# vitasoftAI/ImageRetrievalResearch

Measured on AMD Instinct MI355X. Metric: images/sec embed + queries/sec top-k@100k-gallery, EffNet-B3a 224^2, higher is better.
Workload: dtype bf16

## Files before the change

imageretrievalresearch_amd/_lib.py:

```python
from __future__ import annotations

import ctypes as C
import os

_HERE = os.path.dirname(os.path.abspath(__file__))
LIB_PATH = os.environ.get("MI355_LIB_PATH") or os.path.join(_HERE, "libmi355_retrieval.so")

c_f32p = C.POINTER(C.c_float)
c_i64p = C.POINTER(C.c_int64)
vp = C.c_void_p


class GemmExArgs(C.Structure):
    _fields_ = [("A", vp), ("lda", C.c_int), ("W", vp), ("ldw", C.c_int), ("bias", vp),
                ("res", vp), ("ldr", C.c_int), ("res_n", C.c_int),
                ("gate", vp), ("gate_ld", C.c_int), ("rows_per_img", C.c_int), ("a_relu6", C.c_int),
                ("out", vp), ("ldo", C.c_int), ("out_f32", C.c_int),
                ("M", C.c_int), ("N", C.c_int), ("K", C.c_int), ("act", C.c_int),
                ("M_sel", C.c_int64), ("splitk_ws", vp), ("splitk_ws_bytes", C.c_size_t),
                ("ln_stats", vp), ("ln_colsum", vp)]


class DwconvExArgs(C.Structure):
    _fields_ = [("in_", vp), ("w", vp), ("bias", vp), ("out", vp),
                ("B", C.c_int), ("H", C.c_int), ("W", C.c_int), ("C", C.c_int), ("k", C.c_int), ("stride", C.c_int),
                ("act", C.c_int), ("choice", C.c_int),
                ("se_w1", vp), ("se_b1", vp), ("se_w2t", vp), ("se_b2", vp), ("rd", C.c_int), ("act1", C.c_int),
                ("gate", vp), ("squeeze", vp)]


DW_CHOICE_AUTO, DW_CHOICE_DIRECT, DW_CHOICE_TILED, DW_CHOICE_MFMA = 0, 1, 2, 3


class RankFilter(C.Structure):
    _fields_ = [("query_labels", vp), ("gallery_labels", vp), ("label_mode", C.c_int), ("exclude", vp)]


LABEL_ANY, LABEL_SAME, LABEL_DIFFERENT = 0, 1, 2
DTYPE_F32, DTYPE_F16 = 0, 1

PROTOTYPES = {
    "mi355_abi_version": (C.c_int, []),
    "mi355_last_error": (C.c_char_p, []),
    "mi355_device_count": (C.c_int, []),
    "mi355_synth_fill": (C.c_int, [vp, C.c_int64, C.c_uint64, C.c_int64, C.c_int, vp]),
    "mi355_l2_normalize_rows": (C.c_int, [vp, vp, C.c_int64, C.c_int, C.c_float, vp]),
    "mi355_rank_workspace_bytes": (C.c_size_t, [C.c_int64, C.c_int64, C.c_int, C.c_int]),
    "mi355_rank_topk": (C.c_int, [vp, C.c_int64, vp, C.c_int64, C.c_int, C.c_int, C.c_int, C.c_float,
                                  C.c_int64, vp, vp, vp, C.c_size_t, vp]),
    "mi355_gallery_planes_bytes": (C.c_size_t, [C.c_int64, C.c_int]),
    "mi355_gallery_prepare": (C.c_int, [vp, C.c_int64, C.c_int, vp, C.c_size_t, vp]),
    "mi355_rank_topk_prepared": (C.c_int, [vp, C.c_int64, vp, C.c_int64, C.c_int, C.c_int, C.c_float, C.c_int64, vp, vp, vp,
                                           C.c_size_t, vp]),
    "mi355_gallery_f16_bytes": (C.c_size_t, [C.c_int64, C.c_int]),
    "mi355_gallery_to_f16": (C.c_int, [vp, C.c_int64, C.c_int, C.c_int, C.c_float, vp, C.c_size_t, vp]),
    "mi355_rank_f16_workspace_bytes": (C.c_size_t, [C.c_int64, C.c_int64, C.c_int, C.c_int]),
    "mi355_rank_topk_f16": (C.c_int, [vp, C.c_int64, vp, C.c_int64, C.c_int, C.c_int, C.c_float, C.c_int64, vp, vp, vp,
                                      C.c_size_t, vp]),
    "mi355_rank_topk_filtered": (C.c_int, [vp, C.c_int64, vp, C.c_int64, C.c_int, C.c_int, C.c_int, C.c_float, C.c_int64,
                                           C.POINTER(RankFilter), vp, vp, vp, C.c_size_t, vp]),
    "mi355_rank_topk_f16_filtered": (C.c_int, [vp, C.c_int64, vp, C.c_int64, C.c_int, C.c_int, C.c_float, C.c_int64,
                                               C.POINTER(RankFilter), vp, vp, vp, C.c_size_t, vp]),
    "mi355_rank_last_path": (C.c_int, []),
    "mi355_expand_workspace_bytes": (C.c_size_t, [C.c_int64, C.c_int, C.c_int]),
    "mi355_expand_rows": (C.c_int, [vp, C.c_int, C.c_int64, C.c_int, vp, C.c_int, C.c_int64, C.c_int64, C.c_int, vp, vp,
                                    C.c_int64, C.c_int, C.c_int64, C.c_float, C.c_float, vp, C.c_int, C.c_int64, vp,
                                    C.c_size_t, vp]),
    "mi355_kr_sets": (C.c_int, [vp, vp, vp, C.c_int64, C.c_int, vp, C.c_int64, vp, vp, C.c_int64, vp]),
    "mi355_kr_weights": (C.c_int, [vp, C.c_int, C.c_int64, C.c_int64, vp, C.c_int, C.c_int64, C.c_int64, C.c_int, vp, vp,
                                   C.c_int64, vp, vp]),
    "mi355_kr_local_qe": (C.c_int, [vp, C.c_int64, C.c_int, C.c_int, vp, vp, vp, C.c_int64, vp, vp, vp, C.c_int64, C.c_int64,
                                    vp, vp, vp, C.c_int64, vp]),
    "mi355_kr_score": (C.c_int, [vp, vp, vp, C.c_int64, C.c_int64, vp, vp, vp, C.c_int64, C.c_int64, vp, vp, C.c_int,
                                 C.c_float, vp, vp]),
    "mi355_moments_workspace_bytes": (C.c_size_t, [C.c_int64, C.c_int]),
    "mi355_embedding_moments": (C.c_int, [vp, C.c_int, C.c_int64, C.c_int64, C.c_int, C.c_int, C.c_float, C.c_int, vp, vp, vp,
                                          C.c_size_t, vp]),
    "mi355_whiten_workspace_bytes": (C.c_size_t, [C.c_int64, C.c_int, C.c_int, C.c_int]),
    "mi355_whiten_rows": (C.c_int, [vp, C.c_int, C.c_int64, C.c_int64, C.c_int, C.c_int, C.c_float, vp, vp, C.c_int, C.c_int, vp,
                                    C.c_int, C.c_int64, vp, C.c_size_t, vp]),
    "mi355_clear_pads": (C.c_int, [vp, vp, C.c_int64, C.c_int64, C.c_int64, vp]),
    "mi355_range_workspace_bytes": (C.c_size_t, [C.c_int64, C.c_int64, C.c_int]),
    "mi355_cosine_range": (C.c_int, [vp, C.c_int64, vp, C.c_int64, C.c_int, C.c_int, C.c_float, C.c_double, C.c_int64,
                                     C.POINTER(RankFilter), vp, C.c_int64, C.POINTER(C.c_int64), vp, C.c_size_t, vp]),
    "mi355_range_f16_workspace_bytes": (C.c_size_t, [C.c_int64, C.c_int64, C.c_int]),
    "mi355_cosine_range_f16": (C.c_int, [vp, C.c_int64, vp, C.c_int64, C.c_int, C.c_float, C.c_double, C.c_int64,
                                         C.POINTER(RankFilter), vp, C.c_int64, C.POINTER(C.c_int64), vp, C.c_size_t, vp]),
    "mi355_range_compact": (C.c_int, [vp, C.c_int64, C.c_int64, C.c_int64, C.c_int64, vp, C.c_size_t, vp, vp, vp, vp]),
    "mi355_roc_pairs_workspace_bytes": (C.c_size_t, [C.c_int64, C.c_int64, C.c_int]),
    "mi355_roc_pairs_hist": (C.c_int, [vp, C.c_int64, vp, C.c_int64, C.c_int, C.c_int, C.c_float, vp, vp, vp, C.c_int64,
                                       C.POINTER(C.c_double), vp, C.c_int, vp, vp, C.c_size_t, vp]),
    "mi355_roc_pairs_f16_workspace_bytes": (C.c_size_t, [C.c_int64, C.c_int64, C.c_int]),
    "mi355_roc_pairs_hist_f16": (C.c_int, [vp, C.c_int64, vp, C.c_int64, C.c_int, C.c_float, vp, vp, vp, C.c_int64,
                                           C.POINTER(C.c_double), vp, C.c_int, vp, vp, C.c_size_t, vp]),
    "mi355_roc_scores_hist": (C.c_int, [vp, C.c_int, C.c_int64, vp, C.POINTER(C.c_double), vp, C.c_int, vp, vp]),
    "mi355_roc_finalize": (C.c_int, [vp, C.c_int, vp, vp, vp, vp, vp]),
    "mi355_retrieval_metrics": (C.c_int, [vp, C.c_int64, C.c_int, vp, vp, C.c_int64, vp, vp, vp]),
    "mi355_cosine_scores": (C.c_int, [vp, C.c_int64, vp, C.c_int64, C.c_int, C.c_int, C.c_float, vp, vp,
                                      C.c_size_t, vp]),
    "mi355_topk_rows": (C.c_int, [vp, C.c_int64, C.c_int64, C.c_int, C.c_int64, vp, vp, vp, C.c_size_t, vp]),
    "mi355_merge_topk": (C.c_int, [vp, vp, C.c_int64, C.c_int, C.c_int, vp, vp, vp, C.c_size_t, vp]),
    "mi355_pack_candidates": (C.c_int, [vp, vp, C.c_int64, C.c_int, C.c_int, vp, vp]),
    "mi355_merge_packed_workspace_bytes": (C.c_size_t, [C.c_int64, C.c_int, C.c_int]),
    "mi355_merge_packed_topk": (C.c_int, [vp, vp, C.c_int, C.c_int64, C.c_int, vp, vp, vp, C.c_size_t, vp]),
    "mi355_pair_cosine": (C.c_int, [vp, vp, C.c_int64, C.c_int, C.c_float, vp, vp]),
    "mi355_contrastive_loss": (C.c_int, [vp, vp, C.c_int64, C.c_int, C.c_float, C.c_float, C.c_int, vp, vp, vp]),
    "mi355_cosine_embedding_loss": (C.c_int, [vp, vp, C.c_int64, C.c_int, C.c_float, C.c_float, C.c_int, vp, vp]),
    "mi355_hit_counts": (C.c_int, [vp, C.c_int64, C.c_int, vp, vp, C.c_int64, vp, vp]),
    "mi355_distinct_class_topn": (C.c_int, [vp, vp, C.c_int64, C.c_int, vp, C.c_int64, C.c_int, vp, vp, vp, vp]),
    "mi355_model_create": (C.c_int, [C.c_char_p, C.c_int, C.POINTER(vp)]),
    "mi355_model_destroy": (None, [vp]),
    "mi355_model_num_tensors": (C.c_int, [vp]),
    "mi355_model_tensor_info": (C.c_int, [vp, C.c_int, C.POINTER(C.c_char_p), C.POINTER(C.c_int),
                                          C.POINTER(C.c_int64), C.POINTER(C.c_int)]),
    "mi355_model_feature_dim": (C.c_int, [vp]),
    "mi355_model_num_classes": (C.c_int, [vp]),
    "mi355_model_set_tensor": (C.c_int, [vp, C.c_char_p, vp, C.c_int64]),
    "mi355_model_pack": (C.c_int, [vp, vp]),
    "mi355_model_forward_features": (C.c_int, [vp, vp, C.c_int, C.c_int, C.c_int, vp, vp, vp]),
    "mi355_model_forward": (C.c_int, [vp, vp, C.c_int, C.c_int, C.c_int, vp, vp, vp]),
    "mi355_model_forward_u8": (C.c_int, [vp, vp, C.c_int, C.c_int, C.c_int, C.c_int, C.POINTER(C.c_float), C.POINTER(C.c_float),
                                         vp, C.c_int, vp, vp, vp]),
    "mi355_model_enable_taps": (C.c_int, [vp, C.c_int]),
    "mi355_model_read_tap": (C.c_int, [vp, C.c_char_p, vp, C.c_int64, C.POINTER(C.c_int64), vp]),
    "mi355_model_run_between_taps": (C.c_int, [vp, C.c_char_p, C.c_char_p, vp, C.c_int, C.c_int, C.c_int, C.c_int, vp]),
    "mi355_model_traffic": (C.c_int, [vp, C.c_int, C.c_int, C.c_int, C.POINTER(C.c_double),
                                      C.POINTER(C.c_double), C.POINTER(C.c_double)]),
    "mi355_model_traffic_kinds": (C.c_int, [vp, C.c_int, C.c_int, C.c_int, C.POINTER(C.c_double),
                                            C.POINTER(C.c_double), C.c_int]),
    "mi355_model_set_option": (C.c_int, [vp, C.c_char_p, C.c_int64]),
    "mi355_model_profile_read": (C.c_int, [vp, C.POINTER(C.c_double), C.POINTER(C.c_int64), C.c_int]),
    "mi355_model_profile_ops": (C.c_int, [vp, C.c_int, C.c_int, C.c_int, C.c_int, C.POINTER(C.c_double),
                                          C.POINTER(C.c_double), C.POINTER(C.c_int), C.c_char_p, C.c_int]),
    "mi355_model_block_stamps": (C.c_int, [vp, C.POINTER(C.c_double), C.c_int]),
    "mi355_pool_linear": (C.c_int, [vp, C.c_int, C.c_int, C.c_int, vp, vp, C.c_int, vp, vp, vp]),
    "mi355_gemm_bf16": (C.c_int, [vp, vp, vp, vp, C.c_int, C.c_int, C.c_int, C.c_int, C.c_int, vp]),
    "mi355_gemm_bf16_ex": (C.c_int, [vp, C.POINTER(C.c_int), vp]),
    "mi355_dwconv_se_ex": (C.c_int, [vp, C.POINTER(C.c_int), vp]),
    "mi355_window_attention": (C.c_int, [vp, vp, vp, C.c_int, C.c_int, C.c_int, C.c_int, C.c_int, vp]),
    "mi355_window_attention_ws": (C.c_int, [vp, vp, vp, C.c_int, C.c_int, C.c_int, C.c_int, C.c_int, C.c_int, vp]),
    "mi355_swin_layernorm": (C.c_int, [vp, vp, vp, vp, C.c_int64, C.c_int, C.c_int, C.c_int, C.c_int, C.c_int, C.c_float, vp]),
    "mi355_swin_patch_embed": (C.c_int, [vp, vp, vp, C.c_int, C.c_int, C.c_int, C.c_int, C.c_int, C.c_int, C.POINTER(C.c_float),
                                         C.POINTER(C.c_float), vp, vp, vp, vp, C.c_int, C.c_float, vp, vp]),
    "mi355_swin_ln_token_mean": (C.c_int, [vp, vp, vp, vp, vp, C.c_int, C.c_int, C.c_int, C.c_float, vp]),
    "mi355_square_pad_normalize": (C.c_int, [vp, C.c_int, C.c_int, C.c_int, C.POINTER(C.c_float), C.POINTER(C.c_float), vp, vp]),
    "mi355_conv_input_silu": (C.c_int, [vp, vp, C.c_int, C.c_int, C.c_int, vp, vp]),
    "mi355_resize_bilinear_u8": (C.c_int, [vp, C.c_int, C.c_int, vp, C.c_int, C.c_int, vp, vp]),
    "mi355_resize_batch_workspace_bytes": (C.c_size_t, [vp, C.c_int, C.c_int, C.c_int, C.c_int]),
    "mi355_resize_batch_u8": (C.c_int, [vp, C.c_int64, vp, vp, C.c_int, C.c_int, C.c_int, C.c_int, C.c_int, vp, vp, C.c_size_t,
                                        vp]),
    "mi355_model_forward_images_workspace_bytes": (C.c_size_t, [vp, C.c_int, C.c_int, C.c_int]),
    "mi355_model_forward_images": (C.c_int, [vp, vp, C.c_int64, vp, vp, C.c_int, C.c_int, C.c_int, C.c_int, C.POINTER(C.c_float),
                                             C.POINTER(C.c_float), vp, C.c_int, vp, vp, vp, C.c_size_t, vp]),
    "mi355_score_boost": (C.c_int, [vp, C.c_int64, C.c_float, C.c_float, C.c_float, C.c_int, vp, vp]),
}

_lib = None


class MI355Error(RuntimeError):
    """A libmi355_retrieval call returned nonzero; the message is mi355_last_error()."""


def lib() -> C.CDLL:
    global _lib
    if _lib is None:
        if not os.path.exists(LIB_PATH):
            raise ImportError(
                f"{LIB_PATH} is missing: build it with `python -c 'import __graft_entry__ as g; g.build()'` "
                "(or `make -C imageretrievalresearch_amd/csrc`). There is no fallback path.")
        L = C.CDLL(LIB_PATH)
        for name, (res, args) in PROTOTYPES.items():
            fn = getattr(L, name)
            fn.restype = res
            fn.argtypes = args
        if L.mi355_abi_version() != 3:
            raise ImportError(f"ABI version mismatch: library {L.mi355_abi_version()} != binding 3")
        _lib = L
    return _lib


def check(status: int) -> None:
    if status != 0:
        raise MI355Error(lib().mi355_last_error().decode("utf-8", "replace"))


def stream_ptr(device=None) -> int:
    import torch
    return torch.cuda.current_stream(device).cuda_stream


def require_cuda(t, name: str):
    if not t.is_cuda:
        raise MI355Error(f"{name} must live on the GPU (got device {t.device}); "
                         "the MI355X path has no CPU fallback")
```

imageretrievalresearch_amd/csrc/rank.hip:

```cpp
#include "rank_common.h"
#include "../../include/mi355_retrieval.h"

#include <limits.h>
#include <stdlib.h>
#include <math.h>

namespace mi355 {

template <bool WRITE_ROWS>
__global__ __launch_bounds__(256) void k_row_norm(const float* __restrict__ in, float* __restrict__ out,
                                                  float* __restrict__ inv, i64 rows, int dim, float eps,
                                                  int vec) {
    const int lane = threadIdx.x & 63;
    const i64 row = (i64)blockIdx.x * 4 + (threadIdx.x >> 6);
    if (row >= rows) return;
    const float* x = in + row * dim;
    const float r = row_inv_norm(x, dim, eps, vec, lane);
    if (inv != nullptr && lane == 0) inv[row] = r;
    if (WRITE_ROWS) {
        float* y = out + row * dim;
        if (vec) {
            const f32x4* x4 = reinterpret_cast<const f32x4*>(x);
            f32x4* y4 = reinterpret_cast<f32x4*>(y);
            for (int i = lane; i < dim / 4; i += 64) {
                f32x4 v = x4[i];
                v.x *= r; v.y *= r; v.z *= r; v.w *= r;
                y4[i] = v;
            }
        } else {
            for (int i = lane; i < dim; i += 64) y[i] = x[i] * r;
        }
    }
}

__device__ __forceinline__ bool better(float a, i64 ia, float b, i64 ib) {
    const bool an = a != a, bn = b != b;
    if (an || bn) return (an && !bn) || (an && bn && ia < ib);
    return (a > b) || (a == b && ia < ib);
}

typedef __bf16 bf16x8 __attribute__((ext_vector_type(8)));
typedef unsigned u32x4 __attribute__((ext_vector_type(4)));

__device__ __forceinline__ void split3_pair(float x0, float x1, unsigned& h, unsigned& m, unsigned& l) {
    h = pack2bf(x0, x1);
    const float r0 = x0 - __uint_as_float(h << 16), r1 = x1 - __uint_as_float(h & 0xffff0000u);
    m = pack2bf(r0, r1);
    l = pack2bf(r0 - __uint_as_float(m << 16), r1 - __uint_as_float(m & 0xffff0000u));
}
__device__ __forceinline__ void split3(const f32x4 a, const f32x4 b, u32x4& h, u32x4& m, u32x4& l) {
    unsigned hh[4], mm[4], ll[4];
    split3_pair(a.x, a.y, hh[0], mm[0], ll[0]);
    split3_pair(a.z, a.w, hh[1], mm[1], ll[1]);
    split3_pair(b.x, b.y, hh[2], mm[2], ll[2]);
    split3_pair(b.z, b.w, hh[3], mm[3], ll[3]);
    h = (u32x4){hh[0], hh[1], hh[2], hh[3]};
    m = (u32x4){mm[0], mm[1], mm[2], mm[3]};
    l = (u32x4){ll[0], ll[1], ll[2], ll[3]};
}

__global__ __launch_bounds__(256) void k_split_queries(const float* __restrict__ Qn, bf16_t* __restrict__ Qs, int Q, int D,
                                                       int n_steps, int n_frag) {
    const int f = blockIdx.x * 4 + (threadIdx.x >> 6);
    if (blockIdx.x == 0 && threadIdx.x < 64) reinterpret_cast<unsigned*>(Qs + (size_t)n_frag * 3 * 512)[threadIdx.x] = 0u;
    if (f >= n_frag) return;
    const int lane = threadIdx.x & 63;
    const int rb = f / n_steps, s = f % n_steps;
    const int row = rb * 32 + (lane & 31), k0 = s * 16 + (lane >> 5) * 8;
    float x[8];
#pragma unroll
    for (int e = 0; e < 8; ++e) x[e] = (row < Q && k0 + e < D) ? Qn[(i64)row * D + k0 + e] : 0.f;
    u32x4 h, m, l;
    split3((f32x4){x[0], x[1], x[2], x[3]}, (f32x4){x[4], x[5], x[6], x[7]}, h, m, l);
    u32x4* o = reinterpret_cast<u32x4*>(Qs + (size_t)f * 3 * 512) + lane;
    o[0] = h; o[64] = m; o[128] = l;
}




template <int MT, int RK_BK, bool VEC, int FK>
__global__ __launch_bounds__(256) void k_cos_gemm(const float* __restrict__ Qn, const float* __restrict__ Gal,
                                                  const float* __restrict__ ginv, float* __restrict__ S,
                                                  int Q, i64 G, int D, int k, float* __restrict__ cand_val,
                                                  int* __restrict__ cand_idx, int x0, int ntx, int xtiles, int ny) {
    constexpr bool FILT = false;
    const RankFilter flt{};
#include "rank_gemm_f32.inc"
}
template <int MT, int RK_BK, bool VEC, int FK>
__global__ __launch_bounds__(256) void k_cos_gemm_filt(const float* __restrict__ Qn, const float* __restrict__ Gal,
                                                       const float* __restrict__ ginv, int Q, i64 G, int D, int k,
                                                       float* __restrict__ cand_val, int* __restrict__ cand_idx, int x0,
                                                       int ntx, int xtiles, int ny, RankFilter flt) {
    constexpr bool FILT = true;
    float* const S = nullptr;
#include "rank_gemm_f32.inc"
}
template <int MT, int RK_BK, bool VEC>
__global__ __launch_bounds__(256) void k_cos_gemm_roc(const float* __restrict__ Qn, const float* __restrict__ Gal,
                                                      const float* __restrict__ ginv, int Q, i64 G, int D, int x0, int ntx,
                                                      int xtiles, int ny, RocArgs flt) {
    constexpr int FK = FK_ROC;
    constexpr bool FILT = false;
    float* const S = nullptr;
    const int k = 0;
    float* const cand_val = nullptr;
    int* const cand_idx = nullptr;
#include "rank_gemm_f32.inc"
}
template <int MT, int RK_BK, bool VEC>
__global__ __launch_bounds__(256) void k_cos_gemm_range(const float* __restrict__ Qn, const float* __restrict__ Gal,
                                                        const float* __restrict__ ginv, int Q, i64 G, int D, int x0, int ntx,
                                                        int xtiles, int ny, RangeArgs flt) {
    constexpr int FK = FK_RANGE;
    constexpr bool FILT = false;
    float* const S = nullptr;
    const int k = 0;
    float* const cand_val = nullptr;
    int* const cand_idx = nullptr;
#include "rank_gemm_f32.inc"
}

template <int MT, int FK>
__global__ __launch_bounds__(256, 3) void k_cos_gemm_split(const bf16_t* __restrict__ Qs, const float* __restrict__ Gal,
                                                           const float* __restrict__ ginv, float* __restrict__ S, int Q,
                                                           i64 G, int D, int k, float* __restrict__ cand_val,
                                                           int* __restrict__ cand_idx, int x0, int ntx, int n_steps,
                                                           const float* __restrict__ zeros, int xtiles, int ny) {
    constexpr bool FILT = false;
    const RankFilter flt{};
#include "rank_gemm_split.inc"
}
template <int MT, int FK>
__global__ __launch_bounds__(256, 3) void k_cos_gemm_split_filt(const bf16_t* __restrict__ Qs, const float* __restrict__ Gal,
                                                                const float* __restrict__ ginv, int Q, i64 G, int D, int k,
                                                                float* __restrict__ cand_val, int* __restrict__ cand_idx,
                                                                int x0, int ntx, int n_steps, const float* __restrict__ zeros,
                                                                int xtiles, int ny, RankFilter flt) {
    constexpr bool FILT = true;
    float* const S = nullptr;
#include "rank_gemm_split.inc"
}
template <int MT>
__global__ __launch_bounds__(256, 3) void k_cos_gemm_split_roc(const bf16_t* __restrict__ Qs, const float* __restrict__ Gal,
                                                               const float* __restrict__ ginv, int Q, i64 G, int D, int x0,
                                                               int ntx, int n_steps, const float* __restrict__ zeros, int xtiles,
                                                               int ny, RocArgs flt) {
    constexpr int FK = FK_ROC;
    constexpr bool FILT = false;
    float* const S = nullptr;
    const int k = 0;
    float* const cand_val = nullptr;
    int* const cand_idx = nullptr;
#include "rank_gemm_split.inc"
}
template <int MT>
__global__ __launch_bounds__(256, 3) void k_cos_gemm_split_range(const bf16_t* __restrict__ Qs, const float* __restrict__ Gal,
                                                                 const float* __restrict__ ginv, int Q, i64 G, int D, int x0,
                                                                 int ntx, int n_steps, const float* __restrict__ zeros, int xtiles,
                                                                 int ny, RangeArgs flt) {
    constexpr int FK = FK_RANGE;
    constexpr bool FILT = false;
    float* const S = nullptr;
    const int k = 0;
    float* const cand_val = nullptr;
    int* const cand_idx = nullptr;
#include "rank_gemm_split.inc"
}

template <int MT, int FK>
__global__ __launch_bounds__(256, 2) void k_cos_gemm_pre(const bf16_t* __restrict__ Qs, const bf16_t* __restrict__ Gs,
                                                         float* __restrict__ S, int Q, i64 G, int k,
                                                         float* __restrict__ cand_val, int* __restrict__ cand_idx, int x0,
                                                         int ntx, int n_steps, int xtiles, int ny) {
    constexpr int BM = 64 * MT;
    constexpr int A_PIECES = (BM / 32) * 3;
    constexpr int A_STAGE = A_PIECES * 512;
    constexpr int B_PIECES = (RK_BN / 32) * 3;
    constexpr int B_STAGE = B_PIECES * 512;
    constexpr int A_RING = MT == 1 ? 3 : 2;
    extern __shared__ __attribute__((aligned(16))) float smem[];
    bf16_t* As = reinterpret_cast<bf16_t*>(smem);
    bf16_t* Bs = As + A_RING * A_STAGE;

    const int tid = threadIdx.x, lane = tid & 63, wave = tid >> 6;
    const int wm = wave >> 1, wn = wave & 1;
    int bx, by;
    rank_tile_of((int)blockIdx.x, xtiles, ny, bx, by);
    const i64 n0 = (i64)(bx + x0) * RK_BN;
    const int m0 = by * BM;
    const int swave = __builtin_amdgcn_readfirstlane(wave);

    const bf16_t* a_src = Qs + (size_t)(m0 / 32) * n_steps * 3 * 512 + lane * 8;
    const bf16_t* b_src = Gs + (size_t)(n0 / 32) * n_steps * 3 * 512 + lane * 8;
    const bf16_t* a_piece[(A_PIECES + 3) / 4];
    const bf16_t* b_piece[3];
#pragma unroll
    for (int i = 0; i < (A_PIECES + 3) / 4; ++i) {
        const int piece = (swave + 4 * i) % A_PIECES;
        a_piece[i] = a_src + ((size_t)((piece / 3) * n_steps) * 3 + piece % 3) * 512;
    }
#pragma unroll
    for (int i = 0; i < 3; ++i) {
        const int piece = swave + 4 * i;
        b_piece[i] = b_src + ((size_t)((piece / 3) * n_steps) * 3 + piece % 3) * 512;
    }
    auto dma_a = [&](int buf, int t) {
#pragma unroll
        for (int i = 0; i < (A_PIECES + 3) / 4; ++i) {
            const int piece = swave + 4 * i;
            if (A_PIECES % 4 == 0 || i < A_PIECES / 4 || swave < A_PIECES % 4)
                glds16(a_piece[i] + (size_t)t * 3 * 512, As + buf * A_STAGE + piece * 512);
        }
    };
    auto dma_b = [&](int stage, int t) {
        const int tt = t < n_steps ? t : n_steps - 1;
#pragma unroll
        for (int i = 0; i < 3; ++i) glds16(b_piece[i] + (size_t)tt * 3 * 512, Bs + stage * B_STAGE + (swave + 4 * i) * 512);
    };

    f32x16 acc[MT][2];
#pragma unroll
    for (int i = 0; i < MT; ++i)
#pragma unroll
        for (int j = 0; j < 2; ++j)
#pragma unroll
            for (int e = 0; e < 16; ++e) acc[i][j][e] = 0.f;

    auto compute = [&](int abuf, int bstage) {
        const bf16_t* a = As + abuf * A_STAGE + (wm * MT * 3) * 512 + lane * 8;
        const bf16_t* b = Bs + bstage * B_STAGE + (wn * 2 * 3) * 512 + lane * 8;
        bf16x8 af[MT][3], bfr[2][3];
#pragma unroll
        for (int j = 0; j < 2; ++j)
#pragma unroll
            for (int p = 0; p < 3; ++p) bfr[j][p] = *reinterpret_cast<const bf16x8*>(b + (j * 3 + p) * 512);
#pragma unroll
        for (int i = 0; i < MT; ++i)
#pragma unroll
            for (int p = 0; p < 3; ++p) af[i][p] = *reinterpret_cast<const bf16x8*>(a + (i * 3 + p) * 512);
#pragma unroll
        for (int j = 0; j < 2; ++j)
#pragma unroll
            for (int i = 0; i < MT; ++i) {
                acc[i][j] = __builtin_amdgcn_mfma_f32_32x32x16_bf16(af[i][2], bfr[j][0], acc[i][j], 0, 0, 0);
                acc[i][j] = __builtin_amdgcn_mfma_f32_32x32x16_bf16(af[i][0], bfr[j][2], acc[i][j], 0, 0, 0);
                acc[i][j] = __builtin_amdgcn_mfma_f32_32x32x16_bf16(af[i][1], bfr[j][1], acc[i][j], 0, 0, 0);
                acc[i][j] = __builtin_amdgcn_mfma_f32_32x32x16_bf16(af[i][1], bfr[j][0], acc[i][j], 0, 0, 0);
                acc[i][j] = __builtin_amdgcn_mfma_f32_32x32x16_bf16(af[i][0], bfr[j][1], acc[i][j], 0, 0, 0);
                acc[i][j] = __builtin_amdgcn_mfma_f32_32x32x16_bf16(af[i][0], bfr[j][0], acc[i][j], 0, 0, 0);
            }
    };

    dma_a(0, 0);
    if (A_RING == 3 && n_steps > 1) dma_a(1, 1);
    dma_b(0, 0);
    dma_b(1, 1);
    __syncthreads();

    int bs_cur = 0, bs_far = 2;
    for (int t = 0; t < n_steps; ++t) {
        if constexpr (A_RING == 2) {
            if (t + 1 < n_steps) dma_a((t & 1) ^ 1, t + 1);
        } else {
            if (t + 2 < n_steps) dma_a(bs_far, t + 2);
        }
        __builtin_amdgcn_sched_barrier(0);
        dma_b(bs_far, t + 2);
        __builtin_amdgcn_sched_barrier(0);
        compute(A_RING == 2 ? (t & 1) : bs_cur, bs_cur);
        if constexpr (A_RING == 2) {
            asm volatile("s_waitcnt vmcnt(3)" ::: "memory");
        } else {
            if (t + 2 >= n_steps) asm volatile("s_waitcnt vmcnt(3)" ::: "memory");
            else if (swave < A_PIECES % 4) asm volatile("s_waitcnt vmcnt(5)" ::: "memory");
            else asm volatile("s_waitcnt vmcnt(4)" ::: "memory");
        }
        asm volatile("s_waitcnt lgkmcnt(0)" ::: "memory");
        __builtin_amdgcn_s_barrier();
        asm volatile("" ::: "memory");
        bs_cur = bs_cur == 2 ? 0 : bs_cur + 1;
        bs_far = bs_far == 2 ? 0 : bs_far + 1;
    }
    __syncthreads();
    cos_gemm_epilogue<MT, FK>(acc, smem, nullptr, S, Q, G, k, cand_val, cand_idx, x0, ntx, n0, m0);
}

template <int NQ>
__global__ __launch_bounds__(256) void k_cos_gemv(const float* __restrict__ Qn, const float* __restrict__ Gal,
                                                  const float* __restrict__ ginv, float* __restrict__ S, i64 G, int D,
                                                  int vec) {
    extern __shared__ __attribute__((aligned(16))) float qs[];
    for (int i = threadIdx.x; i < NQ * D; i += 256) qs[i] = Qn[i];
    __syncthreads();
    const int lane = threadIdx.x & 63;
    const i64 wave_id = (i64)blockIdx.x * 4 + (threadIdx.x >> 6);
    const i64 nwaves = (i64)gridDim.x * 4;
    for (i64 g = wave_id; g < G; g += nwaves) {
        const float* row = Gal + g * D;
        float acc[NQ];
#pragma unroll
        for (int q = 0; q < NQ; ++q) acc[q] = 0.f;
        if (vec) {
            const f32x4* r4 = reinterpret_cast<const f32x4*>(row);
#pragma unroll 2
            for (int i = lane; i < D / 4; i += 64) {
                const f32x4 v = r4[i];
#pragma unroll
                for (int q = 0; q < NQ; ++q) {
                    const f32x4 u = *reinterpret_cast<const f32x4*>(&qs[q * D + i * 4]);
                    acc[q] += v.x * u.x + v.y * u.y + v.z * u.z + v.w * u.w;
                }
            }
        } else {
            for (int i = lane; i < D; i += 64) {
                const float v = row[i];
#pragma unroll
                for (int q = 0; q < NQ; ++q) acc[q] += v * qs[q * D + i];
            }
        }
        const float gs = ginv ? ginv[g] : 1.0f;
#pragma unroll
        for (int q = 0; q < NQ; ++q) {
            const float t = wave_sum(acc[q]);
            if (lane == 0) S[(i64)q * G + g] = t * gs;
        }
    }
}

template <int K>
__global__ __launch_bounds__(256) void k_topk_small(const float* __restrict__ vals, const i64* __restrict__ idxs,
                                                    const int* __restrict__ idxs32,
                                                    i64 rowlen, i64 in_stride, i64 chunk_len, int k,
                                                    i64 idx_offset, float* __restrict__ ov, i64* __restrict__ oi) {
    constexpr bool FILT = false;
    const RankFilter flt{};
#include "rank_topk_small.inc"
}
template <int K>
__global__ __launch_bounds__(256) void k_topk_small_filt(const float* __restrict__ vals, i64 rowlen, i64 in_stride,
                                                         i64 chunk_len, int k, i64 idx_offset, float* __restrict__ ov,
                                                         i64* __restrict__ oi, RankFilter flt) {
    constexpr bool FILT = true;
    const i64* const idxs = nullptr;
    const int* const idxs32 = nullptr;
#include "rank_topk_small.inc"
}

constexpr int BT_N = 2048;
__global__ __launch_bounds__(256) void k_topk_bitonic(const float* __restrict__ vals, const i64* __restrict__ idxs,
                                                      i64 rowlen, i64 in_stride, int k, i64 idx_offset,
                                                      float* __restrict__ ov, i64* __restrict__ oi) {
    constexpr bool FILT = false;
    const RankFilter flt{};
#include "rank_topk_bitonic.inc"
}
__global__ __launch_bounds__(256) void k_topk_bitonic_filt(const float* __restrict__ vals, i64 rowlen, i64 in_stride, int k,
                                                           i64 idx_offset, float* __restrict__ ov, i64* __restrict__ oi,
                                                           RankFilter flt) {
    constexpr bool FILT = true;
    const i64* const idxs = nullptr;
#include "rank_topk_bitonic.inc"
}

__global__ __launch_bounds__(256) void k_clear_pads(float* __restrict__ v, i64* __restrict__ ix, i64 n, i64 lo, i64 hi) {
    const i64 t = (i64)blockIdx.x * 256 + threadIdx.x;
    if (t < n && (ix[t] < lo || ix[t] >= hi)) { v[t] = NEG_INF; ix[t] = -1; }
}

__global__ __launch_bounds__(256) void k_pair_cosine(const float* __restrict__ a, const float* __restrict__ b,
                                                     i64 rows, int dim, float eps, float* __restrict__ out) {
    const int lane = threadIdx.x & 63;
    const i64 row = (i64)blockIdx.x * 4 + (threadIdx.x >> 6);
    if (row >= rows) return;
    const float* x = a + row * dim;
    const float* y = b + row * dim;
    float xx = 0.f, yy = 0.f, xy = 0.f;
    for (int i = lane; i < dim; i += 64) {
        const float u = x[i], w = y[i];
        xx += u * u; yy += w * w; xy += u * w;
    }
    xx = wave_sum(xx); yy = wave_sum(yy); xy = wave_sum(xy);
    if (lane == 0) out[row] = xy / (fmaxf(sqrtf(xx), eps) * fmaxf(sqrtf(yy), eps));
}

__global__ __launch_bounds__(1024) void k_contrastive(const float* __restrict__ f1, const float* __restrict__ f2,
                                                      i64 rows, int dim, float label, float margin, int mean,
                                                      float* __restrict__ out, float* __restrict__ per_row) {
    __shared__ float part[16];
    const int lane = threadIdx.x & 63, wave = threadIdx.x >> 6;
    float acc = 0.f;
    for (i64 r = wave; r < rows; r += 16) {
        const float* x = f1 + r * dim;
        const float* y = f2 + r * dim;
        float d = 0.f;
        for (int i = lane; i < dim; i += 64) {
            const float t = y[i] - x[i];
            d += t * t;
        }
        d = wave_sum(d);
        const float h = fmaxf(margin - sqrtf(d + 1e-9f), 0.f);
        const float l = 0.5f * (label * d + (1.0f - label) * h * h);
        if (per_row && lane == 0) per_row[r] = l;
        acc += l;
    }
    if (lane == 0) part[wave] = acc;
    __syncthreads();
    if (threadIdx.x == 0) {
        float s = 0.f;
        for (int w = 0; w < 16; ++w) s += part[w];
        out[0] = mean ? s / (float)rows : s;
    }
}

__global__ __launch_bounds__(1024) void k_cos_embedding_loss(const float* __restrict__ f1, const float* __restrict__ f2,
                                                             i64 rows, int dim, float target, float margin, int mean,
                                                             float* __restrict__ out) {
    __shared__ float part[16];
    const int lane = threadIdx.x & 63, wave = threadIdx.x >> 6;
    float acc = 0.f;
    for (i64 r = wave; r < rows; r += 16) {
        const float* x = f1 + r * dim;
        const float* y = f2 + r * dim;
        float xx = 0.f, yy = 0.f, xy = 0.f;
        for (int i = lane; i < dim; i += 64) {
            const float u = x[i], v = y[i];
            xx += u * u; yy += v * v; xy += u * v;
        }
        xx = wave_sum(xx); yy = wave_sum(yy); xy = wave_sum(xy);
        const float c = xy / sqrtf((xx + 1e-12f) * (yy + 1e-12f));
        acc += target > 0.f ? 1.0f - c : fmaxf(c - margin, 0.f);
    }
    if (lane == 0) part[wave] = acc;
    __syncthreads();
    if (threadIdx.x == 0) {
        float t = 0.f;
        for (int w = 0; w < 16; ++w) t += part[w];
        out[0] = mean ? t / (float)rows : t;
    }
}

__global__ __launch_bounds__(256) void k_pack_candidates(const float* __restrict__ val, const i64* __restrict__ idx, i64 Q,
                                                         int kk, int k, int* __restrict__ packed) {
    const i64 t = (i64)blockIdx.x * 256 + threadIdx.x;
    if (t >= Q * k) return;
    const i64 q = t / k;
    const int j = (int)(t - q * k);
    int2 o;
    if (j < kk) { o.x = __float_as_int(val[q * kk + j]); o.y = (int)idx[q * kk + j]; }
    else { o.x = __float_as_int(NEG_INF); o.y = -1; }
    reinterpret_cast<int2*>(packed)[t] = o;
}

constexpr i64 PACKED_PAD_IDX = NO_CAND_IDX;
__global__ __launch_bounds__(256) void k_unpack_candidates(const int* __restrict__ packed, const i64* __restrict__ offsets,
                                                           int world, i64 Q, int k, float* __restrict__ cv, i64* __restrict__ ci) {
    const i64 t = (i64)blockIdx.x * 256 + threadIdx.x;
    const i64 per = (i64)world * k;
    if (t >= Q * per) return;
    const i64 q = t / per;
    const int c = (int)(t - q * per), r = c / k, j = c - r * k;
    const int2 p = reinterpret_cast<const int2*>(packed)[((i64)r * Q + q) * k + j];
    cv[t] = __int_as_float(p.x);
    ci[t] = p.y >= 0 ? (i64)p.y + offsets[r] : PACKED_PAD_IDX;
}

__global__ void k_hit_counts(const i64* __restrict__ idx, i64 Q, int k, const i64* __restrict__ qcls,
                             const i64* __restrict__ gcls, i64 G, i64* __restrict__ counts) {
    const i64 q = (i64)blockIdx.x * blockDim.x + threadIdx.x;
    int h1 = 0, h3 = 0;
    if (q < Q) {
        const i64 c = qcls[q];
        for (int j = 0; j < min(k, 3); ++j) {
            const i64 g = idx[q * k + j];
            const int hit = (g >= 0 && g < G) ? (gcls[g] == c) : 0;
            if (j == 0) h1 = hit;
            h3 |= hit;
        }
    }
    const unsigned long long m1 = __ballot(h1), m3 = __ballot(h3);
    if ((threadIdx.x & 63) == 0) {
        if (m1) atomicAdd((unsigned long long*)&counts[0], (unsigned long long)__popcll(m1));
        if (m3) atomicAdd((unsigned long long*)&counts[1], (unsigned long long)__popcll(m3));
    }
}

__global__ void k_distinct_topn(const i64* __restrict__ idx, const float* __restrict__ val, i64 Q, int k,
                                const i64* __restrict__ gcls, i64 G, int n, i64* __restrict__ ocls,
                                i64* __restrict__ oidx, float* __restrict__ oval) {
    const i64 q = (i64)blockIdx.x * blockDim.x + threadIdx.x;
    if (q >= Q) return;
    i64 seen[8];
    int ns = 0;
    for (int j = 0; j < n; ++j) { ocls[q * n + j] = -1; oidx[q * n + j] = -1; oval[q * n + j] = NAN; }
    for (int j = 0; j < k && ns < n; ++j) {
        const i64 g = idx[q * k + j];
        if (g < 0 || g >= G) continue;
        const i64 c = gcls[g];
        bool dup = false;
#pragma unroll
        for (int s = 0; s < 8; ++s) dup |= (s < ns && seen[s] == c);
        if (!dup) {
#pragma unroll
            for (int s = 0; s < 8; ++s)
                if (s == ns) seen[s] = c;
            ocls[q * n + ns] = c; oidx[q * n + ns] = g; oval[q * n + ns] = val[q * k + j];
            ++ns;
        }
    }
}

__global__ __launch_bounds__(256) void k_retrieval_metrics(const i64* __restrict__ idx, i64 Q, int k, const i64* __restrict__ qcls,
                                                           const i64* __restrict__ gcls, i64 G, const i64* __restrict__ R,
                                                           double* __restrict__ out) {
    const int lane = threadIdx.x & 63;
    const i64 q = (i64)blockIdx.x * 4 + (threadIdx.x >> 6);
    if (q >= Q) return;
    const i64 c = qcls[q], Rq = R[q];
    int first = k, run = 0, hits = 0;
    double ap = 0.0;
    for (int i0 = 0; i0 < k; i0 += 64) {
        const int i = i0 + lane;
        bool rel = false;
        if (i < k) {
            const i64 g = idx[q * k + i];
            rel = g >= 0 && g < G && gcls[g] == c;
        }
        const unsigned long long m = __ballot(rel);
        if (first == k && m) first = i0 + __ffsll((long long)m) - 1;
        const int cum = run + __popcll(m & ((1ull << lane) - 1)) + (rel ? 1 : 0);
        if (rel && i < Rq) ap += (double)cum / (double)(i + 1);
        hits += __popcll(__ballot(rel && i < Rq));
        run += __popcll(m);
    }
#pragma unroll
    for (int o = 32; o > 0; o >>= 1) ap += __shfl_xor(ap, o, 64);
    if (lane == 0) {
        double* o = out + q * 3;
        o[0] = first;
        o[1] = Rq > 0 ? (double)hits / (double)Rq : 0.0;
        o[2] = Rq > 0 ? ap / (double)Rq : 0.0;
    }
}

constexpr i64 SMALL_CHUNK = 8192;

struct TopkPlan {
    bool small;
    i64 nchunk1;
    size_t cand_elems;
};

static i64 level1_chunks(i64 G, int k) { return k <= SMALL_K ? cdiv(G, SMALL_CHUNK) : cdiv(G, BT_N); }

size_t topk_ws_bytes(i64 Q, i64 G, int k) {
    const i64 per_row = level1_chunks(G, k) * k;
    return 2 * align_up((size_t)Q * per_row * (sizeof(float) + sizeof(i64)), 256) + 256;
}

template <int K>
static void launch_small(const float* v, const i64* ix, const int* ix32, i64 rowlen, i64 in_stride, i64 chunk_len, int k,
                         i64 off, float* ov, i64* oi, i64 nchunk, i64 Q, hipStream_t st, const RankFilter* filt) {
    if (filt)
        hipLaunchKernelGGL((k_topk_small_filt<K>), dim3((unsigned)nchunk, (unsigned)Q), dim3(256), 0, st, v, rowlen, in_stride,
                           chunk_len, k, off, ov, oi, *filt);
    else
        hipLaunchKernelGGL((k_topk_small<K>), dim3((unsigned)nchunk, (unsigned)Q), dim3(256), 0, st, v, ix, ix32, rowlen,
                           in_stride, chunk_len, k, off, ov, oi);
}
static void dispatch_small(const float* v, const i64* ix, const int* ix32, i64 rowlen, i64 in_stride, i64 chunk_len, int k,
                           i64 off, float* ov, i64* oi, i64 nchunk, i64 Q, hipStream_t st, const RankFilter* filt) {
    if (k <= 1) launch_small<1>(v, ix, ix32, rowlen, in_stride, chunk_len, k, off, ov, oi, nchunk, Q, st, filt);
    else if (k <= 2) launch_small<2>(v, ix, ix32, rowlen, in_stride, chunk_len, k, off, ov, oi, nchunk, Q, st, filt);
    else if (k <= 4) launch_small<4>(v, ix, ix32, rowlen, in_stride, chunk_len, k, off, ov, oi, nchunk, Q, st, filt);
    else launch_small<8>(v, ix, ix32, rowlen, in_stride, chunk_len, k, off, ov, oi, nchunk, Q, st, filt);
}

static thread_local int g_rank_path = 0;
void set_rank_path(int path) { g_rank_path = path; }

RankFilter filter_from(const RankFilter& f, i64 q0) {
    RankFilter r = f;
    if (r.qlab) r.qlab += q0;
    if (r.excl) r.excl += q0;
    return r;
}

int make_filter(const mi355_rank_filter* f, i64 idx_offset, const char* who, RankFilter* out) {
    MI355_REQUIRE(f, "%s: null filter (use the unfiltered entry)", who);
    MI355_REQUIRE(f->label_mode == MI355_LABEL_ANY || f->label_mode == MI355_LABEL_SAME || f->label_mode == MI355_LABEL_DIFFERENT,
                  "%s: unknown label_mode %d", who, f->label_mode);
    MI355_REQUIRE(f->label_mode == MI355_LABEL_ANY || (f->query_labels && f->gallery_labels),
                  "%s: label_mode %d needs query_labels and gallery_labels (null pointer)", who, f->label_mode);
    out->qlab = f->label_mode != MI355_LABEL_ANY ? (const i64*)f->query_labels : nullptr;
    out->glab = f->label_mode != MI355_LABEL_ANY ? (const i64*)f->gallery_labels : nullptr;
    out->excl = (const i64*)f->exclude;
    out->idx_offset = idx_offset;
    out->mode = f->label_mode;
    return OK;
}

int topk_select(const float* vals, const i64* idxs, i64 Q, i64 rowlen, i64 in_stride, int k, i64 idx_offset,
                float* out_val, i64* out_idx, void* ws, size_t ws_bytes, hipStream_t st, const int* idxs32,
                const RankFilter* filt) {
    MI355_REQUIRE(k >= 1 && k <= LARGE_K, "top-k: k=%d outside [1,%d]", k, LARGE_K);
    MI355_REQUIRE(k <= rowlen, "top-k: k=%d exceeds row length %lld", k, (long long)rowlen);
    MI355_REQUIRE(!idxs32 || k <= SMALL_K, "top-k: int32 candidate lists need k <= %d", SMALL_K);
    MI355_REQUIRE(Q >= 1 && Q <= 65535 * 16, "top-k: Q=%lld out of range", (long long)Q);
    MI355_REQUIRE(ws_bytes >= topk_ws_bytes(Q, rowlen, k), "top-k: workspace %zu < %zu bytes", ws_bytes,
                  topk_ws_bytes(Q, rowlen, k));
    const i64 per_row_max = level1_chunks(rowlen, k) * k;
    const size_t half = align_up((size_t)Q * per_row_max * (sizeof(float) + sizeof(i64)), 256);
    char* base = (char*)(((uintptr_t)ws + 255) & ~(uintptr_t)255);
    float* cv[2];
    i64* ci[2];
    for (int b = 0; b < 2; ++b) {
        ci[b] = (i64*)(base + b * half);
        cv[b] = (float*)(base + b * half + (size_t)Q * per_row_max * sizeof(i64));
    }
    for (i64 qs = 0; qs < Q; qs += 65535) {
        const i64 qn = (Q - qs < 65535) ? Q - qs : 65535;
        const float* v = vals + qs * in_stride;
        const i64* ix = idxs ? idxs + qs * in_stride : nullptr;
        const int* ix32 = idxs32 ? idxs32 + qs * in_stride : nullptr;
        i64 len = rowlen, stride = in_stride;
        i64 off = idx_offset;
        int cur = 0;
        RankFilter fs{};
        if (filt) fs = filter_from(*filt, qs);
        const RankFilter* f1 = (filt && !ix && !ix32) ? &fs : nullptr;
        while (true) {
            const bool small = (k <= SMALL_K);
            const i64 chunk = small ? SMALL_CHUNK : BT_N;
            const i64 nchunk = cdiv(len, chunk);
            const bool last = (nchunk == 1);
            float* ovp = last ? out_val + qs * k : cv[cur];
            i64* oip = last ? out_idx + qs * k : ci[cur];
            if (small) dispatch_small(v, ix, ix32, len, stride, chunk, k, off, ovp, oip, nchunk, qn, st, f1);
            else if (f1) hipLaunchKernelGGL(k_topk_bitonic_filt, dim3((unsigned)nchunk, (unsigned)qn), dim3(256), 0, st, v, len,
                                            stride, k, off, ovp, oip, *f1);
            else hipLaunchKernelGGL(k_topk_bitonic, dim3((unsigned)nchunk, (unsigned)qn), dim3(256), 0, st, v, ix,
                                    len, stride, k, off, ovp, oip);
            MI355_LAUNCH_CHECK();
            if (last) break;
            v = cv[cur]; ix = ci[cur]; ix32 = nullptr; f1 = nullptr;
            len = nchunk * k; stride = len; off = 0;
            cur ^= 1;
        }
    }
    if (filt) {
        hipLaunchKernelGGL(k_clear_pads, dim3((unsigned)cdiv(Q * k, 256)), dim3(256), 0, st, out_val, out_idx, Q * k, (i64)LLONG_MIN,
                           IDX_PAD);
        MI355_LAUNCH_CHECK();
    }
    return OK;
}

bool fused_select(i64 Q, i64 G, int k) { return k >= 1 && k <= SMALL_K && Q > 4 && G < ((i64)1 << 31) - RK_BN; }

i64 query_block(i64 Q, i64 G, int k) {
    if (fused_select(Q, G, k)) {
        i64 qb = ((i64)1 << 25) / (cdiv(G, RK_BN) * (i64)k * 8);
        qb = qb / 128 * 128;
        if (qb < 128) qb = 128;
        return qb < Q ? qb : Q;
    }
    i64 qb = ((i64)1 << 28) / (G > 0 ? G : 1);
    qb = qb / 256 * 256;
    if (qb < 256) qb = 256;
    return qb < Q ? qb : Q;
}

static size_t split_queries_bytes(i64 Q, int D) { return (size_t)cdiv(Q, 128) * 4 * cdiv(D, 16) * 3 * 1024 + 256; }
static int split_rows(const float* x, i64 n, int D, bf16_t* planes, hipStream_t st) {
    const int n_steps = cdiv(D, 16);
    const i64 n_frag = (i64)cdiv(n, 128) * 4 * n_steps;
    hipLaunchKernelGGL(k_split_queries, dim3((unsigned)cdiv(n_frag, 4)), dim3(256), 0, st, x, planes, (int)n, D, n_steps, (int)n_frag);
    MI355_LAUNCH_CHECK();
    return OK;
}

RankWs carve(void* ws, i64 Q, i64 G, int D, int k, size_t (*planes_bytes)(i64, int), bool need_ginv, bool need_S) {
    RankWs r{};
    const bool fused = need_S && fused_select(Q, G, k);
    const i64 qb = query_block(Q, G, need_S ? k : 0);
    size_t off = 0;
    char* base = ws ? (char*)(((uintptr_t)ws + 255) & ~(uintptr_t)255) : nullptr;
    auto take = [&](size_t bytes) { char* p = base ? base + off : nullptr; off += align_up(bytes, 256); return p; };
    r.qn = (float*)take((size_t)Q * D * sizeof(float));
    const i64 q_split = need_S ? qb : (Q < 256 * 64 ? Q : 256 * 64);
    r.qs = take(planes_bytes ? planes_bytes(q_split, D) : 0);
    r.ginv = (float*)take(need_ginv ? (size_t)G * sizeof(float) : 0);
    if (fused) {
        const size_t ncand = (size_t)qb * cdiv(G, RK_BN) * k;
        r.cand_val = (float*)take(ncand * sizeof(float));
        r.cand_idx = (int*)take(ncand * sizeof(int));
        r.topk_bytes = topk_ws_bytes(qb, cdiv(G, RK_BN) * (i64)k, k);
    } else {
        r.S = (float*)take(need_S ? (size_t)qb * G * sizeof(float) : 0);
        r.topk_bytes = k > 0 ? topk_ws_bytes(qb, G, k) : 0;
    }
    r.topk = take(r.topk_bytes);
    r.total = off + 256;
    return r;
}

int kernel_slots(const void* fn, size_t lds, int* cache, int* slots_out) {
    int dev = 0;
    MI355_CHECK_HIP(hipGetDevice(&dev));
    MI355_REQUIRE(dev >= 0 && dev < MI355_MAX_DEVICES, "rank: device ordinal %d out of range", dev);
    if (!cache[dev]) {
        MI355_CHECK_HIP(hipFuncSetAttribute(fn, hipFuncAttributeMaxDynamicSharedMemorySize, (int)lds));
        int per_cu = 0, cus = 0;
        MI355_CHECK_HIP(hipOccupancyMaxActiveBlocksPerMultiprocessor(&per_cu, fn, 256, lds));
        MI355_CHECK_HIP(hipDeviceGetAttribute(&cus, hipDeviceAttributeMultiprocessorCount, dev));
        cache[dev] = (per_cu > 0 ? per_cu : 1) * (cus > 0 ? cus : 1);
    }
    *slots_out = cache[dev];
    return OK;
}

int whole_round_tiles(int ntx, int ny, int slots) {
    if ((long)ntx * ny > slots && ((long)ntx * ny) % slots != 0) return (int)(((long)ntx * ny / slots) * slots / ny);
    return ntx;
}

template <bool VEC>
struct F32Gemm {
    static constexpr bool SLAB = true, FILTERED = true, ROC = true, RANGE = true;
    template <int MT> static constexpr int BK = MT == 2 ? 16 : 32;
    template <int MT> static constexpr size_t stage_bytes() { return (size_t)2 * (64 * MT + RK_BN) * (BK<MT> + 4) * sizeof(float); }
    template <int MT, int FK, bool FILT> static const void* kernel() {
        if constexpr (FK == FK_ROC) return (const void*)k_cos_gemm_roc<MT, BK<MT>, VEC>;
        else if constexpr (FK == FK_RANGE) return (const void*)k_cos_gemm_range<MT, BK<MT>, VEC>;
        else if constexpr (FILT) return (const void*)k_cos_gemm_filt<MT, BK<MT>, VEC, FK>;
        else return (const void*)k_cos_gemm<MT, BK<MT>, VEC, FK>;
    }
    template <int MT, int FK, bool FILT>
    static void launch(dim3 grid, size_t lds, hipStream_t st, const TileArgs& a, int x0, int ntx, int xtiles, int ny) {
        const float* qn = (const float*)a.qry;
        const float* gal = (const float*)a.gal;
        if constexpr (FK == FK_ROC)
            hipLaunchKernelGGL((k_cos_gemm_roc<MT, BK<MT>, VEC>), grid, dim3(256), lds, st, qn, gal, a.ginv, a.Q, a.G, a.D, x0, ntx,
                               xtiles, ny, *a.roc);
        else if constexpr (FK == FK_RANGE)
            hipLaunchKernelGGL((k_cos_gemm_range<MT, BK<MT>, VEC>), grid, dim3(256), lds, st, qn, gal, a.ginv, a.Q, a.G, a.D, x0, ntx,
                               xtiles, ny, *a.rng);
        else if constexpr (FILT)
            hipLaunchKernelGGL((k_cos_gemm_filt<MT, BK<MT>, VEC, FK>), grid, dim3(256), lds, st, qn, gal, a.ginv, a.Q, a.G, a.D, a.k,
                               a.cand_val, a.cand_idx, x0, ntx, xtiles, ny, *a.filt);
        else
            hipLaunchKernelGGL((k_cos_gemm<MT, BK<MT>, VEC, FK>), grid, dim3(256), lds, st, qn, gal, a.ginv, a.S, a.Q, a.G, a.D, a.k,
                               a.cand_val, a.cand_idx, x0, ntx, xtiles, ny);
    }
};

struct SplitGemm {
    static constexpr bool SLAB = true, FILTERED = true, ROC = true, RANGE = true;
    template <int MT> static constexpr size_t stage_bytes() {
        return (size_t)(MT == 1 ? 3 : 2) * (64 * MT / 32) * 3 * 1024 + (size_t)3 * RK_BN * 16 * sizeof(float);
    }
    template <int MT, int FK, bool FILT> static const void* kernel() {
        if constexpr (FK == FK_ROC) return (const void*)k_cos_gemm_split_roc<MT>;
        else if constexpr (FK == FK_RANGE) return (const void*)k_cos_gemm_split_range<MT>;
        else if constexpr (FILT) return (const void*)k_cos_gemm_split_filt<MT, FK>;
        else return (const void*)k_cos_gemm_split<MT, FK>;
    }
    template <int MT, int FK, bool FILT>
    static void launch(dim3 grid, size_t lds, hipStream_t st, const TileArgs& a, int x0, int ntx, int xtiles, int ny) {
        const bf16_t* qs = (const bf16_t*)a.qry;
        const float* gal = (const float*)a.gal;
        const int n_steps = cdiv(a.D, 16);
        const float* zeros = reinterpret_cast<const float*>(qs + (size_t)cdiv(a.Q, 128) * 4 * n_steps * 3 * 512);
        if constexpr (FK == FK_ROC)
            hipLaunchKernelGGL((k_cos_gemm_split_roc<MT>), grid, dim3(256), lds, st, qs, gal, a.ginv, a.Q, a.G, a.D, x0, ntx, n_steps,
                               zeros, xtiles, ny, *a.roc);
        else if constexpr (FK == FK_RANGE)
            hipLaunchKernelGGL((k_cos_gemm_split_range<MT>), grid, dim3(256), lds, st, qs, gal, a.ginv, a.Q, a.G, a.D, x0, ntx, n_steps,
                               zeros, xtiles, ny, *a.rng);
        else if constexpr (FILT)
            hipLaunchKernelGGL((k_cos_gemm_split_filt<MT, FK>), grid, dim3(256), lds, st, qs, gal, a.ginv, a.Q, a.G, a.D, a.k,
                               a.cand_val, a.cand_idx, x0, ntx, n_steps, zeros, xtiles, ny, *a.filt);
        else
            hipLaunchKernelGGL((k_cos_gemm_split<MT, FK>), grid, dim3(256), lds, st, qs, gal, a.ginv, a.S, a.Q, a.G, a.D, a.k,
                               a.cand_val, a.cand_idx, x0, ntx, n_steps, zeros, xtiles, ny);
    }
};

struct PreparedGemm {
    static constexpr bool SLAB = false, FILTERED = false, ROC = false, RANGE = false;
    template <int MT> static constexpr size_t stage_bytes() {
        return (size_t)(MT == 1 ? 3 : 2) * (64 * MT / 32) * 3 * 1024 + (size_t)3 * (RK_BN / 32) * 3 * 1024;
    }
    template <int MT, int FK, bool FILT> static const void* kernel() {
        static_assert(!FILT && FK > 0, "the prepared gallery has fused unfiltered kernels only");
        return (const void*)k_cos_gemm_pre<MT, FK>;
    }
    template <int MT, int FK, bool FILT>
    static void launch(dim3 grid, size_t lds, hipStream_t st, const TileArgs& a, int x0, int ntx, int xtiles, int ny) {
        hipLaunchKernelGGL((k_cos_gemm_pre<MT, FK>), grid, dim3(256), lds, st, (const bf16_t*)a.qry, (const bf16_t*)a.gal, a.S, a.Q,
                           a.G, a.k, a.cand_val, a.cand_idx, x0, ntx, cdiv(a.D, 16), xtiles, ny);
    }
};

static bool rank_exact_f32() {
    const char* e = getenv("MI355_RANK_EXACT_F32");
    return e && e[0] && e[0] != '0';
}

static int cos_gemm(const float* qn, bf16_t* qs, const float* gal, const float* ginv, float* S, i64 Q, i64 G, int D,
                    hipStream_t st, int k = 0, float* cand_val = nullptr, int* cand_idx = nullptr,
                    const RankFilter* filt = nullptr, const RocArgs* roc = nullptr, const RangeArgs* rng = nullptr) {
    const bool vec = vec_ok(qn, D) && vec_ok(gal, D);
    const int fused_bit = cand_val ? MI355_RANK_PATH_FUSED : 0;
    if (!cand_val && !roc && !rng && Q <= 4 && (size_t)Q * D * sizeof(float) <= 60 * 1024) {
        set_rank_path(MI355_RANK_PATH_GEMV);
        const size_t lds = (size_t)Q * D * sizeof(float);
        const unsigned blocks = (unsigned)(cdiv(G, 4) < 4096 ? cdiv(G, 4) : 4096);
#define GEMV_LAUNCH(NQ) hipLaunchKernelGGL((k_cos_gemv<NQ>), dim3(blocks), dim3(256), lds, st, qn, gal, ginv, S, G, D, (int)vec)
        if (Q == 1) GEMV_LAUNCH(1); else if (Q == 2) GEMV_LAUNCH(2); else if (Q == 3) GEMV_LAUNCH(3); else GEMV_LAUNCH(4);
#undef GEMV_LAUNCH
        MI355_LAUNCH_CHECK();
        return OK;
    }
    TileArgs a{qn, gal, ginv, S, (int)Q, G, D, k, cand_val, cand_idx, filt, roc, rng};
    if (qs && vec_ok(gal, D) && !rank_exact_f32()) {
        if (int e = split_rows(qn, Q, D, qs, st)) return e;
        set_rank_path(MI355_RANK_PATH_SPLIT | fused_bit);
        a.qry = qs;
        return cos_gemm_tiles<SplitGemm>(a, st);
    }
    set_rank_path(MI355_RANK_PATH_EXACT_F32 | fused_bit);
    return vec ? cos_gemm_tiles<F32Gemm<true>>(a, st) : cos_gemm_tiles<F32Gemm<false>>(a, st);
}

int normalize_search(const float* queries, i64 Q, const float* gallery, i64 G, int dim, float eps, const RankWs& w,
                     hipStream_t st) {
    const int vq = vec_ok(queries, dim) && vec_ok(w.qn, dim);
    RoctxRange range("rank/normalize");
    hipLaunchKernelGGL((k_row_norm<true>), dim3((unsigned)cdiv(Q, 4)), dim3(256), 0, st, queries, w.qn, (float*)nullptr, (i64)Q,
                       dim, eps, vq);
    MI355_LAUNCH_CHECK();
    if (gallery) {
        hipLaunchKernelGGL((k_row_norm<false>), dim3((unsigned)cdiv(G, 4)), dim3(256), 0, st, gallery, (float*)nullptr, w.ginv,
                           (i64)G, dim, eps, vec_ok(gallery, dim));
        MI355_LAUNCH_CHECK();
    }
    return OK;
}

static int check_rank_args(const float* queries, i64 Q, const float* gallery, i64 G, int dim) {
    MI355_REQUIRE(queries && gallery, "rank: null queries/gallery pointer");
    MI355_REQUIRE(Q >= 1, "rank: Q=%lld must be >= 1", (long long)Q);
    MI355_REQUIRE(G >= 1, "rank: G=%lld must be >= 1", (long long)G);
    MI355_REQUIRE(dim >= 1, "rank: dim=%d must be >= 1", dim);
    return OK;
}
static int check_topk_args(const float* queries, i64 Q, const float* gallery, i64 G, int dim, int k, const float* out_val,
                           const int64_t* out_idx, const char* who) {
    if (int e = check_rank_args(queries, Q, gallery, G, dim)) return e;
    MI355_REQUIRE(out_val && out_idx, "%s: null output", who);
    MI355_REQUIRE(k >= 1 && k <= LARGE_K, "%s: k=%d outside [1,%d]", who, k, LARGE_K);
    MI355_REQUIRE(k <= G, "%s: k=%d exceeds gallery rows %lld", who, k, (long long)G);
    return OK;
}

static int rank_topk(const float* queries, i64 Q, const float* gallery, i64 G, int dim, int gallery_is_normalized, int k, float eps,
                     i64 idx_offset, float* out_val, i64* out_idx, void* workspace, size_t workspace_bytes, hipStream_t st,
                     const RankFilter* filt) {
    const RankWs w = carve(workspace, Q, G, dim, k, split_queries_bytes, !gallery_is_normalized);
    MI355_REQUIRE(workspace && workspace_bytes >= w.total, "rank_topk: workspace %zu < %zu bytes", workspace_bytes,
                  w.total);
    const float* ginv = gallery_is_normalized ? nullptr : w.ginv;
    return search_blocks(queries, ginv ? gallery : nullptr, Q, G, dim, k, eps, idx_offset, filt, out_val, out_idx, w, st, nullptr,
                         [&](i64 q0, i64 qn, const RankFilter* f) -> int {
                             RoctxRange range(w.cand_val ? "rank/cosine gemm + per-tile top-k" : nullptr);
                             return cos_gemm(w.qn + q0 * dim, (bf16_t*)w.qs, gallery, ginv, w.S, qn, G, dim, st, k, w.cand_val,
                                             w.cand_idx, f);
                         });
}

}

using namespace mi355;

extern "C" {

int mi355_l2_normalize_rows(const float* in, float* out, int64_t rows, int dim, float eps, void* stream) {
    MI355_REQUIRE(in && out, "l2_normalize_rows: null pointer");
    MI355_REQUIRE(rows >= 0 && dim >= 1, "l2_normalize_rows: bad shape rows=%lld dim=%d", (long long)rows, dim);
    if (rows == 0) return OK;
    const int vec = vec_ok(in, dim) && vec_ok(out, dim);
    hipLaunchKernelGGL((k_row_norm<true>), dim3((unsigned)cdiv(rows, 4)), dim3(256), 0, (hipStream_t)stream, in, out,
                       (float*)nullptr, (i64)rows, dim, eps, vec);
    MI355_LAUNCH_CHECK();
    return OK;
}

size_t mi355_rank_workspace_bytes(int64_t Q, int64_t G, int dim, int k) {
    if (Q < 1 || G < 1) return 0;
    if (dim <= 0) return topk_ws_bytes(Q, G, k < 1 ? 1 : k) + 256;
    return carve(nullptr, Q, G, dim, k, split_queries_bytes, true).total;
}

int mi355_cosine_scores(const float* queries, int64_t Q, const float* gallery, int64_t G, int dim,
                        int gallery_is_normalized, float eps, float* out, void* workspace, size_t workspace_bytes,
                        void* stream) {
    if (int e = check_rank_args(queries, Q, gallery, G, dim)) return e;
    MI355_REQUIRE(out, "cosine_scores: null output");
    hipStream_t st = (hipStream_t)stream;
    RankWs w = carve(workspace, Q, G, dim, 0, split_queries_bytes, !gallery_is_normalized, false);
    MI355_REQUIRE(workspace && workspace_bytes >= w.total, "cosine_scores: workspace %zu < %zu bytes",
                  workspace_bytes, w.total);
    const int vq = vec_ok(queries, dim) && vec_ok(w.qn, dim);
    hipLaunchKernelGGL((k_row_norm<true>), dim3((unsigned)cdiv(Q, 4)), dim3(256), 0, st, queries, w.qn,
                       (float*)nullptr, (i64)Q, dim, eps, vq);
    MI355_LAUNCH_CHECK();
    if (!gallery_is_normalized) {
        hipLaunchKernelGGL((k_row_norm<false>), dim3((unsigned)cdiv(G, 4)), dim3(256), 0, st, gallery,
                           (float*)nullptr, w.ginv, (i64)G, dim, eps, vec_ok(gallery, dim));
        MI355_LAUNCH_CHECK();
    }
    const float* ginv = gallery_is_normalized ? nullptr : w.ginv;
    for (i64 qs = 0; qs < Q; qs += 256 * 64) {
        const i64 qn = (Q - qs < 256 * 64) ? Q - qs : 256 * 64;
        if (int e = cos_gemm(w.qn + qs * dim, (bf16_t*)w.qs, gallery, ginv, out + qs * G, qn, G, dim, st)) return e;
    }
    return OK;
}

int mi355_rank_topk(const float* queries, int64_t Q, const float* gallery, int64_t G, int dim,
                    int gallery_is_normalized, int k, float eps, int64_t idx_offset, float* out_val,
                    int64_t* out_idx, void* workspace, size_t workspace_bytes, void* stream) {
    if (int e = check_topk_args(queries, Q, gallery, G, dim, k, out_val, out_idx, "rank_topk")) return e;
    return rank_topk(queries, Q, gallery, G, dim, gallery_is_normalized, k, eps, idx_offset, out_val, (i64*)out_idx, workspace,
                     workspace_bytes, (hipStream_t)stream, nullptr);
}

int mi355_rank_topk_filtered(const float* queries, int64_t Q, const float* gallery, int64_t G, int dim,
                             int gallery_is_normalized, int k, float eps, int64_t idx_offset, const mi355_rank_filter* filter,
                             float* out_val, int64_t* out_idx, void* workspace, size_t workspace_bytes, void* stream) {
    if (int e = check_topk_args(queries, Q, gallery, G, dim, k, out_val, out_idx, "rank_topk_filtered")) return e;
    RankFilter f{};
    if (int e = make_filter(filter, idx_offset, "rank_topk_filtered", &f)) return e;
    return rank_topk(queries, Q, gallery, G, dim, gallery_is_normalized, k, eps, idx_offset, out_val, (i64*)out_idx, workspace,
                     workspace_bytes, (hipStream_t)stream, &f);
}

int mi355_rank_last_path(void) { return g_rank_path; }

size_t mi355_roc_pairs_workspace_bytes(int64_t Q, int64_t G, int dim) {
    if (Q < 1 || G < 1 || dim < 1) return 0;
    return carve(nullptr, Q, G, dim, 0, split_queries_bytes, true, false).total;
}

int mi355_roc_pairs_hist(const float* queries, int64_t Q, const float* gallery, int64_t G, int dim, int gallery_is_normalized,
                         float eps, const int64_t* query_labels, const int64_t* gallery_labels, const int64_t* exclude,
                         int64_t idx_offset, const double* thresholds, const double* thresholds_dev, int T, int64_t* hist,
                         void* workspace, size_t workspace_bytes, void* stream) {
    const char* who = "roc_pairs_hist";
    RocArgs roc{};
    if (int e = roc_check_thresholds(thresholds, T, who, &roc)) return e;
    if (int e = roc_check_pairs(query_labels, gallery_labels, exclude, idx_offset, thresholds_dev, hist, who, &roc)) return e;
    MI355_REQUIRE(queries && gallery, "%s: null queries/gallery pointer", who);
    MI355_REQUIRE(Q >= 1 && G >= 1 && dim >= 1, "%s: bad shape Q=%lld G=%lld dim=%d", who, (long long)Q, (long long)G, dim);
    MI355_REQUIRE(Q <= INT_MAX && G < ((int64_t)1 << 31) - RK_BN, "%s: shape too large Q=%lld G=%lld", who, (long long)Q,
                  (long long)G);
    const i64 qb = roc_query_block(Q, G);
    const RankWs w = carve(workspace, Q, G, dim, 0, split_queries_bytes, !gallery_is_normalized, false);
    const size_t need = mi355_roc_pairs_workspace_bytes(Q, G, dim);
    MI355_REQUIRE(workspace && workspace_bytes >= need, "%s: workspace %zu < %zu bytes", who, workspace_bytes, need);
    hipStream_t st = (hipStream_t)stream;
    MI355_CHECK_HIP(hipMemsetAsync(hist, 0, (size_t)2 * (T + 1) * sizeof(int64_t), st));
    const float* ginv = gallery_is_normalized ? nullptr : w.ginv;
    if (int e = normalize_search(queries, Q, ginv ? gallery : nullptr, G, dim, eps, w, st)) return e;
    for (i64 q0 = 0; q0 < Q; q0 += qb) {
        const i64 qn = (Q - q0 < qb) ? Q - q0 : qb;
        const RocArgs rb = roc_from(roc, q0);
        RoctxRange range("roc/cosine gemm + histogram");
        if (int e = cos_gemm(w.qn + q0 * dim, (bf16_t*)w.qs, gallery, ginv, nullptr, qn, G, dim, st, 0, nullptr, nullptr, nullptr, &rb))
            return e;
    }
    return OK;
}

size_t mi355_range_workspace_bytes(int64_t Q, int64_t G, int dim) {
    if (Q < 0 || G < 0 || dim < 1) return 0;
    return range_carve(nullptr, Q, G, dim, split_queries_bytes, true).total;
}

int mi355_cosine_range(const float* queries, int64_t Q, const float* gallery, int64_t G, int dim, int gallery_is_normalized,
                       float eps, double threshold, int64_t idx_offset, const mi355_rank_filter* filter, void* candidates,
                       int64_t capacity, int64_t* nnz, void* workspace, size_t workspace_bytes, void* stream) {
    const char* who = "cosine_range";
    RankFilter f{};
    if (int e = range_check(queries, Q, gallery, G, dim, threshold, filter, idx_offset, candidates, capacity, nnz, who, &f)) return e;
    const RangeWs w = range_carve(workspace, Q, G, dim, split_queries_bytes, !gallery_is_normalized);
    MI355_REQUIRE(workspace && workspace_bytes >= w.total, "%s: workspace %zu < %zu bytes", who, workspace_bytes, w.total);
    hipStream_t st = (hipStream_t)stream;
    if (Q == 0 || G == 0) return range_empty(w, Q, nnz, st);
    const float* ginv = gallery_is_normalized ? nullptr : w.w.ginv;
    if (int e = normalize_search(queries, Q, ginv ? gallery : nullptr, G, dim, eps, w.w, st)) return e;
    return range_blocks(Q, G, f, threshold, candidates, capacity, nnz, w, st, [&](i64 q0, i64 qn, const RangeArgs& a) -> int {
        RoctxRange range("range/cosine gemm + hits");
        return cos_gemm(w.w.qn + q0 * dim, (bf16_t*)w.w.qs, gallery, ginv, nullptr, qn, G, dim, st, 0, nullptr, nullptr, nullptr,
                        nullptr, &a);
    });
}

int mi355_clear_pads(float* val, int64_t* idx, int64_t n, int64_t lo, int64_t hi, void* stream) {
    MI355_REQUIRE(val && idx, "clear_pads: null pointer");
    MI355_REQUIRE(n >= 0, "clear_pads: n=%lld < 0", (long long)n);
    if (n == 0) return OK;
    hipLaunchKernelGGL(k_clear_pads, dim3((unsigned)cdiv(n, 256)), dim3(256), 0, (hipStream_t)stream, val, (i64*)idx, (i64)n,
                       (i64)lo, (i64)hi);
    MI355_LAUNCH_CHECK();
    return OK;
}

int mi355_retrieval_metrics(const int64_t* idx, int64_t Q, int k, const int64_t* query_cls, const int64_t* gallery_cls,
                            int64_t G, const int64_t* R, double* per_query, void* stream) {
    MI355_REQUIRE(idx && query_cls && gallery_cls && R && per_query, "retrieval_metrics: null pointer");
    MI355_REQUIRE(Q >= 1 && G >= 1, "retrieval_metrics: bad shape Q=%lld G=%lld", (long long)Q, (long long)G);
    MI355_REQUIRE(k >= 1 && k <= LARGE_K, "retrieval_metrics: k=%d outside [1,%d]", k, LARGE_K);
    hipLaunchKernelGGL(k_retrieval_metrics, dim3((unsigned)cdiv(Q, 4)), dim3(256), 0, (hipStream_t)stream, (const i64*)idx, (i64)Q,
                       k, (const i64*)query_cls, (const i64*)gallery_cls, (i64)G, (const i64*)R, per_query);
    MI355_LAUNCH_CHECK();
    return OK;
}

size_t mi355_gallery_planes_bytes(int64_t G, int dim) {
    if (G < 1 || dim < 1) return 0;
    return split_queries_bytes(G, dim);
}

int mi355_gallery_prepare(const float* gallery_normalized, int64_t G, int dim, void* planes, size_t planes_bytes, void* stream) {
    MI355_REQUIRE(gallery_normalized && planes, "gallery_prepare: null pointer");
    MI355_REQUIRE(G >= 1 && dim >= 1 && G < ((int64_t)1 << 31) - RK_BN, "gallery_prepare: bad shape G=%lld dim=%d", (long long)G, dim);
    MI355_REQUIRE(planes_bytes >= mi355_gallery_planes_bytes(G, dim), "gallery_prepare: planes buffer %zu < %zu bytes", planes_bytes,
                  mi355_gallery_planes_bytes(G, dim));
    MI355_REQUIRE((i64)cdiv(G, 128) * 4 * cdiv(dim, 16) < ((i64)1 << 31), "gallery_prepare: gallery too large for one call");
    return split_rows(gallery_normalized, G, dim, (bf16_t*)planes, (hipStream_t)stream);
}

int mi355_rank_topk_prepared(const float* queries, int64_t Q, const void* gallery_planes, int64_t G, int dim, int k, float eps,
                             int64_t idx_offset, float* out_val, int64_t* out_idx, void* workspace, size_t workspace_bytes,
                             void* stream) {
    MI355_REQUIRE(queries && gallery_planes && out_val && out_idx, "rank_topk_prepared: null pointer");
    MI355_REQUIRE(Q >= 1 && G >= 1 && dim >= 1, "rank_topk_prepared: bad shape Q=%lld G=%lld dim=%d", (long long)Q, (long long)G, dim);
    MI355_REQUIRE(k >= 1 && k <= G, "rank_topk_prepared: k=%d outside [1, %lld]", k, (long long)G);
    MI355_REQUIRE(fused_select(Q, G, k), "rank_topk_prepared: needs k <= %d and more than 4 queries (got k=%d, Q=%lld)", SMALL_K, k, (long long)Q);
    hipStream_t st = (hipStream_t)stream;
    const RankWs w = carve(workspace, Q, G, dim, k, split_queries_bytes, false);
    MI355_REQUIRE(workspace && workspace_bytes >= w.total, "rank_topk_prepared: workspace %zu < %zu bytes", workspace_bytes, w.total);
    return search_blocks(queries, nullptr, Q, G, dim, k, eps, idx_offset, nullptr, out_val, (i64*)out_idx, w, st, nullptr,
                         [&](i64 q0, i64 qn, const RankFilter*) -> int {
                             RoctxRange range("rank/cosine gemm (prepared gallery) + per-tile top-k");
                             if (int e = split_rows(w.qn + q0 * dim, qn, dim, (bf16_t*)w.qs, st)) return e;
                             set_rank_path(MI355_RANK_PATH_PREPARED | MI355_RANK_PATH_FUSED);
                             return cos_gemm_tiles<PreparedGemm>({w.qs, gallery_planes, nullptr, nullptr, (int)qn, G, dim, k, w.cand_val,
                                                                  w.cand_idx, nullptr}, st);
                         });
}

int mi355_topk_rows(const float* scores, int64_t Q, int64_t G, int k, int64_t idx_offset, float* out_val,
                    int64_t* out_idx, void* workspace, size_t workspace_bytes, void* stream) {
    MI355_REQUIRE(scores && out_val && out_idx, "topk_rows: null pointer");
    MI355_REQUIRE(Q >= 1 && G >= 1, "topk_rows: bad shape Q=%lld G=%lld", (long long)Q, (long long)G);
    MI355_REQUIRE(workspace, "topk_rows: null workspace");
    return topk_select(scores, nullptr, Q, G, G, k, idx_offset, out_val, (i64*)out_idx, workspace, workspace_bytes,
                       (hipStream_t)stream);
}

int mi355_merge_topk(const float* cand_val, const int64_t* cand_idx, int64_t Q, int ncand, int k, float* out_val,
                     int64_t* out_idx, void* workspace, size_t workspace_bytes, void* stream) {
    MI355_REQUIRE(cand_val && cand_idx && out_val && out_idx, "merge_topk: null pointer");
    MI355_REQUIRE(Q >= 1 && ncand >= 1, "merge_topk: bad shape Q=%lld ncand=%d", (long long)Q, ncand);
    MI355_REQUIRE(workspace, "merge_topk: null workspace");
    return topk_select(cand_val, (const i64*)cand_idx, Q, ncand, ncand, k, 0, out_val, (i64*)out_idx, workspace,
                       workspace_bytes, (hipStream_t)stream);
}

int mi355_pack_candidates(const float* val, const int64_t* idx, int64_t Q, int kk, int k, int32_t* packed, void* stream) {
    MI355_REQUIRE(packed && Q >= 1 && k >= 1 && kk >= 0 && kk <= k, "pack_candidates: bad arguments Q=%lld kk=%d k=%d",
                  (long long)Q, kk, k);
    MI355_REQUIRE(kk == 0 || (val && idx), "pack_candidates: null candidates");
    const i64 n = (i64)Q * k;
    hipLaunchKernelGGL(k_pack_candidates, dim3((unsigned)cdiv(n, 256)), dim3(256), 0, (hipStream_t)stream, val,
                       (const i64*)idx, (i64)Q, kk, k, packed);
    MI355_LAUNCH_CHECK();
    return OK;
}

size_t mi355_merge_packed_workspace_bytes(int64_t Q, int world, int k) {
    if (Q < 1 || world < 1 || k < 1) return 0;
    const size_t n = (size_t)Q * world * k;
    return align_up(n * sizeof(i64), 256) + align_up(n * sizeof(float), 256) + topk_ws_bytes(Q, (i64)world * k, k) + 512;
}

int mi355_merge_packed_topk(const int32_t* packed, const int64_t* shard_offsets, int world, int64_t Q, int k,
                            float* out_val, int64_t* out_idx, void* workspace, size_t workspace_bytes, void* stream) {
    MI355_REQUIRE(packed && shard_offsets && out_val && out_idx, "merge_packed_topk: null pointer");
    MI355_REQUIRE(Q >= 1 && world >= 1 && k >= 1, "merge_packed_topk: bad shape Q=%lld world=%d k=%d", (long long)Q, world, k);
    MI355_REQUIRE(workspace && workspace_bytes >= mi355_merge_packed_workspace_bytes(Q, world, k),
                  "merge_packed_topk: workspace %zu < %zu bytes", workspace_bytes, mi355_merge_packed_workspace_bytes(Q, world, k));
    const size_t n = (size_t)Q * world * k;
    char* base = (char*)(((uintptr_t)workspace + 255) & ~(uintptr_t)255);
    i64* ci = (i64*)base;
    float* cv = (float*)(base + align_up(n * sizeof(i64), 256));
    char* rest = base + align_up(n * sizeof(i64), 256) + align_up(n * sizeof(float), 256);
    hipLaunchKernelGGL(k_unpack_candidates, dim3((unsigned)cdiv((i64)n, 256)), dim3(256), 0, (hipStream_t)stream, packed,
                       (const i64*)shard_offsets, world, (i64)Q, k, cv, ci);
    MI355_LAUNCH_CHECK();
    return topk_select(cv, ci, Q, (i64)world * k, (i64)world * k, k, 0, out_val, (i64*)out_idx, rest,
                       workspace_bytes - (size_t)(rest - (char*)workspace), (hipStream_t)stream);
}

int mi355_pair_cosine(const float* a, const float* b, int64_t rows, int dim, float eps, float* out, void* stream) {
    MI355_REQUIRE(a && b && out, "pair_cosine: null pointer");
    MI355_REQUIRE(rows >= 0 && dim >= 1, "pair_cosine: bad shape");
    if (rows == 0) return OK;
    hipLaunchKernelGGL(k_pair_cosine, dim3((unsigned)cdiv(rows, 4)), dim3(256), 0, (hipStream_t)stream, a, b,
                       (i64)rows, dim, eps, out);
    MI355_LAUNCH_CHECK();
    return OK;
}

int mi355_contrastive_loss(const float* fm1, const float* fm2, int64_t rows, int dim, float label, float margin,
                           int mean, float* out, float* per_row, void* stream) {
    MI355_REQUIRE(fm1 && fm2 && out, "contrastive_loss: null pointer");
    MI355_REQUIRE(rows >= 1 && dim >= 1, "contrastive_loss: bad shape rows=%lld dim=%d", (long long)rows, dim);
    hipLaunchKernelGGL(k_contrastive, dim3(1), dim3(1024), 0, (hipStream_t)stream, fm1, fm2, (i64)rows, dim, label,
                       margin, mean, out, per_row);
    MI355_LAUNCH_CHECK();
    return OK;
}

int mi355_cosine_embedding_loss(const float* x1, const float* x2, int64_t rows, int dim, float target, float margin,
                                int mean, float* out, void* stream) {
    MI355_REQUIRE(x1 && x2 && out, "cosine_embedding_loss: null pointer");
    MI355_REQUIRE(rows >= 1 && dim >= 1, "cosine_embedding_loss: bad shape rows=%lld dim=%d", (long long)rows, dim);
    MI355_REQUIRE(target == 1.0f || target == -1.0f, "cosine_embedding_loss: target must be +1 or -1");
    hipLaunchKernelGGL(k_cos_embedding_loss, dim3(1), dim3(1024), 0, (hipStream_t)stream, x1, x2, (i64)rows, dim, target,
                       margin, mean, out);
    MI355_LAUNCH_CHECK();
    return OK;
}

int mi355_hit_counts(const int64_t* idx, int64_t Q, int k, const int64_t* query_cls, const int64_t* gallery_cls,
                     int64_t G, int64_t* counts, void* stream) {
    MI355_REQUIRE(idx && query_cls && gallery_cls && counts, "hit_counts: null pointer");
    MI355_REQUIRE(Q >= 1 && k >= 1 && G >= 1, "hit_counts: bad shape");
    hipLaunchKernelGGL(k_hit_counts, dim3((unsigned)cdiv(Q, 256)), dim3(256), 0, (hipStream_t)stream, (const i64*)idx,
                       (i64)Q, k, (const i64*)query_cls, (const i64*)gallery_cls, (i64)G, (i64*)counts);
    MI355_LAUNCH_CHECK();
    return OK;
}

int mi355_distinct_class_topn(const int64_t* idx, const float* val, int64_t Q, int k, const int64_t* gallery_cls,
                              int64_t G, int n, int64_t* out_cls, int64_t* out_idx, float* out_val, void* stream) {
    MI355_REQUIRE(idx && val && gallery_cls && out_cls && out_idx && out_val, "distinct_class_topn: null pointer");
    MI355_REQUIRE(Q >= 1 && k >= 1 && G >= 1 && n >= 1 && n <= 8, "distinct_class_topn: bad shape (n must be 1..8)");
    hipLaunchKernelGGL(k_distinct_topn, dim3((unsigned)cdiv(Q, 128)), dim3(128), 0, (hipStream_t)stream,
                       (const i64*)idx, val, (i64)Q, k, (const i64*)gallery_cls, (i64)G, n, (i64*)out_cls, (i64*)out_idx,
                       out_val);
    MI355_LAUNCH_CHECK();
    return OK;
}

}
```

imageretrievalresearch_amd/csrc/rank_common.h:

```cpp
#pragma once
#include "common.h"
#include "../../include/mi355_retrieval.h"

#include <limits.h>
#include <math.h>

namespace mi355 {

typedef float f32x4 __attribute__((ext_vector_type(4)));
typedef float f32x16 __attribute__((ext_vector_type(16)));
typedef long long i64;

constexpr float NEG_INF = -INFINITY;
constexpr i64 IDX_PAD = LLONG_MAX;
constexpr i64 NO_CAND_IDX = (i64)1 << 62;

constexpr int IDX32_PAD = INT_MAX;

__device__ __forceinline__ unsigned score_key(float x) {
    const unsigned u = __float_as_uint(x + 0.0f);
    if ((u & 0x7fffffffu) > 0x7f800000u) return 0xffffffffu;
    return (u & 0x80000000u) ? ~u : (u | 0x80000000u);
}
__device__ __forceinline__ float key_score(unsigned key) {
// ... 115 lines not shown
#pragma unroll
                for (int src = 1; src < 4; ++src) {
#pragma unroll
                    for (int i = 0; i < FK; ++i) {
                        const unsigned ok = (unsigned)__shfl(kv[i], (lane & ~3) + src, 64);
                        const int oi = __shfl(ki[i], (lane & ~3) + src, 64);
                        if (part == 0) insert(ok, oi);
                    }
                }
                const int qrow = m0 + h * 64 + lrow;
                if (part == 0 && qrow < Q) {
                    const size_t o = ((size_t)qrow * ntx + (size_t)(n0 / RK_BN)) * k;
#pragma unroll
                    for (int i = 0; i < FK; ++i)
                        if (i < k) { cand_val[o + i] = ki[i] == IDX32_PAD ? NEG_INF : key_score(kv[i]); cand_idx[o + i] = ki[i]; }
                }
            }
            __syncthreads();
        }
        return;
    }
#pragma unroll
    for (int j = 0; j < 2; ++j) {
        const i64 col = n0 + wn * 64 + j * 32 + lr;
        if (col >= G) continue;
        const float gs = ginv ? ginv[col] : 1.0f;
#pragma unroll
        for (int i = 0; i < MT; ++i) {
#pragma unroll
            for (int r = 0; r < 16; ++r) {
                const int row = m0 + wm * MT * 32 + i * 32 + (r & 3) + 8 * (r >> 2) + 4 * (lane >> 5);
                if (row < Q) S[(i64)row * G + col] = acc[i][j][r] * gs;
            }
        }
    }
}

constexpr int ROC_MAX_T = MI355_ROC_MAX_THRESHOLDS;
constexpr int ROC_SUB_T = 1024;
constexpr int ROC_BIN_WORDS = ROC_MAX_T + 4;
constexpr int FK_ROC = -1;

__host__ __device__ __forceinline__ float roc_ceil_f32(double t) {
    float f = (float)t;
    if ((double)f < t) f = nextafterf(f, INFINITY);
    return f;
}

struct RocArgs {
    const i64* qlab;
    const i64* glab;
    const i64* excl;
    i64 idx_offset;
    const double* thr;
    unsigned long long* hist;
    int T;
    int top;
    int uniform;
    float scale;
};

template <class V>
__device__ __forceinline__ int roc_bin(V s, const V* tab, const RocArgs& a) {
    if (a.uniform) {
        if (!(s >= tab[0])) return 0;
        const V x = (s - tab[0]) * (V)a.scale;
        int g = x < (V)(a.T - 1) ? (int)x + 1 : a.T;
        while (g < a.T && s >= tab[g]) ++g;
        while (s < tab[g - 1]) --g;
        return g;
    }
    int b = 0;
    for (int step = a.top; step > 0; step >>= 1)
        if (b + step <= a.T && tab[b + step - 1] <= s) b += step;
    return b;
}

constexpr size_t ROC_EPI_BYTES = (size_t)ROC_MAX_T * sizeof(float) + (size_t)ROC_BIN_WORDS * sizeof(unsigned) +
                                 (size_t)3 * RK_BN * sizeof(i64);

template <int MT, int FK, bool FILT>
__device__ __forceinline__ void cos_gemm_epilogue(f32x16 (&acc)[MT][2], float* smem, const float* __restrict__ ginv, float*, int Q,
                                                  i64 G, int, float*, int*, int, int, i64 n0, int m0, const RocArgs& roc) {
    static_assert(FK == FK_ROC && !FILT, "the histogram twins pass FK = FK_ROC, FILT = false");
    constexpr int BM = 64 * MT;
    const int tid = threadIdx.x, lane = tid & 63, wave = tid >> 6;
    const int wm = wave >> 1, wn = wave & 1, lr = lane & 31;
    const int T = roc.T, nb = T + 1;
    const bool sub = T <= ROC_SUB_T;
    float* tab = smem;
    unsigned* bins = reinterpret_cast<unsigned*>(smem + ROC_MAX_T);
    i64* glab = reinterpret_cast<i64*>(bins + ROC_BIN_WORDS);
    i64* qlab = glab + RK_BN;
    i64* qex = qlab + RK_BN;
    for (int i = tid; i < T; i += 256) tab[i] = roc_ceil_f32(roc.thr[i]);
    for (int i = tid; i < (sub ? 4 * nb : nb); i += 256) bins[i] = 0u;
    if (tid < RK_BN) glab[tid] = n0 + tid < G ? roc.glab[n0 + tid] : 0;
    if (tid < BM) {
        const bool ok = m0 + tid < Q;
        const i64 e = ok && roc.excl ? roc.excl[m0 + tid] : -1;
        qlab[tid] = ok ? roc.qlab[m0 + tid] : 0;
        qex[tid] = e >= 0 ? e - roc.idx_offset : -1;
    }
    __syncthreads();
    unsigned* mine = bins + (sub ? wave * nb : 0);
#pragma unroll
    for (int j = 0; j < 2; ++j) {
        const int c = wn * 64 + j * 32 + lr;
        const i64 col = n0 + c;
        if (col < G) {
            const float gs = ginv ? ginv[col] : 1.0f;
            const i64 gl = glab[c];
#pragma unroll
            for (int i = 0; i < MT; ++i)
#pragma unroll
                for (int r = 0; r < 16; ++r) {
                    const int row = wm * MT * 32 + i * 32 + (r & 3) + 8 * (r >> 2) + 4 * (lane >> 5);
                    if (m0 + row < Q && col != qex[row])
                        atomicAdd(&mine[roc_bin(acc[i][j][r] * gs, tab, roc)], qlab[row] == gl ? 0x10000u : 1u);
                }
        }
    }
    __syncthreads();
    for (int b = tid; b < nb; b += 256) {
        unsigned u = bins[b];
        if (sub) u += bins[nb + b] + bins[2 * nb + b] + bins[3 * nb + b];
        if (u >> 16) atomicAdd(&roc.hist[b], (unsigned long long)(u >> 16));
        if (u & 0xffffu) atomicAdd(&roc.hist[nb + b], (unsigned long long)(u & 0xffffu));
    }
}

constexpr int FK_RANGE = -2;

struct RangeArgs {
    RankFilter f;
    float thr;
    unsigned long long* cursor;
    unsigned long long* raw;
    i64 cap;
    i64* tstart;
    int* tcount;
};

constexpr size_t RANGE_EPI_BYTES = (size_t)128 * 4 * sizeof(unsigned) + (size_t)128 * sizeof(int) + 2 * sizeof(i64) +
                                   (size_t)(RK_BN + 2 * 128) * sizeof(i64);

template <int MT, int FK, bool FILT>
__device__ __forceinline__ void cos_gemm_epilogue(f32x16 (&acc)[MT][2], float* smem, const float* __restrict__ ginv, float*, int Q,
                                                  i64 G, int, float*, int*, int, int ntx, i64 n0, int m0, const RangeArgs& rg) {
    static_assert(FK == FK_RANGE && !FILT, "the range twins pass FK = FK_RANGE, FILT = false");
    constexpr int BM = 64 * MT;
    const int tid = threadIdx.x, lane = tid & 63, wave = tid >> 6;
    const int wm = wave >> 1, wn = wave & 1, lr = lane & 31;
    unsigned* mask = reinterpret_cast<unsigned*>(smem);
    int* rpre = reinterpret_cast<int*>(mask + 128 * 4);
    unsigned long long* sbase = reinterpret_cast<unsigned long long*>(rpre + 128);
    i64* glab = reinterpret_cast<i64*>(sbase + 2);
    i64* qlab = glab + RK_BN;
    i64* qex = qlab + 128;
    const bool filt = rg.f.mode != MI355_LABEL_ANY || rg.f.excl;
    if (filt) {
        if (tid < RK_BN) glab[tid] = rg.f.mode != MI355_LABEL_ANY && n0 + tid < G ? rg.f.glab[n0 + tid] : 0;
        if (tid < BM) {
            i64 l = 0, e = -1;
            if (m0 + tid < Q) query_filter(rg.f, m0 + tid, l, e);
            qlab[tid] = l;
            qex[tid] = e;
        }
        __syncthreads();
    }
#pragma unroll
    for (int j = 0; j < 2; ++j) {
        const int c = wn * 64 + j * 32 + lr;
        const i64 col = n0 + c;
        const float gs = (ginv && col < G) ? ginv[col] : 1.0f;
        const i64 gl = filt ? glab[c] : 0;
#pragma unroll
        for (int i = 0; i < MT; ++i)
#pragma unroll
            for (int r = 0; r < 16; ++r) {
                const int row = wm * MT * 32 + i * 32 + (r & 3) + 8 * (r >> 2) + 4 * (lane >> 5);
                bool hit = col < G && m0 + row < Q && acc[i][j][r] * gs >= rg.thr;
                if (filt) hit = hit && eligible(rg.f.mode, qlab[row], gl, qex[row], col);
                const unsigned long long b = __ballot(hit);
                if (lane == 0) {
                    mask[row * 4 + wn * 2 + j] = (unsigned)b;
                    mask[(row + 4) * 4 + wn * 2 + j] = (unsigned)(b >> 32);
                }
            }
    }
    __syncthreads();
    int cnt = 0, incl = 0;
    if (tid < BM) {
        cnt = __popc(mask[tid * 4]) + __popc(mask[tid * 4 + 1]) + __popc(mask[tid * 4 + 2]) + __popc(mask[tid * 4 + 3]);
        incl = cnt;
#pragma unroll
        for (int d = 1; d < 64; d <<= 1) {
            const int v = __shfl_up(incl, d, 64);
            if (lane >= d) incl += v;
        }
        if (tid == 63) sbase[1] = (unsigned long long)incl;
    }
    __syncthreads();
    if (tid < BM) {
        if (tid >= 64) incl += (int)sbase[1];
        rpre[tid] = incl - cnt;
        if (tid == BM - 1) sbase[0] = incl > 0 ? atomicAdd(rg.cursor, (unsigned long long)incl) : 0ull;
    }
    __syncthreads();
    const unsigned long long base = sbase[0];
    const int tile = (int)(n0 / RK_BN);
    if (tid < BM && m0 + tid < Q) {
        const size_t t = (size_t)(m0 + tid) * ntx + tile;
        rg.tstart[t] = (i64)base + rpre[tid];
        rg.tcount[t] = cnt;
    }
    const int total = rpre[BM - 1] + __popc(mask[(BM - 1) * 4]) + __popc(mask[(BM - 1) * 4 + 1]) + __popc(mask[(BM - 1) * 4 + 2]) +
                      __popc(mask[(BM - 1) * 4 + 3]);
    if (total == 0 || (i64)base + total > rg.cap) return;
#pragma unroll
    for (int j = 0; j < 2; ++j) {
        const int c = wn * 64 + j * 32 + lr, w = wn * 2 + j;
        const i64 col = n0 + c;
        const float gs = (ginv && col < G) ? ginv[col] : 1.0f;
#pragma unroll
        for (int i = 0; i < MT; ++i)
#pragma unroll
            for (int r = 0; r < 16; ++r) {
                const int row = wm * MT * 32 + i * 32 + (r & 3) + 8 * (r >> 2) + 4 * (lane >> 5);
                const unsigned* m = mask + row * 4;
                if ((m[w] >> lr) & 1u) {
                    int before = __popc(m[w] & ((1u << lr) - 1u));
                    for (int u = 0; u < w; ++u) before += __popc(m[u]);
                    const float s = acc[i][j][r] * gs;
                    rg.raw[base + rpre[row] + before] = (unsigned long long)(unsigned)col |
                                                        ((unsigned long long)__float_as_uint(s) << 32);
                }
            }
    }
}

__device__ __forceinline__ float row_inv_norm(const float* __restrict__ x, int dim, float eps, int vec, int lane) {
    float ss = 0.f;
    if (vec) {
        const f32x4* x4 = reinterpret_cast<const f32x4*>(x);
        for (int i = lane; i < dim / 4; i += 64) {
            f32x4 v = x4[i];
            ss += v.x * v.x + v.y * v.y + v.z * v.z + v.w * v.w;
        }
    } else {
        for (int i = lane; i < dim; i += 64) ss += x[i] * x[i];
    }
    ss = wave_sum(ss);
    return 1.0f / fmaxf(sqrtf(ss), eps);
}

__device__ __forceinline__ _Float16 scaled_f16(float x, float r) {
    float p = x * r;
    asm volatile("" : "+v"(p));
    return (_Float16)p;
}

typedef _Float16 f16x4_t __attribute__((ext_vector_type(4)));
template <bool VEC, bool OF16>
__device__ __forceinline__ void normalize_row_store(float* x, _Float16* y, int dim, int ld, float eps, int lane) {
    const int nu = VEC ? dim / 4 : dim;
    const float r = row_inv_norm(x, dim, eps, VEC ? 1 : 0, lane);
    if constexpr (!OF16) {
        if constexpr (VEC) {
            f32x4* x4 = reinterpret_cast<f32x4*>(x);
            for (int i = lane; i < nu; i += 64) {
                f32x4 v = x4[i];
                v.x *= r; v.y *= r; v.z *= r; v.w *= r;
                x4[i] = v;
            }
        } else {
            for (int i = lane; i < dim; i += 64) x[i] = x[i] * r;
        }
    } else {
        if constexpr (VEC) {
            const f32x4* x4 = reinterpret_cast<const f32x4*>(x);
            for (int i = lane; i < ld / 4; i += 64) {
                f16x4_t h = {(_Float16)0.f, (_Float16)0.f, (_Float16)0.f, (_Float16)0.f};
                if (i < nu) {
                    const f32x4 v = x4[i];
                    h = (f16x4_t){scaled_f16(v.x, r), scaled_f16(v.y, r), scaled_f16(v.z, r), scaled_f16(v.w, r)};
                }
                reinterpret_cast<f16x4_t*>(y)[i] = h;
            }
        } else {
            for (int i = lane; i < ld; i += 64) y[i] = i < dim ? scaled_f16(x[i], r) : (_Float16)0.f;
        }
    }
}

static inline int vec_ok(const void* p, int dim) { return (dim % 4 == 0) && (((uintptr_t)p & 15) == 0); }

constexpr int SMALL_K = 8;
constexpr int LARGE_K = 1024;

size_t topk_ws_bytes(i64 Q, i64 G, int k);
int topk_select(const float* vals, const i64* idxs, i64 Q, i64 rowlen, i64 in_stride, int k, i64 idx_offset, float* out_val,
                i64* out_idx, void* ws, size_t ws_bytes, hipStream_t st, const int* idxs32 = nullptr,
                const RankFilter* filt = nullptr);
RankFilter filter_from(const RankFilter& f, i64 q0);
int make_filter(const mi355_rank_filter* f, i64 idx_offset, const char* who, RankFilter* out);
void set_rank_path(int path);
bool fused_select(i64 Q, i64 G, int k);
i64 query_block(i64 Q, i64 G, int k);
int kernel_slots(const void* fn, size_t lds, int* cache, int* slots_out);
int whole_round_tiles(int ntx, int ny, int slots);


struct TileArgs {
    const void* qry;
    const void* gal;
    const float* ginv;
    float* S;
    int Q;
    i64 G;
    int D;
    int k;
    float* cand_val;
    int* cand_idx;
    const RankFilter* filt;
    const RocArgs* roc;
    const RangeArgs* rng;
};

constexpr size_t EPI_TILE_BYTES = (size_t)64 * (RK_BN + 4) * sizeof(float);

template <class F, int MT, int FK, bool FILT>
int tile_slots(size_t lds, int* slots_out) {
    static int slots[MI355_MAX_DEVICES] = {0};
    return kernel_slots((const void*)F::template kernel<MT, FK, FILT>(), lds, slots, slots_out);
}

template <class F, int MT, int FK, bool FILT>
int launch_tiles(const TileArgs& a, hipStream_t st, int x0 = 0) {
    constexpr size_t stage = F::template stage_bytes<MT>();
    static_assert(!FILT || stage >= EPI_TILE_BYTES + FILT_LABELS_BYTES, "the filtered epilogue would grow the GEMM's LDS");
    static_assert(FK != FK_RANGE || stage >= RANGE_EPI_BYTES, "the range epilogue would grow the GEMM's LDS");
    constexpr size_t lds = FK == FK_ROC ? (ROC_EPI_BYTES > stage ? ROC_EPI_BYTES : stage)
                                        : FK > 0 && EPI_TILE_BYTES > stage ? EPI_TILE_BYTES : stage;
    int slots = 0;
    if (int e = tile_slots<F, MT, FK, FILT>(lds, &slots)) return e;
    const int ntx = cdiv(a.G, RK_BN), ny = cdiv(a.Q, 64 * MT);
    const int x1 = MT == 2 ? whole_round_tiles(ntx, ny, slots) : ntx;
    if (x1 > x0) {
        F::template launch<MT, FK, FILT>(dim3((unsigned)(x1 - x0) * (unsigned)ny), lds, st, a, x0, ntx, x1 - x0, ny);
        MI355_LAUNCH_CHECK();
    }
    if constexpr (MT == 2) {
        if (x1 < ntx) return launch_tiles<F, 1, FK, FILT>(a, st, x1);
    }
    return OK;
}

template <class F, int MT, bool FILT>
int launch_fk(const TileArgs& a, hipStream_t st) {
    if (a.k <= 1) return launch_tiles<F, MT, 1, FILT>(a, st);
    if (a.k <= 2) return launch_tiles<F, MT, 2, FILT>(a, st);
    if (a.k <= 4) return launch_tiles<F, MT, 4, FILT>(a, st);
    return launch_tiles<F, MT, 8, FILT>(a, st);
}
template <class F, int MT>
int launch_mt(const TileArgs& a, hipStream_t st) {
    if constexpr (F::ROC) {
        if (a.roc) return launch_tiles<F, MT, FK_ROC, false>(a, st);
    }
    if constexpr (F::RANGE) {
        if (a.rng) return launch_tiles<F, MT, FK_RANGE, false>(a, st);
    }
    if constexpr (F::SLAB) {
        if (!a.cand_val) {
            TileArgs s = a;
            s.k = 0;
            return launch_tiles<F, MT, 0, false>(s, st);
        }
    }
    if constexpr (F::FILTERED) {
        if (a.filt) return launch_fk<F, MT, true>(a, st);
    }
    return launch_fk<F, MT, false>(a, st);
}
template <class F>
int cos_gemm_tiles(const TileArgs& a, hipStream_t st) {
    return a.Q > 64 ? launch_mt<F, 2>(a, st) : launch_mt<F, 1>(a, st);
}

int roc_check_thresholds(const double* thr, int T, const char* who, RocArgs* a);
int roc_check_pairs(const int64_t* query_labels, const int64_t* gallery_labels, const int64_t* exclude, int64_t idx_offset,
                    const double* thresholds_dev, int64_t* hist, const char* who, RocArgs* a);
RocArgs roc_from(const RocArgs& a, i64 q0);
i64 roc_query_block(i64 Q, i64 G);

struct RankWs {
    float* qn; void* qs; float* ginv; float* S; float* cand_val; int* cand_idx; void* topk; size_t topk_bytes; size_t total;
};
RankWs carve(void* ws, i64 Q, i64 G, int D, int k, size_t (*planes_bytes)(i64, int), bool need_ginv, bool need_S = true);
int normalize_search(const float* queries, i64 Q, const float* gallery, i64 G, int dim, float eps, const RankWs& w,
                     hipStream_t st);

template <class Score>
int search_blocks(const float* queries, const float* gallery_to_norm, i64 Q, i64 G, int dim, int k, float eps, i64 idx_offset,
                  const RankFilter* filt, float* out_val, i64* out_idx, const RankWs& w, hipStream_t st, const char* slab_range,
                  Score&& score) {
    if (int e = normalize_search(queries, Q, gallery_to_norm, G, dim, eps, w, st)) return e;
    const bool fused = fused_select(Q, G, k);
    const i64 qb = query_block(Q, G, k), rowlen = fused ? cdiv(G, RK_BN) * (i64)k : G;
    for (i64 q0 = 0; q0 < Q; q0 += qb) {
        const i64 qn = (Q - q0 < qb) ? Q - q0 : qb;
        const RankFilter fb = filt ? filter_from(*filt, q0) : RankFilter{};
        const RankFilter* f = filt ? &fb : nullptr;
        if (int e = score(q0, qn, f)) return e;
        if (!fused && k > SMALL_K) set_rank_path(mi355_rank_last_path() | MI355_RANK_PATH_BITONIC);
        RoctxRange range(fused ? "rank/merge candidates" : slab_range);
        if (int e = topk_select(fused ? w.cand_val : w.S, nullptr, qn, rowlen, rowlen, k, idx_offset, out_val + q0 * k,
                                out_idx + q0 * k, w.topk, w.topk_bytes, st, w.cand_idx, f))
            return e;
    }
    return OK;
}

struct RangeWs {
    i64* offsets; unsigned long long* cursor; RankWs w; i64* tstart; int* tcount; i64* rowcnt; size_t total;
};
RangeWs range_carve(void* ws, i64 Q, i64 G, int D, size_t (*planes_bytes)(i64, int), bool need_ginv);
i64 range_query_block(i64 Q, i64 G);
int range_check(const void* queries, i64 Q, const void* gallery, i64 G, int dim, double threshold,
                const mi355_rank_filter* filter, i64 idx_offset, void* candidates, i64 capacity, const int64_t* nnz,
                const char* who, RankFilter* f);
int range_empty(const RangeWs& w, i64 Q, int64_t* nnz, hipStream_t st);
int range_compact_block(const RangeWs& w, i64 q0, i64 qn, i64 G, i64 off, const unsigned long long* raw,
                        unsigned long long* canon, hipStream_t st);

template <class Score>
int range_blocks(i64 Q, i64 G, const RankFilter& filt, double threshold, void* candidates, i64 capacity, int64_t* nnz,
                 const RangeWs& w, hipStream_t st, Score&& score) {
    unsigned long long* raw = (unsigned long long*)candidates;
    unsigned long long* canon = raw ? raw + capacity : nullptr;
    MI355_CHECK_HIP(hipMemsetAsync(w.offsets, 0, sizeof(i64), st));
    const i64 qb = range_query_block(Q, G);
    i64 off = 0;
    bool fits = true;
    for (i64 q0 = 0; q0 < Q; q0 += qb) {
        const i64 qn = (Q - q0 < qb) ? Q - q0 : qb;
        MI355_CHECK_HIP(hipMemsetAsync(w.cursor, 0, sizeof(unsigned long long), st));
        const RangeArgs a{filter_from(filt, q0), roc_ceil_f32(threshold), w.cursor, raw, fits ? capacity : 0, w.tstart, w.tcount};
        if (int e = score(q0, qn, a)) return e;
        unsigned long long n = 0;
        MI355_CHECK_HIP(hipMemcpyAsync(&n, w.cursor, sizeof(n), hipMemcpyDeviceToHost, st));
        MI355_CHECK_HIP(hipStreamSynchronize(st));
        fits = fits && off + (i64)n <= capacity;
        if (fits) {
            RoctxRange range("range/compact");
            if (int e = range_compact_block(w, q0, qn, G, off, raw, canon, st)) return e;
        }
        off += (i64)n;
    }
    *nnz = off;
    return OK;
}

}
```

imageretrievalresearch_amd/csrc/rank_gemm_split.inc:

```
    constexpr int BM = 64 * MT;
    constexpr int BK = 16;
    constexpr int A_STAGE = (BM / 32) * 3 * 512;
    constexpr int A_PIECES = (BM / 32) * 3;
    constexpr int B_STAGE = RK_BN * BK;
    extern __shared__ __attribute__((aligned(16))) float smem[];
    bf16_t* As = reinterpret_cast<bf16_t*>(smem);
    constexpr int A_RING = MT == 1 ? 3 : 2;
    float* Bs = smem + (A_RING * A_STAGE * 2) / 4;

    const int tid = threadIdx.x, lane = tid & 63, wave = tid >> 6;
    const int wm = wave >> 1, wn = wave & 1;
    int bx, by;
    rank_tile_of((int)blockIdx.x, xtiles, ny, bx, by);
    const i64 n0 = (i64)(bx + x0) * RK_BN;
    const int m0 = by * BM;
    const int swave = __builtin_amdgcn_readfirstlane(wave);

    const float* b_row[2];
    int b_k[2];
    bool b_ok[2];
#pragma unroll
    for (int i = 0; i < 2; ++i) {
        const int r = (swave * 2 + i) * 16 + (lane >> 2);
        const int c = (lane & 3) ^ ((r >> 2) & 3);
        b_ok[i] = n0 + r < G;
        b_row[i] = Gal + (b_ok[i] ? (n0 + r) * D : 0);
        b_k[i] = c * 4;
    }
    auto dma_b = [&](int stage, int k0) {
#pragma unroll
        for (int i = 0; i < 2; ++i) {
            const bool ok = b_ok[i] && k0 + b_k[i] < D;
            glds16(reinterpret_cast<const bf16_t*>(ok ? b_row[i] + k0 + b_k[i] : zeros),
                   reinterpret_cast<bf16_t*>(Bs + stage * B_STAGE + (swave * 2 + i) * 256));
        }
    };
    const bf16_t* a_src = Qs + (size_t)(m0 / 32) * n_steps * 3 * 512 + lane * 8;
    const bf16_t* a_piece[(A_PIECES + 3) / 4];
#pragma unroll
    for (int i = 0; i < (A_PIECES + 3) / 4; ++i) {
        const int piece = (swave + 4 * i) % A_PIECES;
        a_piece[i] = a_src + ((size_t)((piece / 3) * n_steps) * 3 + piece % 3) * 512;
    }
    auto dma_a = [&](int buf, int t) {
#pragma unroll
        for (int i = 0; i < (A_PIECES + 3) / 4; ++i) {
            const int piece = swave + 4 * i;
            if (A_PIECES % 4 == 0 || i < A_PIECES / 4 || swave < A_PIECES % 4)
                glds16(a_piece[i] + (size_t)t * 3 * 512, As + buf * A_STAGE + piece * 512);
        }
    };

    f32x16 acc[MT][2];
#pragma unroll
    for (int i = 0; i < MT; ++i)
#pragma unroll
        for (int j = 0; j < 2; ++j)
#pragma unroll
            for (int e = 0; e < 16; ++e) acc[i][j][e] = 0.f;

    const int lr = lane & 31;
    int b_off[2][2];
#pragma unroll
    for (int j = 0; j < 2; ++j) {
        const int r = wn * 64 + j * 32 + lr, sw = (r >> 2) & 3, c0 = (lane >> 5) * 2;
        b_off[j][0] = r * BK + ((c0 ^ sw) << 2);
        b_off[j][1] = r * BK + (((c0 + 1) ^ sw) << 2);
    }
    auto compute = [&](int abuf, int bstage) {
        const bf16_t* a = As + abuf * A_STAGE + (wm * MT * 3) * 512 + lane * 8;
        const float* b = Bs + bstage * B_STAGE;
        bf16x8 af[MT][3];
        u32x4 bh[2], bm[2], bl[2];
        f32x4 v0[2], v1[2];
#pragma unroll
        for (int j = 0; j < 2; ++j) {
            v0[j] = *reinterpret_cast<const f32x4*>(b + b_off[j][0]);
            v1[j] = *reinterpret_cast<const f32x4*>(b + b_off[j][1]);
        }
#pragma unroll
        for (int i = 0; i < MT; ++i)
#pragma unroll
            for (int p = 0; p < 3; ++p) af[i][p] = *reinterpret_cast<const bf16x8*>(a + (i * 3 + p) * 512);
        split3(v0[0], v1[0], bh[0], bm[0], bl[0]);
        auto products = [&](int j) {
            const bf16x8 gh = *reinterpret_cast<const bf16x8*>(&bh[j]);
            const bf16x8 gm = *reinterpret_cast<const bf16x8*>(&bm[j]);
            const bf16x8 gl = *reinterpret_cast<const bf16x8*>(&bl[j]);
#pragma unroll
            for (int i = 0; i < MT; ++i) {
                acc[i][j] = __builtin_amdgcn_mfma_f32_32x32x16_bf16(af[i][2], gh, acc[i][j], 0, 0, 0);
                acc[i][j] = __builtin_amdgcn_mfma_f32_32x32x16_bf16(af[i][0], gl, acc[i][j], 0, 0, 0);
                acc[i][j] = __builtin_amdgcn_mfma_f32_32x32x16_bf16(af[i][1], gm, acc[i][j], 0, 0, 0);
                acc[i][j] = __builtin_amdgcn_mfma_f32_32x32x16_bf16(af[i][1], gh, acc[i][j], 0, 0, 0);
                acc[i][j] = __builtin_amdgcn_mfma_f32_32x32x16_bf16(af[i][0], gm, acc[i][j], 0, 0, 0);
                acc[i][j] = __builtin_amdgcn_mfma_f32_32x32x16_bf16(af[i][0], gh, acc[i][j], 0, 0, 0);
            }
        };
        split3(v0[1], v1[1], bh[1], bm[1], bl[1]);
        products(0);
#pragma unroll
        for (int g = 0; g < 6 * MT; ++g) {
            __builtin_amdgcn_sched_group_barrier(0x008, 1, 0);
            __builtin_amdgcn_sched_group_barrier(0x002, 4, 0);
        }
        products(1);
    };

    dma_a(0, 0);
    if (A_RING == 3 && n_steps > 1) dma_a(1, 1);
    dma_b(0, 0);
    dma_b(1, BK);
    __syncthreads();

    int bs_cur = 0, bs_far = 2;
    for (int t = 0; t < n_steps; ++t) {
        if constexpr (A_RING == 2) {
            if (t + 1 < n_steps) dma_a((t & 1) ^ 1, t + 1);
        } else {
            if (t + 2 < n_steps) dma_a(bs_far, t + 2);
        }
        __builtin_amdgcn_sched_barrier(0);
        dma_b(bs_far, (t + 2) * BK);
        __builtin_amdgcn_sched_barrier(0);
        compute(A_RING == 2 ? (t & 1) : bs_cur, bs_cur);
        if constexpr (A_RING == 2) {
            asm volatile("s_waitcnt vmcnt(2)" ::: "memory");
        } else {
            if (t + 2 >= n_steps) asm volatile("s_waitcnt vmcnt(2)" ::: "memory");
            else if (swave < A_PIECES % 4) asm volatile("s_waitcnt vmcnt(4)" ::: "memory");
            else asm volatile("s_waitcnt vmcnt(3)" ::: "memory");
        }
        asm volatile("s_waitcnt lgkmcnt(0)" ::: "memory");
        __builtin_amdgcn_s_barrier();
        asm volatile("" ::: "memory");
        bs_cur = bs_cur == 2 ? 0 : bs_cur + 1;
        bs_far = bs_far == 2 ? 0 : bs_far + 1;
    }
    __syncthreads();
    cos_gemm_epilogue<MT, FK, FILT>(acc, smem, ginv, S, Q, G, k, cand_val, cand_idx, x0, ntx, n0, m0, flt);
```

imageretrievalresearch_amd/rank.py:

```python
from __future__ import annotations

import ctypes
from typing import NamedTuple

import numpy as np
import torch

from ._lib import (DTYPE_F16, DTYPE_F32, LABEL_ANY, LABEL_DIFFERENT, LABEL_SAME, MI355Error, RankFilter, check, lib,
                   require_cuda, stream_ptr)

_EPS = 1e-6


def _f32c(t: torch.Tensor, name: str) -> torch.Tensor:
    require_cuda(t, name)
    if t.dtype != torch.float32:
        t = t.float()
    return t.contiguous()


class _Workspace:

    def __init__(self):
        self.buf = {}

    def get(self, device, nbytes: int) -> torch.Tensor:
        device = torch.device(device)
        stream = torch.cuda.current_stream(device)
        key = (device, stream.cuda_stream)
        b = self.buf.get(key)
        if b is None or b.numel() < nbytes:
            if b is not None:
                b.record_stream(stream)
            with torch.cuda.stream(stream):
                b = torch.empty(int(nbytes), dtype=torch.uint8, device=device)
            self.buf[key] = b
        return b


_ws = _Workspace()


def synth_fill(n: int, seed: int, kind: int, device, offset: int = 0) -> torch.Tensor:
    out = torch.empty(int(n), dtype=torch.float32, device=device)
    require_cuda(out, "synth_fill output")
    with torch.cuda.device(out.device):
        check(lib().mi355_synth_fill(out.data_ptr(), int(n), int(seed), int(offset), int(kind),
                                     stream_ptr(out.device)))
    return out


def l2_normalize_rows(x: torch.Tensor, eps: float = _EPS, out: torch.Tensor | None = None) -> torch.Tensor:
    x = _f32c(x, "x")
    if x.dim() != 2:
        raise MI355Error(f"l2_normalize_rows expects (rows, dim), got {tuple(x.shape)}")
    if out is None:
        out = torch.empty_like(x)
    with torch.cuda.device(x.device):
        check(lib().mi355_l2_normalize_rows(x.data_ptr(), out.data_ptr(), x.shape[0], x.shape[1], eps,
                                            stream_ptr(x.device)))
    return out


def _check_qg(q, g):
    if len(q.shape) != 2 or len(g.shape) != 2:
        raise MI355Error(f"expected (Q,D) queries and (G,D) gallery, got {tuple(q.shape)} and {tuple(g.shape)}")
    if q.shape[1] != g.shape[1]:
        raise MI355Error(f"embedding dims differ: {q.shape[1]} vs {g.shape[1]}")
    if q.device != g.device:
        raise MI355Error(f"queries on {q.device} but gallery on {g.device}")


def _row_stride(t: torch.Tensor) -> int:
    return int(t.stride(0)) if t.shape[0] > 1 else int(t.shape[1])


class _Rows:

    def __init__(self, buf, rows: int, dim: int, normalized: bool, planes: torch.Tensor | None = None):
        self.buf, self.rows, self.dim, self.normalized, self.planes = buf, int(rows), int(dim), bool(normalized), planes
        self.shape = (self.rows, self.dim)
        self.dtype = torch.float32 if buf is None else buf.dtype
        self.device = planes.device if buf is None else buf.device
        self.ld = self.dim if buf is None else _row_stride(buf)

    @classmethod
    def of(cls, gallery, normalized: bool = False) -> "_Rows":
        if isinstance(gallery, cls):
            return gallery
        g = _f32c(gallery, "gallery")
        if g.dim() != 2:
            raise MI355Error(f"expected a (G,D) gallery, got {tuple(g.shape)}")
        return cls(g, g.shape[0], g.shape[1], normalized)

    @property
    def data(self) -> torch.Tensor:
        return self.buf[: self.rows, : self.dim]

    def c_args(self):
        norm = () if self.dtype == torch.float16 else (int(self.normalized),)
        return (self.buf.data_ptr(), self.rows, self.dim) + norm


_ENTRIES = {
    torch.float32: {"topk": ("mi355_rank_topk", "mi355_rank_topk_filtered", "mi355_rank_workspace_bytes"),
                    "range": ("mi355_cosine_range", "mi355_range_workspace_bytes"),
                    "roc": ("mi355_roc_pairs_hist", "mi355_roc_pairs_workspace_bytes")},
    torch.float16: {"topk": ("mi355_rank_topk_f16", "mi355_rank_topk_f16_filtered", "mi355_rank_f16_workspace_bytes"),
                    "range": ("mi355_cosine_range_f16", "mi355_range_f16_workspace_bytes"),
                    "roc": ("mi355_roc_pairs_hist_f16", "mi355_roc_pairs_f16_workspace_bytes")},
}


def cosine_scores(queries: torch.Tensor, gallery: torch.Tensor, eps: float = _EPS,
                  gallery_is_normalized: bool = False) -> torch.Tensor:
    q, g = _f32c(queries, "queries"), _f32c(gallery, "gallery")
    _check_qg(q, g)
    Q, D = q.shape
    G = g.shape[0]
    out = torch.empty((Q, G), dtype=torch.float32, device=q.device)
    if Q == 0 or G == 0:
        return out
    nbytes = lib().mi355_rank_workspace_bytes(Q, G, D, 0)
    ws = _ws.get(q.device, nbytes)
    with torch.cuda.device(q.device):
        check(lib().mi355_cosine_scores(q.data_ptr(), Q, g.data_ptr(), G, D, int(gallery_is_normalized), eps,
                                        out.data_ptr(), ws.data_ptr(), ws.numel(), stream_ptr(q.device)))
    return out


_LABEL_MODES = {None: LABEL_ANY, "same": LABEL_SAME, "different": LABEL_DIFFERENT}


def _int64_on(t, name: str, n: int, device) -> torch.Tensor:
    if not torch.is_tensor(t):
        raise MI355Error(f"{name} must be a tensor")
    require_cuda(t, name)
    if t.device != torch.device(device):
        raise MI355Error(f"{name} is on {t.device} but the search runs on {device}")
    if t.dtype.is_floating_point or t.dtype.is_complex or t.dtype == torch.bool:
        raise MI355Error(f"{name} must hold integers, got {t.dtype}")
    if t.dim() != 1 or t.shape[0] != n:
        raise MI355Error(f"{name} must have shape ({n},), got {tuple(t.shape)}")
    return t.to(torch.int64).contiguous()


def _need_labels(labels, rows: int, what: str, source: str) -> torch.Tensor:
    if labels is None:
        raise MI355Error(f"{what} needs {source}")
    if labels.shape[0] != rows:
        raise MI355Error(f"{what}: {labels.shape[0]} labels for {rows} rows ({source})")
    return labels


def _rank_filter(Q: int, G: int, device, query_labels, gallery_labels, label_filter, exclude):
    if label_filter not in _LABEL_MODES:
        raise MI355Error(f'label_filter must be None, "same" or "different", got {label_filter!r}')
    if label_filter is None and exclude is None:
        return None
    keep = []
    f = RankFilter()
    f.label_mode = _LABEL_MODES[label_filter]
    if label_filter is not None:
        if query_labels is None or gallery_labels is None:
            raise MI355Error(f'label_filter="{label_filter}" needs query_labels and gallery labels')
        ql = _int64_on(query_labels, "query_labels", Q, device)
        gl = _int64_on(gallery_labels, "gallery_labels", G, device)
        keep += [ql, gl]
        f.query_labels, f.gallery_labels = ql.data_ptr(), gl.data_ptr()
    if exclude is not None:
        ex = _int64_on(exclude, "exclude", Q, device)
        keep.append(ex)
        f.exclude = ex.data_ptr()
    return f, keep


def cosine_topk(queries: torch.Tensor, gallery: torch.Tensor, k: int, eps: float = _EPS,
                gallery_is_normalized: bool = False, idx_offset: int = 0, query_labels: torch.Tensor | None = None,
                gallery_labels: torch.Tensor | None = None, label_filter: str | None = None,
                exclude: torch.Tensor | None = None):
    return _topk(queries, _Rows.of(gallery, gallery_is_normalized), k, eps, idx_offset, query_labels, gallery_labels,
                 label_filter, exclude)


def _topk(queries: torch.Tensor, rows: _Rows, k: int, eps: float = _EPS, idx_offset: int = 0, query_labels=None,
          gallery_labels=None, label_filter=None, exclude=None):
    q = _f32c(queries, "queries")
    _check_qg(q, rows)
    Q, G = q.shape[0], rows.rows
    if k > G or k < 1:
        raise MI355Error(f"selected index k out of range: k={k}, gallery rows={G}")
    filt = _rank_filter(Q, G, q.device, query_labels, gallery_labels, label_filter, exclude)
    vals = torch.empty((Q, k), dtype=torch.float32, device=q.device)
    idx = torch.empty((Q, k), dtype=torch.int64, device=q.device)
    if Q == 0:
        return vals, idx
    on_planes = filt is None and rows.planes is not None and PreparedGallery.supports(Q, k)
    if not on_planes and rows.buf is None:
        raise MI355Error(f"prepared search needs k <= 8 and more than 4 queries (got k={k}, Q={Q}): use cosine_topk on the rows")
    L = lib()
    plain, filtered, ws_bytes = _ENTRIES[torch.float32 if on_planes else rows.dtype]["topk"]
    ws = _ws.get(q.device, getattr(L, ws_bytes)(Q, G, rows.dim, k))
    out = (vals.data_ptr(), idx.data_ptr(), ws.data_ptr(), ws.numel(), stream_ptr(q.device))
    with torch.cuda.device(q.device):
        if on_planes:
            check(L.mi355_rank_topk_prepared(q.data_ptr(), Q, rows.planes.data_ptr(), G, rows.dim, k, eps, int(idx_offset), *out))
        elif filt is None:
            check(getattr(L, plain)(q.data_ptr(), Q, *rows.c_args(), k, eps, int(idx_offset), *out))
        else:
            check(getattr(L, filtered)(q.data_ptr(), Q, *rows.c_args(), k, eps, int(idx_offset), filt[0], *out))
    return vals, idx


class PreparedGallery:

    def __init__(self, gallery_normalized: torch.Tensor):
        g = _f32c(gallery_normalized, "gallery")
        if g.dim() != 2 or g.shape[0] < 1:
            raise MI355Error(f"a prepared gallery needs (G, D) rows with G >= 1, got {tuple(g.shape)}")
        self.rows, self.dim, self.device = int(g.shape[0]), int(g.shape[1]), g.device
        nbytes = lib().mi355_gallery_planes_bytes(self.rows, self.dim)
        self.planes = torch.empty((nbytes,), dtype=torch.uint8, device=g.device)
        with torch.cuda.device(g.device):
            check(lib().mi355_gallery_prepare(g.data_ptr(), self.rows, self.dim, self.planes.data_ptr(), nbytes,
                                              stream_ptr(g.device)))

    @staticmethod
    def supports(Q: int, k: int) -> bool:
        return Q > 4 and 1 <= k <= 8

    def search(self, queries: torch.Tensor, k: int, eps: float = _EPS, idx_offset: int = 0):
        return _topk(queries, _Rows(None, self.rows, self.dim, True, self.planes), k, eps, idx_offset)


def topk(scores: torch.Tensor, k: int, idx_offset: int = 0):
    squeeze = scores.dim() == 1
    s = _f32c(scores.unsqueeze(0) if squeeze else scores, "scores")
    if s.dim() != 2:
        raise MI355Error(f"topk expects a 1-D or 2-D tensor, got {tuple(scores.shape)}")
    Q, G = s.shape
    if k > G or k < 1:
        raise MI355Error(f"selected index k out of range: k={k}, row length={G}")
    vals = torch.empty((Q, k), dtype=torch.float32, device=s.device)
    idx = torch.empty((Q, k), dtype=torch.int64, device=s.device)
    if Q:
        nbytes = lib().mi355_rank_workspace_bytes(Q, G, 0, k)
        ws = _ws.get(s.device, nbytes)
        with torch.cuda.device(s.device):
            check(lib().mi355_topk_rows(s.data_ptr(), Q, G, k, int(idx_offset), vals.data_ptr(), idx.data_ptr(),
                                        ws.data_ptr(), ws.numel(), stream_ptr(s.device)))
    return (vals[0], idx[0]) if squeeze else (vals, idx)


def merge_topk(cand_val: torch.Tensor, cand_idx: torch.Tensor, k: int):
    v = _f32c(cand_val, "cand_val")
    require_cuda(cand_idx, "cand_idx")
    i = cand_idx.to(torch.int64).contiguous()
    if v.shape != i.shape or v.dim() != 2:
        raise MI355Error(f"merge_topk expects matching (Q, ncand) tensors, got {tuple(v.shape)} / {tuple(i.shape)}")
    Q, n = v.shape
    if k > n or k < 1:
        raise MI355Error(f"selected index k out of range: k={k}, candidates={n}")
    vals = torch.empty((Q, k), dtype=torch.float32, device=v.device)
    idx = torch.empty((Q, k), dtype=torch.int64, device=v.device)
    if Q:
        nbytes = lib().mi355_rank_workspace_bytes(Q, n, 0, k)
        ws = _ws.get(v.device, nbytes)
        with torch.cuda.device(v.device):
            check(lib().mi355_merge_topk(v.data_ptr(), i.data_ptr(), Q, n, k, vals.data_ptr(), idx.data_ptr(),
                                         ws.data_ptr(), ws.numel(), stream_ptr(v.device)))
    return vals, idx


def pack_candidates(vals: "torch.Tensor | None", idx: "torch.Tensor | None", Q: int, k: int, device) -> torch.Tensor:
    packed = torch.empty((Q, k, 2), dtype=torch.int32, device=device)
    kk = 0 if vals is None else vals.shape[1]
    if Q:
        v = _f32c(vals, "vals") if kk else None
        i = idx.to(torch.int64).contiguous() if kk else None
        with torch.cuda.device(packed.device):
            check(lib().mi355_pack_candidates(v.data_ptr() if kk else None, i.data_ptr() if kk else None, Q, kk, k,
                                              packed.data_ptr(), stream_ptr(packed.device)))
    return packed


def merge_packed_topk(packed: torch.Tensor, shard_offsets: torch.Tensor, k: int):
    require_cuda(packed, "packed candidates")
    if packed.dtype != torch.int32 or packed.dim() != 4 or packed.shape[3] != 2 or packed.shape[2] != k:
        raise MI355Error(f"merge_packed_topk expects (world, Q, {k}, 2) int32, got {packed.dtype} {tuple(packed.shape)}")
    packed = packed.contiguous()
    world, Q = packed.shape[0], packed.shape[1]
    off = shard_offsets.to(packed.device, torch.int64).contiguous().view(-1)
    if off.numel() != world:
        raise MI355Error(f"merge_packed_topk: {off.numel()} shard offsets for {world} shards")
    vals = torch.empty((Q, k), dtype=torch.float32, device=packed.device)
    idx = torch.empty((Q, k), dtype=torch.int64, device=packed.device)
    if Q:
        ws = _ws.get(packed.device, lib().mi355_merge_packed_workspace_bytes(Q, world, k))
        with torch.cuda.device(packed.device):
            check(lib().mi355_merge_packed_topk(packed.data_ptr(), off.data_ptr(), world, Q, k, vals.data_ptr(),
                                                idx.data_ptr(), ws.data_ptr(), ws.numel(), stream_ptr(packed.device)))
    return vals, idx


def pair_cosine(a: torch.Tensor, b: torch.Tensor, eps: float = _EPS) -> torch.Tensor:
    a, b = _f32c(a, "a"), _f32c(b, "b")
    if a.shape != b.shape or a.dim() != 2:
        raise MI355Error(f"pair_cosine expects two (B,D) tensors, got {tuple(a.shape)} / {tuple(b.shape)}")
    out = torch.empty((a.shape[0],), dtype=torch.float32, device=a.device)
    if a.shape[0]:
        with torch.cuda.device(a.device):
            check(lib().mi355_pair_cosine(a.data_ptr(), b.data_ptr(), a.shape[0], a.shape[1], eps, out.data_ptr(),
                                          stream_ptr(a.device)))
    return out


class CosineSimilarity(torch.nn.Module):

    def __init__(self, dim: int = 1, eps: float = _EPS):
        super().__init__()
        if dim != 1:
            raise MI355Error("only dim=1 (the reference's setting) is implemented")
        self.dim, self.eps = dim, eps

    def forward(self, x1: torch.Tensor, x2: torch.Tensor) -> torch.Tensor:
        if x1.dim() != 2 or x2.dim() != 2:
            raise MI355Error(f"CosineSimilarity expects 2-D inputs, got {tuple(x1.shape)} / {tuple(x2.shape)}")
        if x1.shape == x2.shape and x1.shape[0] != 1:
            return pair_cosine(x1, x2, self.eps)
        if x1.shape[0] == 1:
            return cosine_scores(x1, x2, self.eps)[0]
        if x2.shape[0] == 1:
            return cosine_scores(x2, x1, self.eps)[0]
        raise MI355Error(f"unsupported broadcast {tuple(x1.shape)} vs {tuple(x2.shape)}")


class ContrastiveLoss(torch.nn.Module):

    def __init__(self, margin):
        super().__init__()
        self.margin, self.eps = margin, 1e-9

    def forward(self, fm1, fm2, label, mean=True):
        a, b = _f32c(fm1, "fm1"), _f32c(fm2, "fm2")
        if a.shape != b.shape or a.dim() != 2:
            raise MI355Error(f"ContrastiveLoss expects two (B,D) tensors, got {tuple(a.shape)} / {tuple(b.shape)}")
        out = torch.empty((), dtype=torch.float32, device=a.device)
        with torch.cuda.device(a.device):
            check(lib().mi355_contrastive_loss(a.data_ptr(), b.data_ptr(), a.shape[0], a.shape[1], float(label),
                                               float(self.margin), int(bool(mean)), out.data_ptr(), None,
                                               stream_ptr(a.device)))
        return out


class CosineEmbeddingLoss(torch.nn.Module):

    def __init__(self, margin: float = 0.0, reduction: str = "mean"):
        super().__init__()
        if reduction not in ("mean", "sum"):
            raise MI355Error("reduction must be 'mean' or 'sum'")
        self.margin, self.reduction = margin, reduction

    def forward(self, input1, input2, target):
        a, b = _f32c(input1, "input1"), _f32c(input2, "input2")
        if a.shape != b.shape or a.dim() != 2:
            raise MI355Error(f"CosineEmbeddingLoss expects two (B,D) tensors, got {tuple(a.shape)} / {tuple(b.shape)}")
        t = float(target.reshape(-1)[0].item()) if torch.is_tensor(target) else float(target)
        if torch.is_tensor(target) and target.numel() != 1:
            raise MI355Error("only a scalar (broadcast) target is supported, as in the reference")
        out = torch.empty((), dtype=torch.float32, device=a.device)
        with torch.cuda.device(a.device):
            check(lib().mi355_cosine_embedding_loss(a.data_ptr(), b.data_ptr(), a.shape[0], a.shape[1], t,
                                                    float(self.margin), int(self.reduction == "mean"), out.data_ptr(),
                                                    stream_ptr(a.device)))
        return out


def validation_metrics(fm_ims, fm_poss, fm_negs, clss, margin: float = 0.5, k: int = 3):
    cel = CosineEmbeddingLoss(margin)
    loss_pos = cel(fm_ims, fm_poss, 1.0)
    loss_neg = cel(fm_ims, fm_negs, -1.0)
    vals, inds = cosine_topk(fm_ims, fm_poss, min(k, fm_poss.shape[0]))
    counts = hit_counts(inds, clss, clss)
    n = fm_ims.shape[0]
    return {"loss_cos_poss": loss_pos, "loss_cos_negs": loss_neg, "loss_cos": loss_pos + loss_neg,
            "cos_sims": pair_cosine(fm_ims, fm_poss).mean(), "cos_unsims": pair_cosine(fm_ims, fm_negs).mean(),
            "top1": counts[0].float() / n, "top3": counts[1].float() / n, "topk_vals": vals, "topk_inds": inds}


def hit_counts(idx: torch.Tensor, query_cls: torch.Tensor, gallery_cls: torch.Tensor):
    require_cuda(idx, "idx")
    idx = idx.to(torch.int64).contiguous()
    qc = query_cls.to(idx.device, torch.int64).contiguous()
    gc = gallery_cls.to(idx.device, torch.int64).contiguous()
    if idx.dim() != 2 or qc.shape[0] != idx.shape[0]:
        raise MI355Error("hit_counts expects idx (Q,k) and query_cls (Q,)")
    counts = torch.zeros(2, dtype=torch.int64, device=idx.device)
    if idx.shape[0]:
        with torch.cuda.device(idx.device):
            check(lib().mi355_hit_counts(idx.data_ptr(), idx.shape[0], idx.shape[1], qc.data_ptr(), gc.data_ptr(),
                                         gc.numel(), counts.data_ptr(), stream_ptr(idx.device)))
    return counts


def distinct_class_topn(idx: torch.Tensor, val: torch.Tensor, gallery_cls: torch.Tensor, n: int = 3):
    require_cuda(idx, "idx")
    idx = idx.to(torch.int64).contiguous()
    val = _f32c(val, "val")
    gc = gallery_cls.to(idx.device, torch.int64).contiguous()
    Q, k = idx.shape
    oc = torch.empty((Q, n), dtype=torch.int64, device=idx.device)
    oi = torch.empty((Q, n), dtype=torch.int64, device=idx.device)
    ov = torch.empty((Q, n), dtype=torch.float32, device=idx.device)
    if Q:
        with torch.cuda.device(idx.device):
            check(lib().mi355_distinct_class_topn(idx.data_ptr(), val.data_ptr(), Q, k, gc.data_ptr(), gc.numel(), n,
                                                  oc.data_ptr(), oi.data_ptr(), ov.data_ptr(),
                                                  stream_ptr(idx.device)))
    return oc, oi, ov


def _score_boost(score, eps, alpha, threshold, mode):
    s = _f32c(score, "score")
    out = torch.empty_like(s)
    if s.numel():
        with torch.cuda.device(s.device):
            check(lib().mi355_score_boost(s.data_ptr(), s.numel(), float(eps), float(alpha), float(threshold), mode,
                                          out.data_ptr(), stream_ptr(s.device)))
    return out


# ... 491 lines not shown
```

include/mi355_retrieval.h:

```cpp
#ifndef MI355_RETRIEVAL_H
#define MI355_RETRIEVAL_H

#include <stddef.h>
#include <stdint.h>

#ifdef __cplusplus
extern "C" {
#endif

#define MI355_ABI_VERSION 3

int mi355_abi_version(void);
const char* mi355_last_error(void);
int mi355_device_count(void);

int mi355_synth_fill(float* out, int64_t n, uint64_t seed, int64_t offset, int kind, void* stream);


int mi355_l2_normalize_rows(const float* in, float* out, int64_t rows, int dim, float eps, void* stream);

size_t mi355_rank_workspace_bytes(int64_t Q, int64_t G, int dim, int k);

int mi355_rank_topk(const float* queries, int64_t Q, const float* gallery, int64_t G, int dim,
                    int gallery_is_normalized, int k, float eps, int64_t idx_offset,
                    float* out_val, int64_t* out_idx, void* workspace, size_t workspace_bytes,
                    void* stream);

int mi355_cosine_scores(const float* queries, int64_t Q, const float* gallery, int64_t G, int dim,
                        int gallery_is_normalized, float eps, float* out, void* workspace,
                        size_t workspace_bytes, void* stream);

size_t mi355_gallery_planes_bytes(int64_t G, int dim);
int mi355_gallery_prepare(const float* gallery_normalized, int64_t G, int dim, void* planes, size_t planes_bytes, void* stream);
int mi355_rank_topk_prepared(const float* queries, int64_t Q, const void* gallery_planes, int64_t G, int dim, int k, float eps,
                             int64_t idx_offset, float* out_val, int64_t* out_idx, void* workspace, size_t workspace_bytes,
                             void* stream);

size_t mi355_gallery_f16_bytes(int64_t G, int dim);
int mi355_gallery_to_f16(const float* rows, int64_t G, int dim, int rows_are_normalized, float eps, void* out, size_t out_bytes,
                         void* stream);
size_t mi355_rank_f16_workspace_bytes(int64_t Q, int64_t G, int dim, int k);
int mi355_rank_topk_f16(const float* queries, int64_t Q, const void* gallery_f16, int64_t G, int dim, int k, float eps,
                        int64_t idx_offset, float* out_val, int64_t* out_idx, void* workspace, size_t workspace_bytes,
                        void* stream);

enum { MI355_LABEL_ANY = 0, MI355_LABEL_SAME = 1, MI355_LABEL_DIFFERENT = 2 };
typedef struct mi355_rank_filter {
    const int64_t* query_labels;
    const int64_t* gallery_labels;
    int label_mode;
    const int64_t* exclude;
} mi355_rank_filter;
int mi355_rank_topk_filtered(const float* queries, int64_t Q, const float* gallery, int64_t G, int dim,
                             int gallery_is_normalized, int k, float eps, int64_t idx_offset, const mi355_rank_filter* filter,
                             float* out_val, int64_t* out_idx, void* workspace, size_t workspace_bytes, void* stream);
int mi355_rank_topk_f16_filtered(const float* queries, int64_t Q, const void* gallery_f16, int64_t G, int dim, int k, float eps,
                                 int64_t idx_offset, const mi355_rank_filter* filter, float* out_val, int64_t* out_idx,
                                 void* workspace, size_t workspace_bytes, void* stream);
enum {
    MI355_RANK_PATH_GEMV = 1,
    MI355_RANK_PATH_SPLIT = 2,
    MI355_RANK_PATH_EXACT_F32 = 3,
    MI355_RANK_PATH_PREPARED = 4,
    MI355_RANK_PATH_F16_GEMM = 5,
    MI355_RANK_PATH_F16_GEMV = 6,
    MI355_RANK_PATH_FUSED = 0x100,
    MI355_RANK_PATH_BITONIC = 0x200
};
int mi355_rank_last_path(void);

#define MI355_ROC_MAX_THRESHOLDS 4096
size_t mi355_roc_pairs_workspace_bytes(int64_t Q, int64_t G, int dim);
int mi355_roc_pairs_hist(const float* queries, int64_t Q, const float* gallery, int64_t G, int dim, int gallery_is_normalized,
                         float eps, const int64_t* query_labels, const int64_t* gallery_labels, const int64_t* exclude,
                         int64_t idx_offset, const double* thresholds, const double* thresholds_dev, int T, int64_t* hist,
                         void* workspace, size_t workspace_bytes, void* stream);
size_t mi355_roc_pairs_f16_workspace_bytes(int64_t Q, int64_t G, int dim);
int mi355_roc_pairs_hist_f16(const float* queries, int64_t Q, const void* gallery_f16, int64_t G, int dim, float eps,
                             const int64_t* query_labels, const int64_t* gallery_labels, const int64_t* exclude, int64_t idx_offset,
                             const double* thresholds, const double* thresholds_dev, int T, int64_t* hist, void* workspace,
                             size_t workspace_bytes, void* stream);
int mi355_roc_scores_hist(const void* scores, int scores_f64, int64_t n, const int8_t* actual, const double* thresholds,
                          const double* thresholds_dev, int T, int64_t* hist, void* stream);
int mi355_roc_finalize(const int64_t* hist, int T, int64_t* counts, int64_t* totals, double* rates, double* auc, void* stream);

size_t mi355_range_workspace_bytes(int64_t Q, int64_t G, int dim);
int mi355_cosine_range(const float* queries, int64_t Q, const float* gallery, int64_t G, int dim, int gallery_is_normalized,
                       float eps, double threshold, int64_t idx_offset, const mi355_rank_filter* filter, void* candidates,
                       int64_t capacity, int64_t* nnz, void* workspace, size_t workspace_bytes, void* stream);
size_t mi355_range_f16_workspace_bytes(int64_t Q, int64_t G, int dim);
int mi355_cosine_range_f16(const float* queries, int64_t Q, const void* gallery_f16, int64_t G, int dim, float eps, double threshold,
                           int64_t idx_offset, const mi355_rank_filter* filter, void* candidates, int64_t capacity, int64_t* nnz,
                           void* workspace, size_t workspace_bytes, void* stream);
int mi355_range_compact(const void* candidates, int64_t capacity, int64_t Q, int64_t nnz, int64_t idx_offset, const void* workspace,
                        size_t workspace_bytes, int64_t* offsets, int64_t* indices, float* scores, void* stream);

enum { MI355_DTYPE_F32 = 0, MI355_DTYPE_F16 = 1 };
size_t mi355_expand_workspace_bytes(int64_t R, int dim, int out_dtype);
int mi355_expand_rows(const void* base, int base_dtype, int64_t base_ld, int normalize_base, const void* gallery,
                      int gallery_dtype, int64_t gallery_rows, int64_t gallery_ld, int dim, const float* vals,
                      const int64_t* idx, int64_t R, int n, int64_t idx_offset, float alpha, float eps, void* out,
                      int out_dtype, int64_t out_ld, void* workspace, size_t workspace_bytes, void* stream);

#define MI355_KR_MAX_K1 32
int mi355_kr_sets(const int64_t* lists, const float* list_vals, const float* tau, int64_t R, int k1, const int64_t* graph,
                  int64_t G, int64_t* offsets, int32_t* cols, int64_t cols_capacity, void* stream);
int mi355_kr_weights(const void* rows, int rows_dtype, int64_t rows_ld, int64_t R, const void* gallery, int gallery_dtype,
                     int64_t G, int64_t gallery_ld, int dim, const int64_t* offsets, const int32_t* cols, int64_t nnz,
                     float* vals, void* stream);
int mi355_kr_local_qe(const int64_t* lists, int64_t R, int k1, int k2, const int64_t* own_offsets, const int32_t* own_cols,
                      const float* own_vals, int64_t own_nnz, const int64_t* gallery_offsets, const int32_t* gallery_cols,
                      const float* gallery_vals, int64_t gallery_nnz, int64_t G, int64_t* out_offsets, int32_t* out_cols,
                      float* out_vals, int64_t out_capacity, void* stream);
int mi355_kr_score(const int64_t* query_offsets, const int32_t* query_cols, const float* query_vals, int64_t query_nnz, int64_t Q,
                   const int64_t* gallery_offsets, const int32_t* gallery_cols, const float* gallery_vals, int64_t gallery_nnz,
                   int64_t G, const float* shortlist_vals, const int64_t* shortlist_idx, int K, float lam, float* out,
                   void* stream);

size_t mi355_moments_workspace_bytes(int64_t R, int dim);
int mi355_embedding_moments(const void* rows, int rows_dtype, int64_t R, int64_t ld, int dim, int normalize_rows, float eps,
                            int accumulate, double* sum, double* outer, void* workspace, size_t workspace_bytes, void* stream);

size_t mi355_whiten_workspace_bytes(int64_t R, int dim_in, int dim_out, int out_dtype);
int mi355_whiten_rows(const void* x, int x_dtype, int64_t R, int64_t x_ld, int dim_in, int normalize_input, float eps,
                      const float* matrix, const float* bias, int dim_out, int normalize_output, void* out, int out_dtype,
                      int64_t out_ld, void* workspace, size_t workspace_bytes, void* stream);

int mi355_clear_pads(float* val, int64_t* idx, int64_t n, int64_t lo, int64_t hi, void* stream);

int mi355_retrieval_metrics(const int64_t* idx, int64_t Q, int k, const int64_t* query_cls, const int64_t* gallery_cls,
                            int64_t G, const int64_t* R, double* per_query, void* stream);

int mi355_topk_rows(const float* scores, int64_t Q, int64_t G, int k, int64_t idx_offset,
                    float* out_val, int64_t* out_idx, void* workspace, size_t workspace_bytes,
                    void* stream);

int mi355_merge_topk(const float* cand_val, const int64_t* cand_idx, int64_t Q, int ncand, int k,
                     float* out_val, int64_t* out_idx, void* workspace, size_t workspace_bytes,
                     void* stream);

int mi355_pack_candidates(const float* val, const int64_t* idx, int64_t Q, int kk, int k, int32_t* packed, void* stream);
size_t mi355_merge_packed_workspace_bytes(int64_t Q, int world, int k);
int mi355_merge_packed_topk(const int32_t* packed, const int64_t* shard_offsets, int world, int64_t Q, int k,
                            float* out_val, int64_t* out_idx, void* workspace, size_t workspace_bytes, void* stream);

int mi355_pair_cosine(const float* a, const float* b, int64_t rows, int dim, float eps, float* out,
                      void* stream);

int mi355_contrastive_loss(const float* fm1, const float* fm2, int64_t rows, int dim, float label,
                           float margin, int mean, float* out, float* per_row, void* stream);

int mi355_cosine_embedding_loss(const float* x1, const float* x2, int64_t rows, int dim, float target, float margin,
                                int mean, float* out, void* stream);

int mi355_hit_counts(const int64_t* idx, int64_t Q, int k, const int64_t* query_cls,
                     const int64_t* gallery_cls, int64_t G, int64_t* counts, void* stream);

int mi355_distinct_class_topn(const int64_t* idx, const float* val, int64_t Q, int k,
                              const int64_t* gallery_cls, int64_t G, int n, int64_t* out_cls, int64_t* out_idx,
                              float* out_val, void* stream);

typedef struct mi355_model* mi355_model_t;

int mi355_model_create(const char* name, int num_classes, mi355_model_t* out);
void mi355_model_destroy(mi355_model_t m);

int mi355_model_num_tensors(mi355_model_t m);
int mi355_model_tensor_info(mi355_model_t m, int i, const char** name, int* ndim, int64_t shape[4],
                            int* kind);
int mi355_model_feature_dim(mi355_model_t m);
int mi355_model_num_classes(mi355_model_t m);

int mi355_model_set_tensor(mi355_model_t m, const char* name, const float* host_data, int64_t numel);

int mi355_model_pack(mi355_model_t m, void* stream);

int mi355_model_forward_features(mi355_model_t m, const float* x, int B, int H, int W, float* out,
                                 float* pooled_out, void* stream);
int mi355_model_forward(mi355_model_t m, const float* x, int B, int H, int W, float* out,
                        float* pooled_out, void* stream);

int mi355_model_forward_u8(mi355_model_t m, const unsigned char* images, int B, int h, int w, int fill,
                           const float* mean, const float* stdv, const float* conv_input_w, int features_only,
                           float* out, float* pooled_out, void* stream);

size_t mi355_resize_batch_workspace_bytes(const int64_t* desc_host, int B, int out_h, int out_w, int pad);
int mi355_resize_batch_u8(const unsigned char* pixels, int64_t pixels_bytes, const int64_t* desc_host, const int64_t* desc_dev,
                          int B, int out_h, int out_w, int pad, int fill, unsigned char* out, void* workspace,
                          size_t workspace_bytes, void* stream);

size_t mi355_model_forward_images_workspace_bytes(const int64_t* desc_host, int B, int transform, int out_size);
int mi355_model_forward_images(mi355_model_t m, const unsigned char* pixels, int64_t pixels_bytes, const int64_t* desc_host,
                               const int64_t* desc_dev, int B, int transform, int out_size, int fill, const float* mean,
                               const float* stdv, const float* conv_input_w, int features_only, float* out, float* pooled_out,
                               void* workspace, size_t workspace_bytes, void* stream);

int mi355_model_enable_taps(mi355_model_t m, int enable);
int mi355_model_read_tap(mi355_model_t m, const char* tap_name, float* out, int64_t out_numel,
                         int64_t shape[4], void* stream);

int mi355_model_run_between_taps(mi355_model_t m, const char* from_tap, const char* to_tap, const float* x, int B,
                                 int C, int h, int w, void* stream);

int mi355_model_traffic(mi355_model_t m, int B, int H, int W, double* act_bytes, double* weight_bytes,
                        double* macs);

int mi355_model_traffic_kinds(mi355_model_t m, int B, int H, int W, double* bytes_by_kind, double* macs_by_kind, int n);

int mi355_model_set_option(mi355_model_t m, const char* key, int64_t value);
int mi355_model_profile_read(mi355_model_t m, double* ms_by_kind, int64_t* launches_by_kind, int n);

int mi355_model_profile_ops(mi355_model_t m, int B, int H, int W, int max_ops, double* avg_ms, double* bytes,
                            int* kinds, char* labels, int label_stride);

int mi355_model_block_stamps(mi355_model_t m, double* out, int max_ops);

int mi355_pool_linear(const float* fm, int B, int C, int HW, const float* weight, const float* bias, int N, float* out,
                      float* pooled_out, void* stream);

int mi355_gemm_bf16(const void* A, const void* W, const float* bias, void* out, int M, int N, int K, int ldw, int act,
                    void* stream);

typedef struct mi355_gemm_ex_args {
    const void* A; int lda;
    const void* W; int ldw;
    const float* bias;
    const void* res; int ldr; int res_n;
    const float* gate; int gate_ld; int rows_per_img; int a_relu6;
    void* out; int ldo; int out_f32;
    int M, N, K, act;
    int64_t M_sel;
    void* splitk_ws; size_t splitk_ws_bytes;
    const float* ln_stats; const float* ln_colsum;
} mi355_gemm_ex_args;

enum {
    MI355_GEMM_PATH_TILE_M64_BK32 = 1,
    MI355_GEMM_PATH_TILE_M64_BK64 = 2,
    MI355_GEMM_PATH_TILE = 3,
    MI355_GEMM_PATH_BIG = 4,
    MI355_GEMM_PATH_BIG_KTAIL = 5,
    MI355_GEMM_PATH_BIG32 = 6,
    MI355_GEMM_PATH_BIG32_KTAIL = 7,
    MI355_GEMM_PATH_BIG_GATED = 8,
    MI355_GEMM_PATH_BIG_GATED_KTAIL = 9,
    MI355_GEMM_PATH_STREAM = 10,
    MI355_GEMM_PATH_PROJ = 11,
    MI355_GEMM_PATH_SPLITK = 12,
    MI355_GEMM_PATH_WIDE = 13
};
#define MI355_GEMM_PATH_KIND(p) ((p) & 0xff)
#define MI355_GEMM_PATH_NT(p) (((p) >> 8) & 0xff)

int mi355_gemm_bf16_ex(const mi355_gemm_ex_args* args, int* path, void* stream);

typedef struct mi355_dwconv_ex_args {
    const void* in; const void* w; const float* bias; void* out;
    int B, H, W, C, k, stride, act, choice;
    const float* se_w1; const float* se_b1; const float* se_w2t; const float* se_b2;
    int rd, act1;
    float* gate;
    float* squeeze;
} mi355_dwconv_ex_args;

enum { MI355_DW_CHOICE_AUTO = 0, MI355_DW_CHOICE_DIRECT = 1, MI355_DW_CHOICE_TILED = 2, MI355_DW_CHOICE_MFMA = 3 };

enum {
    MI355_DW_PATH_DIRECT = 1,
    MI355_DW_PATH_LDS3 = 2,
    MI355_DW_PATH_TILED = 3,
    MI355_DW_PATH_SE_SMALL = 1,
    MI355_DW_PATH_SE_FULL = 2
};
#define MI355_DW_PATH(kind, ks, s, arg, se) ((kind) | (ks) << 8 | (s) << 12 | (arg) << 16 | (se) << 24)
#define MI355_DW_PATH_KIND(p) ((p) & 0xff)
#define MI355_DW_PATH_KS(p) (((p) >> 8) & 0xf)
#define MI355_DW_PATH_S(p) (((p) >> 12) & 0xf)
#define MI355_DW_PATH_ARG(p) (((p) >> 16) & 0xff)
#define MI355_DW_PATH_SE(p) (((p) >> 24) & 0xff)

int mi355_dwconv_se_ex(const mi355_dwconv_ex_args* args, int* path, void* stream);

int mi355_window_attention(const void* qkv, const float* bias_table, void* out, int B, int res, int C, int heads, int shift,
                           void* stream);

int mi355_window_attention_ws(const void* qkv, const float* bias_table, void* out, int B, int res, int C, int heads, int window,
                              int shift, void* stream);

int mi355_swin_layernorm(const void* in, const float* gamma, const float* beta, void* out, int64_t rows, int C, int merge, int gh, int gw,
                         int stats, float eps, void* stream);

int mi355_swin_patch_embed(const float* x, const unsigned char* images, const int64_t* desc_dev, int b0, int B, int H, int h, int w,
                           int fill, const float* mean, const float* stdv, const float* weight, const float* bias, const float* gamma,
                           const float* beta, int embed, float eps, void* out, void* stream);

int mi355_swin_ln_token_mean(const void* in, const float* gamma, const float* beta, float* pooled, void* pooled_bf16, int B, int L, int C,
                             float eps, void* stream);

int mi355_square_pad_normalize(const unsigned char* img, int h, int w, int fill, const float* mean, const float* stdv,
                               float* out, void* stream);

int mi355_resize_bilinear_u8(const unsigned char* img, int h, int w, unsigned char* out, int out_h, int out_w,
                             unsigned char* tmp, void* stream);

int mi355_score_boost(const float* scores, int64_t n, float eps, float alpha, float threshold, int mode, float* out,
                      void* stream);

int mi355_conv_input_silu(const float* x, const float* w, int B, int H, int W, float* out, void* stream);

#ifdef __cplusplus
}
#endif
#endif
```

Baseline: 60650.

## Add screened top-k: bf16 screen pass then exact rescoring of candidate rows

Adds a screened ranking path. A bf16 MFMA screen GEMM computes approximate scores and gallery norms, per-row error bounds mark every gallery row that could still enter the top-k, and an exact split GEMM then rescoring runs only over the compacted row list, with a gated full fallback when the list overflows. The aim is to skip most exact fp32-gallery GEMM work over the 100k gallery. In exchange it adds several extra kernels, atomics on a bitmap and more workspace, and the path only pays off when the screen prunes well.

```diff
diff --git a/imageretrievalresearch_amd/_lib.py b/imageretrievalresearch_amd/_lib.py
--- a/imageretrievalresearch_amd/_lib.py
+++ b/imageretrievalresearch_amd/_lib.py
@@ -62,6 +62,8 @@
     "mi355_rank_topk_f16_filtered": (C.c_int, [vp, C.c_int64, vp, C.c_int64, C.c_int, C.c_int, C.c_float, C.c_int64,
                                                C.POINTER(RankFilter), vp, vp, vp, C.c_size_t, vp]),
     "mi355_rank_last_path": (C.c_int, []),
+    "mi355_rank_screen_stats": (C.c_int, [vp, vp, vp]),
+    "mi355_rank_screen_scores": (C.c_int, [vp, C.c_int64, vp, C.c_int64, C.c_int, C.c_int, C.c_float, vp, vp, vp, C.c_size_t, vp]),
     "mi355_expand_workspace_bytes": (C.c_size_t, [C.c_int64, C.c_int, C.c_int]),
     "mi355_expand_rows": (C.c_int, [vp, C.c_int, C.c_int64, C.c_int, vp, C.c_int, C.c_int64, C.c_int64, C.c_int, vp, vp,
                                     C.c_int64, C.c_int, C.c_int64, C.c_float, C.c_float, vp, C.c_int, C.c_int64, vp,
diff --git a/imageretrievalresearch_amd/csrc/rank.hip b/imageretrievalresearch_amd/csrc/rank.hip
--- a/imageretrievalresearch_amd/csrc/rank.hip
+++ b/imageretrievalresearch_amd/csrc/rank.hip
@@ -130,6 +130,7 @@
                                                            const float* __restrict__ zeros, int xtiles, int ny) {
     constexpr bool FILT = false;
     const RankFilter flt{};
+    const auto split_row = [](i64 i) { return i; };
 #include "rank_gemm_split.inc"
 }
 template <int MT, int FK>
@@ -140,6 +141,7 @@
                                                                 int xtiles, int ny, RankFilter flt) {
     constexpr bool FILT = true;
     float* const S = nullptr;
+    const auto split_row = [](i64 i) { return i; };
 #include "rank_gemm_split.inc"
 }
 template <int MT>
@@ -153,6 +155,7 @@
     const int k = 0;
     float* const cand_val = nullptr;
     int* const cand_idx = nullptr;
+    const auto split_row = [](i64 i) { return i; };
 #include "rank_gemm_split.inc"
 }
 template <int MT>
@@ -166,7 +169,60 @@
     const int k = 0;
     float* const cand_val = nullptr;
     int* const cand_idx = nullptr;
+    const auto split_row = [](i64 i) { return i; };
 #include "rank_gemm_split.inc"
+}
+
+template <int MT, int FK>
+__global__ __launch_bounds__(256, 3) void k_cos_gemm_split_list(const bf16_t* __restrict__ Qs, const float* __restrict__ Gal,
+                                                                const float* __restrict__ ginv, int Q, int D, int k,
+                                                                float* __restrict__ cand_val, int* __restrict__ cand_idx, int x0,
+                                                                int ntx, int n_steps, const float* __restrict__ zeros, int xtiles,
+                                                                int ny, const unsigned* __restrict__ cur,
+                                                                const int* __restrict__ row_list) {
+    constexpr bool FILT = false;
+    const RankFilter flt{};
+    float* const S = nullptr;
+    const i64 G = cur[0];
+    {
+        int tx, ty;
+        rank_tile_of((int)blockIdx.x, xtiles, ny, tx, ty);
+        if ((i64)(tx + x0) * RK_BN >= G) {
+            for (int i = threadIdx.x; i < 64 * MT * k; i += 256) {
+                const int row = ty * 64 * MT + i / k;
+                if (row < Q) {
+                    const size_t o = ((size_t)row * ntx + (size_t)(tx + x0)) * k + i % k;
+                    cand_val[o] = NEG_INF;
+                    cand_idx[o] = IDX32_PAD;
+                }
+            }
+            return;
+        }
+    }
+    const auto split_row = [&](i64 i) { return (i64)row_list[i]; };
+#include "rank_gemm_split.inc"
+}
+template <int MT, int FK>
+__global__ __launch_bounds__(256, 3) void k_cos_gemm_split_gated(const bf16_t* __restrict__ Qs, const float* __restrict__ Gal,
+                                                                 const float* __restrict__ ginv, int Q, i64 G, int D, int k,
+                                                                 float* __restrict__ cand_val, int* __restrict__ cand_idx, int x0,
+                                                                 int ntx, int n_steps, const float* __restrict__ zeros, int xtiles,
+                                                                 int ny, const unsigned* __restrict__ cur) {
+    constexpr bool FILT = false;
+    const RankFilter flt{};
+    float* const S = nullptr;
+    if (cur[1] == 0u) return;
+    const auto split_row = [](i64 i) { return i; };
+#include "rank_gemm_split.inc"
+}
+
+template <int MT, int FK>
+__global__ __launch_bounds__(256, 2) void k_cos_gemm_screen(const bf16_t* __restrict__ Qs, const float* __restrict__ Gal,
+                                                            const float* __restrict__ ginv, float* __restrict__ S, int Q, i64 G,
+                                                            int D, int k, float* __restrict__ cand_val, int* __restrict__ cand_idx,
+                                                            int x0, int ntx, int n_steps, const float* __restrict__ zeros,
+                                                            int xtiles, int ny, float* __restrict__ gn2) {
+#include "rank_gemm_screen.inc"
 }
 
 template <int MT, int FK>
@@ -345,6 +401,17 @@
     constexpr bool FILT = true;
     const i64* const idxs = nullptr;
     const int* const idxs32 = nullptr;
+#include "rank_topk_small.inc"
+}
+
+template <int K>
+__global__ __launch_bounds__(256) void k_topk_small_gated(const float* __restrict__ vals, const i64* __restrict__ idxs,
+                                                          const int* __restrict__ idxs32, i64 rowlen, i64 in_stride,
+                                                          i64 chunk_len, int k, i64 idx_offset, float* __restrict__ ov,
+                                                          i64* __restrict__ oi, const unsigned* __restrict__ gate) {
+    constexpr bool FILT = false;
+    const RankFilter flt{};
+    if (gate[1] == 0u) return;
 #include "rank_topk_small.inc"
 }
 
@@ -561,8 +628,12 @@
 
 template <int K>
 static void launch_small(const float* v, const i64* ix, const int* ix32, i64 rowlen, i64 in_stride, i64 chunk_len, int k,
-                         i64 off, float* ov, i64* oi, i64 nchunk, i64 Q, hipStream_t st, const RankFilter* filt) {
-    if (filt)
+                         i64 off, float* ov, i64* oi, i64 nchunk, i64 Q, hipStream_t st, const RankFilter* filt,
+                         const unsigned* gate) {
+    if (gate)
+        hipLaunchKernelGGL((k_topk_small_gated<K>), dim3((unsigned)nchunk, (unsigned)Q), dim3(256), 0, st, v, ix, ix32, rowlen,
+                           in_stride, chunk_len, k, off, ov, oi, gate);
+    else if (filt)
         hipLaunchKernelGGL((k_topk_small_filt<K>), dim3((unsigned)nchunk, (unsigned)Q), dim3(256), 0, st, v, rowlen, in_stride,
                            chunk_len, k, off, ov, oi, *filt);
     else
@@ -570,11 +641,12 @@
                            in_stride, chunk_len, k, off, ov, oi);
 }
 static void dispatch_small(const float* v, const i64* ix, const int* ix32, i64 rowlen, i64 in_stride, i64 chunk_len, int k,
-                           i64 off, float* ov, i64* oi, i64 nchunk, i64 Q, hipStream_t st, const RankFilter* filt) {
-    if (k <= 1) launch_small<1>(v, ix, ix32, rowlen, in_stride, chunk_len, k, off, ov, oi, nchunk, Q, st, filt);
-    else if (k <= 2) launch_small<2>(v, ix, ix32, rowlen, in_stride, chunk_len, k, off, ov, oi, nchunk, Q, st, filt);
-    else if (k <= 4) launch_small<4>(v, ix, ix32, rowlen, in_stride, chunk_len, k, off, ov, oi, nchunk, Q, st, filt);
-    else launch_small<8>(v, ix, ix32, rowlen, in_stride, chunk_len, k, off, ov, oi, nchunk, Q, st, filt);
+                           i64 off, float* ov, i64* oi, i64 nchunk, i64 Q, hipStream_t st, const RankFilter* filt,
+                           const unsigned* gate) {
+    if (k <= 1) launch_small<1>(v, ix, ix32, rowlen, in_stride, chunk_len, k, off, ov, oi, nchunk, Q, st, filt, gate);
+    else if (k <= 2) launch_small<2>(v, ix, ix32, rowlen, in_stride, chunk_len, k, off, ov, oi, nchunk, Q, st, filt, gate);
+    else if (k <= 4) launch_small<4>(v, ix, ix32, rowlen, in_stride, chunk_len, k, off, ov, oi, nchunk, Q, st, filt, gate);
+    else launch_small<8>(v, ix, ix32, rowlen, in_stride, chunk_len, k, off, ov, oi, nchunk, Q, st, filt, gate);
 }
 
 static thread_local int g_rank_path = 0;
@@ -603,7 +675,8 @@
 
 int topk_select(const float* vals, const i64* idxs, i64 Q, i64 rowlen, i64 in_stride, int k, i64 idx_offset,
                 float* out_val, i64* out_idx, void* ws, size_t ws_bytes, hipStream_t st, const int* idxs32,
-                const RankFilter* filt) {
+                const RankFilter* filt, const unsigned* gate) {
+    MI355_REQUIRE(!gate || (k <= SMALL_K && !filt), "top-k: a gated selection needs k <= %d and no filter", SMALL_K);
     MI355_REQUIRE(k >= 1 && k <= LARGE_K, "top-k: k=%d outside [1,%d]", k, LARGE_K);
     MI355_REQUIRE(k <= rowlen, "top-k: k=%d exceeds row length %lld", k, (long long)rowlen);
     MI355_REQUIRE(!idxs32 || k <= SMALL_K, "top-k: int32 candidate lists need k <= %d", SMALL_K);
@@ -637,7 +710,7 @@
             const bool last = (nchunk == 1);
             float* ovp = last ? out_val + qs * k : cv[cur];
             i64* oip = last ? out_idx + qs * k : ci[cur];
-            if (small) dispatch_small(v, ix, ix32, len, stride, chunk, k, off, ovp, oip, nchunk, qn, st, f1);
+            if (small) dispatch_small(v, ix, ix32, len, stride, chunk, k, off, ovp, oip, nchunk, qn, st, f1, gate);
             else if (f1) hipLaunchKernelGGL(k_topk_bitonic_filt, dim3((unsigned)nchunk, (unsigned)qn), dim3(256), 0, st, v, len,
                                             stride, k, off, ovp, oip, *f1);
             else hipLaunchKernelGGL(k_topk_bitonic, dim3((unsigned)nchunk, (unsigned)qn), dim3(256), 0, st, v, ix,
@@ -681,13 +754,14 @@
     return OK;
 }
 
-RankWs carve(void* ws, i64 Q, i64 G, int D, int k, size_t (*planes_bytes)(i64, int), bool need_ginv, bool need_S) {
+RankWs carve(void* ws, i64 Q, i64 G, int D, int k, size_t (*planes_bytes)(i64, int), bool need_ginv, bool need_S, bool screen) {
     RankWs r{};
     const bool fused = need_S && fused_select(Q, G, k);
     const i64 qb = query_block(Q, G, need_S ? k : 0);
     size_t off = 0;
-    char* base = ws ? (char*)(((uintptr_t)ws + 255) & ~(uintptr_t)255) : nullptr;
+    char* base = ws ? ws_base(ws) : nullptr;
     auto take = [&](size_t bytes) { char* p = base ? base + off : nullptr; off += align_up(bytes, 256); return p; };
+    r.stats = (unsigned*)take(256);
     r.qn = (float*)take((size_t)Q * D * sizeof(float));
     const i64 q_split = need_S ? qb : (Q < 256 * 64 ? Q : 256 * 64);
     r.qs = take(planes_bytes ? planes_bytes(q_split, D) : 0);
@@ -702,6 +776,16 @@
         r.topk_bytes = k > 0 ? topk_ws_bytes(qb, G, k) : 0;
     }
     r.topk = take(r.topk_bytes);
+    if (screen && fused) {
+        const i64 ntx = cdiv(G, RK_BN);
+        r.sc.cap = ntx * RK_BN < SCREEN_CAP ? ntx * RK_BN : SCREEN_CAP;
+        r.sc.blk = (unsigned*)take(256 + (size_t)ntx * 4 * sizeof(unsigned));
+        r.sc.bitmap = r.sc.blk ? r.sc.blk + 64 : nullptr;
+        r.sc.list = (int*)take((size_t)r.sc.cap * sizeof(int));
+        r.sc.ginv_c = (float*)take((size_t)r.sc.cap * sizeof(float));
+        r.sc.erow = (float*)take((size_t)G * sizeof(float));
+        r.sc.etile = (float*)take((size_t)ntx * sizeof(float));
+    }
     r.total = off + 256;
     return r;
 }
@@ -788,6 +872,43 @@
     }
 };
 
+struct ScreenGemm {
+    static constexpr bool SLAB = true, FILTERED = false, ROC = false, RANGE = false;
+    template <int MT> static constexpr size_t stage_bytes() { return (size_t)3 * (64 * MT / 32) * 2 * 1024 + (size_t)3 * RK_BN * 32 * sizeof(float); }
+    template <int MT, int FK, bool FILT> static const void* kernel() { return (const void*)k_cos_gemm_screen<MT, FK>; }
+    template <int MT, int FK, bool FILT>
+    static void launch(dim3 grid, size_t lds, hipStream_t st, const TileArgs& a, int x0, int ntx, int xtiles, int ny) {
+        static_assert(!FILT, "the screen is unfiltered");
+        const bf16_t* qs = (const bf16_t*)a.qry;
+        const int n_steps = cdiv(a.D, 16);
+        const float* zeros = reinterpret_cast<const float*>(qs + (size_t)cdiv(a.Q, 128) * 4 * n_steps * 3 * 512);
+        hipLaunchKernelGGL((k_cos_gemm_screen<MT, FK>), grid, dim3(256), lds, st, qs, (const float*)a.gal, a.ginv, a.S, a.Q, a.G, a.D,
+                           a.k, a.cand_val, a.cand_idx, x0, ntx, n_steps, zeros, xtiles, ny, a.gn2);
+    }
+};
+template <bool LIST>
+struct SplitTwinGemm {
+    static constexpr bool SLAB = false, FILTERED = false, ROC = false, RANGE = false;
+    template <int MT> static constexpr size_t stage_bytes() { return SplitGemm::stage_bytes<MT>(); }
+    template <int MT, int FK, bool FILT> static const void* kernel() {
+        if constexpr (LIST) return (const void*)k_cos_gemm_split_list<MT, FK>;
+        else return (const void*)k_cos_gemm_split_gated<MT, FK>;
+    }
+    template <int MT, int FK, bool FILT>
+    static void launch(dim3 grid, size_t lds, hipStream_t st, const TileArgs& a, int x0, int ntx, int xtiles, int ny) {
+        static_assert(!FILT && FK > 0, "the twins of the screened search are fused and unfiltered");
+        const bf16_t* qs = (const bf16_t*)a.qry;
+        const int n_steps = cdiv(a.D, 16);
+        const float* zeros = reinterpret_cast<const float*>(qs + (size_t)cdiv(a.Q, 128) * 4 * n_steps * 3 * 512);
+        if constexpr (LIST)
+            hipLaunchKernelGGL((k_cos_gemm_split_list<MT, FK>), grid, dim3(256), lds, st, qs, (const float*)a.gal, a.ginv, a.Q, a.D, a.k,
+                               a.cand_val, a.cand_idx, x0, ntx, n_steps, zeros, xtiles, ny, a.cur, a.row_list);
+        else
+            hipLaunchKernelGGL((k_cos_gemm_split_gated<MT, FK>), grid, dim3(256), lds, st, qs, (const float*)a.gal, a.ginv, a.Q, a.G, a.D,
+                               a.k, a.cand_val, a.cand_idx, x0, ntx, n_steps, zeros, xtiles, ny, a.cur);
+    }
+};
+
 struct PreparedGemm {
     static constexpr bool SLAB = false, FILTERED = false, ROC = false, RANGE = false;
     template <int MT> static constexpr size_t stage_bytes() {
@@ -850,6 +971,209 @@
     return OK;
 }
 
+static float screen_c(int D) {
+    const double u = 1.0 / 256, v = 1.0 / 16777216;
+    return (float)((2 * u + u * u + 15.0 * D * v + 8 * v) * (1.0 + 1.0 / 128) * (1.0 + 1e-6));
+}
+static float screen_floor(int D) { return (float)(sqrt((double)D) * ldexp(1.0, -62) * (1.0 + 1e-6)); }
+constexpr int SCREEN_MAX_D = 16384;
+
+__device__ __forceinline__ float nan_max(float a, float b) { return (a > b || a != a) ? a : b; }
+
+__global__ __launch_bounds__(128) void k_screen_eps(float* __restrict__ erow, const float* __restrict__ ginv,
+                                                    float* __restrict__ etile, i64 G, float c, float floor_) {
+    __shared__ float part[2];
+    const i64 g = (i64)blockIdx.x * RK_BN + threadIdx.x;
+    float e = 0.f;
+    if (g < G) {
+        const float n2 = erow[g];
+        if (ginv) e = (n2 < INFINITY && ginv[g] > 0.f) ? c : INFINITY;
+        else e = c * (sqrtf(n2) + floor_);
+        erow[g] = e;
+    }
+    float m = e;
+#pragma unroll
+    for (int o = 32; o > 0; o >>= 1) m = nan_max(m, __shfl_xor(m, o, 64));
+    if ((threadIdx.x & 63) == 0) part[threadIdx.x >> 6] = m;
+    __syncthreads();
+    if (threadIdx.x == 0 && etile) etile[blockIdx.x] = nan_max(part[0], part[1]);
+}
+
+__device__ __forceinline__ bool screen_finite(float x) { return fabsf(x) < INFINITY; }
+
+__global__ __launch_bounds__(256) void k_screen_mark(const float* __restrict__ cand_val, const int* __restrict__ cand_idx, int Q,
+                                                     int ntx, int k, i64 G, const float* __restrict__ tv, const i64* __restrict__ ti,
+                                                     const float* __restrict__ erow, const float* __restrict__ etile,
+                                                     unsigned* __restrict__ bitmap, unsigned* __restrict__ blk) {
+    const i64 t = (i64)blockIdx.x * 256 + threadIdx.x;
+    if (t >= (i64)Q * ntx) return;
+    const int q = (int)(t / ntx), tile = (int)(t - (i64)q * ntx);
+    float ea = 0.f;
+    for (int j = 0; j < k; ++j) {
+        const i64 id = ti[(i64)q * k + j];
+        ea = nan_max(ea, (id >= 0 && id < G) ? erow[id] : NAN);
+    }
+    const float thr = tv[(i64)q * k + k - 1] - ea;
+    const bool thr_ok = screen_finite(thr);
+    const size_t o = (size_t)t * k;
+    bool full = true;
+    float last = 0.f;
+    for (int i = 0; i < k; ++i) {
+        const int id = cand_idx[o + i];
+        if (id == IDX32_PAD) { full = false; break; }
+        last = cand_val[o + i];
+        if (!(thr_ok && screen_finite(last) && last + erow[id] < thr)) atomicOr(&bitmap[id >> 5], 1u << (id & 31));
+    }
+    if (full && !(thr_ok && screen_finite(last) && last + etile[tile] < thr)) {
+        const i64 left = G - (i64)tile * RK_BN;
+        for (int w = 0; w < 4; ++w) {
+            const i64 n = left - w * 32;
+            if (n > 0) atomicOr(&bitmap[tile * 4 + w], n >= 32 ? 0xffffffffu : ((1u << n) - 1u));
+        }
+        atomicAdd(&blk[2], 1u);
+    }
+}
+
+__global__ __launch_bounds__(1024) void k_screen_compact(const unsigned* __restrict__ bitmap, i64 nwords, i64 cap,
+                                                         int* __restrict__ list, const float* __restrict__ ginv,
+                                                         float* __restrict__ ginv_c, unsigned* __restrict__ blk,
+                                                         unsigned* __restrict__ stats, int first) {
+    __shared__ unsigned wtot[16];
+    __shared__ unsigned long long base;
+    const int tid = threadIdx.x, lane = tid & 63, wave = tid >> 6;
+    if (tid == 0) base = 0ull;
+    __syncthreads();
+    for (i64 w0 = 0; w0 < nwords; w0 += 1024) {
+        unsigned w = w0 + tid < nwords ? bitmap[w0 + tid] : 0u;
+        const unsigned c = __popc(w);
+        unsigned incl = c;
+#pragma unroll
+        for (int d = 1; d < 64; d <<= 1) {
+            const unsigned v = __shfl_up(incl, d, 64);
+            if (lane >= d) incl += v;
+        }
+        if (lane == 63) wtot[wave] = incl;
+        __syncthreads();
+        unsigned before = 0, total = 0;
+        for (int i = 0; i < 16; ++i) { before += i < wave ? wtot[i] : 0u; total += wtot[i]; }
+        unsigned long long pos = base + before + incl - c;
+        while (w) {
+            const int b = __ffs(w) - 1;
+            w &= w - 1;
+            if (pos < (unsigned long long)cap) {
+                const i64 row = (w0 + tid) * 32 + b;
+                list[pos] = (int)row;
+                if (ginv) ginv_c[pos] = ginv[row];
+            }
+            ++pos;
+        }
+        __syncthreads();
+        if (tid == 0) base += total;
+        __syncthreads();
+    }
+    if (tid == 0) {
+        const unsigned long long n = base;
+        const unsigned fb = n > (unsigned long long)cap ? 1u : 0u;
+        blk[0] = fb ? 0u : (unsigned)n;
+        blk[1] = fb;
+        const unsigned rows = n > 0xffffffffull ? 0xffffffffu : (unsigned)n;
+        stats[0] = (first ? 0u : stats[0]) + rows;
+        stats[1] = (first ? 0u : stats[1]) + blk[2];
+        stats[2] = (first ? 0u : stats[2]) + fb;
+        stats[3] = (unsigned)cap;
+        stats[4] = (first ? 0u : stats[4]) + 1u;
+    }
+}
+
+__global__ __launch_bounds__(256) void k_screen_remap(i64* __restrict__ idx, i64 n, const int* __restrict__ list,
+                                                      const unsigned* __restrict__ blk, i64 idx_offset) {
+    const i64 t = (i64)blockIdx.x * 256 + threadIdx.x;
+    if (t >= n) return;
+    const i64 v = idx[t];
+    if (v >= 0 && v < (i64)blk[0]) idx[t] = (i64)list[v] + idx_offset;
+}
+
+constexpr i64 SCREEN_MIN_Q = 256, SCREEN_MIN_G = 100000, SCREEN_BLOCK_Q = 256;
+constexpr int SCREEN_MAX_K = 4;
+enum { SCREEN_OFF = 0, SCREEN_FORCED = 1, SCREEN_AUTO = 2 };
+static int screen_mode(i64 Q, i64 G, int k) {
+    const char* e = getenv("MI355_RANK_SCREEN");
+    if (e && e[0] == '0') return SCREEN_OFF;
+    if (e && e[0] == '1') return SCREEN_FORCED;
+    return Q >= SCREEN_MIN_Q && G >= SCREEN_MIN_G && k <= SCREEN_MAX_K ? SCREEN_AUTO : SCREEN_OFF;
+}
+static bool screen_in_scope(const float* gallery, i64 Q, i64 G, int dim, int k, float eps, const RankFilter* filt) {
+    return !filt && fused_select(Q, G, k) && vec_ok(gallery, dim) && !rank_exact_f32() && dim <= SCREEN_MAX_D && eps >= 1e-12f;
+}
+
+static int rank_topk_screened(const float* queries, i64 Q, const float* gallery, const float* ginv, i64 G, int dim, int k, float eps,
+                              i64 idx_offset, float* out_val, i64* out_idx, const RankWs& w, hipStream_t st, bool forced) {
+    if (int e = normalize_search(queries, Q, ginv ? gallery : nullptr, G, dim, eps, w, st)) return e;
+    const ScreenWs& sc = w.sc;
+    const i64 qb0 = query_block(Q, G, k), qb = qb0 < SCREEN_BLOCK_Q ? qb0 : SCREEN_BLOCK_Q;
+    bool first = true;
+    const int ntx = cdiv(G, RK_BN), ltx = (int)(sc.cap / RK_BN);
+    const i64 rowlen = (i64)ntx * k;
+    const float c = screen_c(dim), fl = screen_floor(dim);
+    bf16_t* qs = (bf16_t*)w.qs;
+    for (i64 q0 = 0; q0 < Q; q0 += qb) {
+        const i64 qn = (Q - q0 < qb) ? Q - q0 : qb;
+        float* ov = out_val + q0 * k;
+        i64* oi = out_idx + q0 * k;
+        if (!forced && qn < SCREEN_MIN_Q) {
+            if (int e = cos_gemm(w.qn + q0 * dim, qs, gallery, ginv, nullptr, qn, G, dim, st, k, w.cand_val, w.cand_idx)) return e;
+            if (int e = topk_select(w.cand_val, nullptr, qn, rowlen, rowlen, k, idx_offset, ov, oi, w.topk, w.topk_bytes, st, w.cand_idx))
+                return e;
+            continue;
+        }
+        if (int e = split_rows(w.qn + q0 * dim, qn, dim, qs, st)) return e;
+        MI355_CHECK_HIP(hipMemsetAsync(sc.blk, 0, 256 + (size_t)ntx * 4 * sizeof(unsigned), st));
+        {
+            RoctxRange range("rank/screen gemm + per-tile top-k");
+            TileArgs a{qs, gallery, ginv, nullptr, (int)qn, G, dim, k, w.cand_val, w.cand_idx};
+            a.gn2 = sc.erow;
+            if (int e = cos_gemm_tiles<ScreenGemm>(a, st)) return e;
+        }
+        {
+            RoctxRange range("rank/screen candidates");
+            hipLaunchKernelGGL(k_screen_eps, dim3((unsigned)ntx), dim3(128), 0, st, sc.erow, ginv, sc.etile, G, c, fl);
+            MI355_LAUNCH_CHECK();
+            if (int e = topk_select(w.cand_val, nullptr, qn, rowlen, rowlen, k, 0, ov, oi, w.topk, w.topk_bytes, st, w.cand_idx)) return e;
+            hipLaunchKernelGGL(k_screen_mark, dim3((unsigned)cdiv(qn * ntx, 256)), dim3(256), 0, st, w.cand_val, w.cand_idx, (int)qn, ntx,
+                               k, G, ov, oi, sc.erow, sc.etile, sc.bitmap, sc.blk);
+            MI355_LAUNCH_CHECK();
+            hipLaunchKernelGGL(k_screen_compact, dim3(1), dim3(1024), 0, st, sc.bitmap, (i64)ntx * 4, sc.cap, sc.list, ginv, sc.ginv_c,
+                               sc.blk, w.stats, first ? 1 : 0);
+            first = false;
+            MI355_LAUNCH_CHECK();
+        }
+        {
+            RoctxRange range("rank/exact re-score of the candidates");
+            TileArgs a{qs, gallery, ginv ? sc.ginv_c : nullptr, nullptr, (int)qn, sc.cap, dim, k, w.cand_val, w.cand_idx};
+            a.cur = sc.blk;
+            a.row_list = sc.list;
+            if (int e = launch_fk<SplitTwinGemm<true>, 1, false>(a, st)) return e;
+            if (int e = topk_select(w.cand_val, nullptr, qn, (i64)ltx * k, (i64)ltx * k, k, 0, ov, oi, w.topk, w.topk_bytes, st,
+                                    w.cand_idx))
+                return e;
+            hipLaunchKernelGGL(k_screen_remap, dim3((unsigned)cdiv(qn * k, 256)), dim3(256), 0, st, oi, qn * k, sc.list, sc.blk,
+                               idx_offset);
+            MI355_LAUNCH_CHECK();
+        }
+        {
+            RoctxRange range("rank/full fallback (gated)");
+            TileArgs a{qs, gallery, ginv, nullptr, (int)qn, G, dim, k, w.cand_val, w.cand_idx};
+            a.cur = sc.blk;
+            if (int e = cos_gemm_tiles<SplitTwinGemm<false>>(a, st)) return e;
+            if (int e = topk_select(w.cand_val, nullptr, qn, rowlen, rowlen, k, idx_offset, ov, oi, w.topk, w.topk_bytes, st,
+                                    w.cand_idx, nullptr, sc.blk))
+                return e;
+        }
+    }
+    set_rank_path(MI355_RANK_PATH_SPLIT | MI355_RANK_PATH_FUSED | MI355_RANK_PATH_SCREENED);
+    return OK;
+}
+
 static int check_rank_args(const float* queries, i64 Q, const float* gallery, i64 G, int dim) {
     MI355_REQUIRE(queries && gallery, "rank: null queries/gallery pointer");
     MI355_REQUIRE(Q >= 1, "rank: Q=%lld must be >= 1", (long long)Q);
@@ -869,10 +1193,13 @@
 static int rank_topk(const float* queries, i64 Q, const float* gallery, i64 G, int dim, int gallery_is_normalized, int k, float eps,
                      i64 idx_offset, float* out_val, i64* out_idx, void* workspace, size_t workspace_bytes, hipStream_t st,
                      const RankFilter* filt) {
-    const RankWs w = carve(workspace, Q, G, dim, k, split_queries_bytes, !gallery_is_normalized);
+    const RankWs w = carve(workspace, Q, G, dim, k, split_queries_bytes, !gallery_is_normalized, true, true);
     MI355_REQUIRE(workspace && workspace_bytes >= w.total, "rank_topk: workspace %zu < %zu bytes", workspace_bytes,
                   w.total);
     const float* ginv = gallery_is_normalized ? nullptr : w.ginv;
+    const int screen = screen_in_scope(gallery, Q, G, dim, k, eps, filt) ? screen_mode(Q, G, k) : SCREEN_OFF;
+    if (screen != SCREEN_OFF)
+        return rank_topk_screened(queries, Q, gallery, ginv, G, dim, k, eps, idx_offset, out_val, out_idx, w, st, screen == SCREEN_FORCED);
     return search_blocks(queries, ginv ? gallery : nullptr, Q, G, dim, k, eps, idx_offset, filt, out_val, out_idx, w, st, nullptr,
                          [&](i64 q0, i64 qn, const RankFilter* f) -> int {
                              RoctxRange range(w.cand_val ? "rank/cosine gemm + per-tile top-k" : nullptr);
@@ -901,7 +1228,7 @@
 size_t mi355_rank_workspace_bytes(int64_t Q, int64_t G, int dim, int k) {
     if (Q < 1 || G < 1) return 0;
     if (dim <= 0) return topk_ws_bytes(Q, G, k < 1 ? 1 : k) + 256;
-    return carve(nullptr, Q, G, dim, k, split_queries_bytes, true).total;
+    return carve(nullptr, Q, G, dim, k, split_queries_bytes, true, true, true).total;
 }
 
 int mi355_cosine_scores(const float* queries, int64_t Q, const float* gallery, int64_t G, int dim,
@@ -949,6 +1276,41 @@
 }
 
 int mi355_rank_last_path(void) { return g_rank_path; }
+
+int mi355_rank_screen_stats(const void* workspace, int64_t* out, void* stream) {
+    MI355_REQUIRE(workspace && out, "rank_screen_stats: null pointer");
+    const unsigned* stats = (const unsigned*)ws_base((void*)workspace);
+    unsigned h[5] = {0, 0, 0, 0, 0};
+    MI355_CHECK_HIP(hipMemcpyAsync(h, stats, sizeof(h), hipMemcpyDeviceToHost, (hipStream_t)stream));
+    MI355_CHECK_HIP(hipStreamSynchronize((hipStream_t)stream));
+    for (int i = 0; i < 5; ++i) out[i] = h[i];
+    return OK;
+}
+
+int mi355_rank_screen_scores(const float* queries, int64_t Q, const float* gallery, int64_t G, int dim, int gallery_is_normalized,
+                             float eps, float* out_scores, float* out_bound, void* workspace, size_t workspace_bytes, void* stream) {
+    if (int e = check_rank_args(queries, Q, gallery, G, dim)) return e;
+    MI355_REQUIRE(out_scores && out_bound, "rank_screen_scores: null output");
+    MI355_REQUIRE(Q <= 256 * 64 && G < ((int64_t)1 << 31) - RK_BN, "rank_screen_scores: shape too large Q=%lld G=%lld", (long long)Q,
+                  (long long)G);
+    if (!vec_ok(gallery, dim) || dim > SCREEN_MAX_D || !(eps >= 1e-12f)) {
+        set_error("rank_screen_scores: the screen needs 16-byte aligned rows, dim <= %d and eps >= 1e-12", SCREEN_MAX_D);
+        return ERR_UNSUPPORTED;
+    }
+    hipStream_t st = (hipStream_t)stream;
+    const RankWs w = carve(workspace, Q, G, dim, 0, split_queries_bytes, !gallery_is_normalized, false);
+    MI355_REQUIRE(workspace && workspace_bytes >= w.total, "rank_screen_scores: workspace %zu < %zu bytes", workspace_bytes, w.total);
+    const float* ginv = gallery_is_normalized ? nullptr : w.ginv;
+    if (int e = normalize_search(queries, Q, ginv ? gallery : nullptr, G, dim, eps, w, st)) return e;
+    if (int e = split_rows(w.qn, Q, dim, (bf16_t*)w.qs, st)) return e;
+    TileArgs a{w.qs, gallery, ginv, out_scores, (int)Q, G, dim, 0};
+    a.gn2 = out_bound;
+    if (int e = cos_gemm_tiles<ScreenGemm>(a, st)) return e;
+    hipLaunchKernelGGL(k_screen_eps, dim3((unsigned)cdiv(G, RK_BN)), dim3(128), 0, st, out_bound, ginv, (float*)nullptr, (i64)G,
+                       screen_c(dim), screen_floor(dim));
+    MI355_LAUNCH_CHECK();
+    return OK;
+}
 
 size_t mi355_roc_pairs_workspace_bytes(int64_t Q, int64_t G, int dim) {
     if (Q < 1 || G < 1 || dim < 1) return 0;
diff --git a/imageretrievalresearch_amd/csrc/rank_common.h b/imageretrievalresearch_amd/csrc/rank_common.h
--- a/imageretrievalresearch_amd/csrc/rank_common.h
+++ b/imageretrievalresearch_amd/csrc/rank_common.h
@@ -441,7 +441,7 @@
 size_t topk_ws_bytes(i64 Q, i64 G, int k);
 int topk_select(const float* vals, const i64* idxs, i64 Q, i64 rowlen, i64 in_stride, int k, i64 idx_offset, float* out_val,
                 i64* out_idx, void* ws, size_t ws_bytes, hipStream_t st, const int* idxs32 = nullptr,
-                const RankFilter* filt = nullptr);
+                const RankFilter* filt = nullptr, const unsigned* gate = nullptr);
 RankFilter filter_from(const RankFilter& f, i64 q0);
 int make_filter(const mi355_rank_filter* f, i64 idx_offset, const char* who, RankFilter* out);
 void set_rank_path(int path);
@@ -465,6 +465,9 @@
     const RankFilter* filt;
     const RocArgs* roc;
     const RangeArgs* rng;
+    float* gn2;
+    const unsigned* cur;
+    const int* row_list;
 };
 
 constexpr size_t EPI_TILE_BYTES = (size_t)64 * (RK_BN + 4) * sizeof(float);
@@ -534,10 +537,24 @@
 RocArgs roc_from(const RocArgs& a, i64 q0);
 i64 roc_query_block(i64 Q, i64 G);
 
+struct ScreenWs {
+    unsigned* blk;
+    unsigned* bitmap;
+    int* list;
+    float* ginv_c;
+    float* erow;
+    float* etile;
+    i64 cap;
+};
 struct RankWs {
+    unsigned* stats;
     float* qn; void* qs; float* ginv; float* S; float* cand_val; int* cand_idx; void* topk; size_t topk_bytes; size_t total;
+    ScreenWs sc;
 };
-RankWs carve(void* ws, i64 Q, i64 G, int D, int k, size_t (*planes_bytes)(i64, int), bool need_ginv, bool need_S = true);
+constexpr i64 SCREEN_CAP = 32768;
+static inline char* ws_base(void* ws) { return (char*)(((uintptr_t)ws + 255) & ~(uintptr_t)255); }
+RankWs carve(void* ws, i64 Q, i64 G, int D, int k, size_t (*planes_bytes)(i64, int), bool need_ginv, bool need_S = true,
+             bool screen = false);
 int normalize_search(const float* queries, i64 Q, const float* gallery, i64 G, int dim, float eps, const RankWs& w,
                      hipStream_t st);
 
diff --git a/imageretrievalresearch_amd/csrc/rank_gemm_screen.inc b/imageretrievalresearch_amd/csrc/rank_gemm_screen.inc
--- /dev/null
+++ b/imageretrievalresearch_amd/csrc/rank_gemm_screen.inc
@@ -0,0 +1,136 @@
+    constexpr int BM = 64 * MT;
+    constexpr int BK = 32;
+    constexpr int A_PIECES = (BM / 32) * 2;
+    constexpr int A_STAGE = A_PIECES * 512;
+    constexpr int A_PER_WAVE = A_PIECES / 4;
+    constexpr int B_STAGE = RK_BN * BK;
+    extern __shared__ __attribute__((aligned(16))) float smem[];
+    bf16_t* As = reinterpret_cast<bf16_t*>(smem);
+    float* Bs = smem + (3 * A_STAGE * 2) / 4;
+
+    const int tid = threadIdx.x, lane = tid & 63, wave = tid >> 6;
+    const int wm = wave >> 1, wn = wave & 1;
+    int bx, by;
+    rank_tile_of((int)blockIdx.x, xtiles, ny, bx, by);
+    const i64 n0 = (i64)(bx + x0) * RK_BN;
+    const int m0 = by * BM;
+    const int swave = __builtin_amdgcn_readfirstlane(wave);
+    const int n32 = (n_steps + 1) >> 1;
+
+    const float* b_row[4];
+    int b_k[4];
+    bool b_ok[4];
+#pragma unroll
+    for (int i = 0; i < 4; ++i) {
+        const int r = (swave * 4 + i) * 8 + (lane >> 3);
+        const int c = (lane & 7) ^ ((r >> 1) & 7);
+        b_ok[i] = n0 + r < G;
+        b_row[i] = Gal + (b_ok[i] ? (n0 + r) * D : 0);
+        b_k[i] = c * 4;
+    }
+    auto dma_b = [&](int stage, int k0) {
+#pragma unroll
+        for (int i = 0; i < 4; ++i) {
+            const bool ok = b_ok[i] && k0 + b_k[i] < D;
+            glds16(reinterpret_cast<const bf16_t*>(ok ? b_row[i] + k0 + b_k[i] : zeros),
+                   reinterpret_cast<bf16_t*>(Bs + stage * B_STAGE + (swave * 4 + i) * 256));
+        }
+    };
+    const bf16_t* a_src[A_PER_WAVE];
+#pragma unroll
+    for (int i = 0; i < A_PER_WAVE; ++i) {
+        const int a = swave + 4 * i;
+        a_src[i] = Qs + (size_t)(m0 / 32 + (a >> 1)) * n_steps * 3 * 512 + lane * 8;
+    }
+    auto dma_a = [&](int stage, int t) {
+#pragma unroll
+        for (int i = 0; i < A_PER_WAVE; ++i) {
+            const int a = swave + 4 * i;
+            int t16 = 2 * t + (a & 1);
+            t16 = t16 < n_steps ? t16 : n_steps - 1;
+            glds16(a_src[i] + (size_t)t16 * 3 * 512, As + stage * A_STAGE + a * 512);
+        }
+    };
+
+    f32x16 acc[MT][2];
+#pragma unroll
+    for (int i = 0; i < MT; ++i)
+#pragma unroll
+        for (int j = 0; j < 2; ++j)
+#pragma unroll
+            for (int e = 0; e < 16; ++e) acc[i][j][e] = 0.f;
+    const bool want_n2 = gn2 != nullptr;
+    float n2[2] = {0.f, 0.f};
+
+    const int lr = lane & 31;
+    int b_off[2][2][2];
+#pragma unroll
+    for (int j = 0; j < 2; ++j) {
+        const int r = wn * 64 + j * 32 + lr, sw = (r >> 1) & 7;
+#pragma unroll
+        for (int s = 0; s < 2; ++s) {
+            const int c0 = 4 * s + (lane >> 5) * 2;
+            b_off[j][s][0] = r * BK + ((c0 ^ sw) << 2);
+            b_off[j][s][1] = r * BK + (((c0 + 1) ^ sw) << 2);
+        }
+    }
+    auto compute = [&](int stage) {
+        const bf16_t* a = As + stage * A_STAGE + (wm * MT * 2) * 512 + lane * 8;
+        const float* b = Bs + stage * B_STAGE;
+#pragma unroll
+        for (int s = 0; s < 2; ++s) {
+            bf16x8 af[MT], gf[2];
+#pragma unroll
+            for (int j = 0; j < 2; ++j) {
+                const f32x4 v0 = *reinterpret_cast<const f32x4*>(b + b_off[j][s][0]);
+                const f32x4 v1 = *reinterpret_cast<const f32x4*>(b + b_off[j][s][1]);
+                const u32x4 p = {pack2bf(v0.x, v0.y), pack2bf(v0.z, v0.w), pack2bf(v1.x, v1.y), pack2bf(v1.z, v1.w)};
+                gf[j] = *reinterpret_cast<const bf16x8*>(&p);
+                if (want_n2) {
+#pragma unroll
+                    for (int e = 0; e < 4; ++e) {
+                        const float lo = __uint_as_float(p[e] << 16), hi = __uint_as_float(p[e] & 0xffff0000u);
+                        n2[j] = fmaf(lo, lo, n2[j]);
+                        n2[j] = fmaf(hi, hi, n2[j]);
+                    }
+                }
+            }
+#pragma unroll
+            for (int i = 0; i < MT; ++i) af[i] = *reinterpret_cast<const bf16x8*>(a + (i * 2 + s) * 512);
+#pragma unroll
+            for (int j = 0; j < 2; ++j)
+#pragma unroll
+                for (int i = 0; i < MT; ++i) acc[i][j] = __builtin_amdgcn_mfma_f32_32x32x16_bf16(af[i], gf[j], acc[i][j], 0, 0, 0);
+        }
+    };
+
+    dma_a(0, 0);
+    dma_b(0, 0);
+    dma_a(1, 1);
+    dma_b(1, BK);
+    __syncthreads();
+
+    int cur = 0, far = 2;
+    for (int t = 0; t < n32; ++t) {
+        dma_a(far, t + 2);
+        dma_b(far, (t + 2) * BK);
+        __builtin_amdgcn_sched_barrier(0);
+        compute(cur);
+        if constexpr (A_PER_WAVE == 2) asm volatile("s_waitcnt vmcnt(6)" ::: "memory");
+        else asm volatile("s_waitcnt vmcnt(5)" ::: "memory");
+        asm volatile("s_waitcnt lgkmcnt(0)" ::: "memory");
+        __builtin_amdgcn_s_barrier();
+        asm volatile("" ::: "memory");
+        cur = cur == 2 ? 0 : cur + 1;
+        far = far == 2 ? 0 : far + 1;
+    }
+    __syncthreads();
+    if (want_n2 && wm == 0 && by == 0) {
+#pragma unroll
+        for (int j = 0; j < 2; ++j) {
+            const float v = n2[j] + __shfl_xor(n2[j], 32, 64);
+            const i64 col = n0 + wn * 64 + j * 32 + lr;
+            if (lane < 32 && col < G) gn2[col] = v;
+        }
+    }
+    cos_gemm_epilogue<MT, FK, false>(acc, smem, ginv, S, Q, G, k, cand_val, cand_idx, x0, ntx, n0, m0, RankFilter{});
diff --git a/imageretrievalresearch_amd/csrc/rank_gemm_split.inc b/imageretrievalresearch_amd/csrc/rank_gemm_split.inc
--- a/imageretrievalresearch_amd/csrc/rank_gemm_split.inc
+++ b/imageretrievalresearch_amd/csrc/rank_gemm_split.inc
@@ -24,7 +24,7 @@
         const int r = (swave * 2 + i) * 16 + (lane >> 2);
         const int c = (lane & 3) ^ ((r >> 2) & 3);
         b_ok[i] = n0 + r < G;
-        b_row[i] = Gal + (b_ok[i] ? (n0 + r) * D : 0);
+        b_row[i] = Gal + (b_ok[i] ? split_row(n0 + r) * D : 0);
         b_k[i] = c * 4;
     }
     auto dma_b = [&](int stage, int k0) {
diff --git a/imageretrievalresearch_amd/rank.py b/imageretrievalresearch_amd/rank.py
--- a/imageretrievalresearch_amd/rank.py
+++ b/imageretrievalresearch_amd/rank.py
@@ -127,6 +127,36 @@
         check(lib().mi355_cosine_scores(q.data_ptr(), Q, g.data_ptr(), G, D, int(gallery_is_normalized), eps,
                                         out.data_ptr(), ws.data_ptr(), ws.numel(), stream_ptr(q.device)))
     return out
+
+
+class ScreenStats(NamedTuple):
+    union_rows: int
+    whole_tile_marks: int
+    full_fallbacks: int
+    capacity: int
+    query_blocks: int
+
+
+def screen_stats(device) -> ScreenStats:
+    ws = _ws.get(device, 256)
+    out = (ctypes.c_int64 * 5)()
+    with torch.cuda.device(device):
+        check(lib().mi355_rank_screen_stats(ws.data_ptr(), out, stream_ptr(torch.device(device))))
+    return ScreenStats(*(int(v) for v in out))
+
+
+def screen_scores(queries: torch.Tensor, gallery: torch.Tensor, eps: float = _EPS, gallery_is_normalized: bool = False):
+    q, g = _f32c(queries, "queries"), _f32c(gallery, "gallery")
+    _check_qg(q, g)
+    Q, D = q.shape
+    G = g.shape[0]
+    out = torch.empty((Q, G), dtype=torch.float32, device=q.device)
+    bound = torch.empty((G,), dtype=torch.float32, device=q.device)
+    ws = _ws.get(q.device, lib().mi355_rank_workspace_bytes(Q, G, D, 0))
+    with torch.cuda.device(q.device):
+        check(lib().mi355_rank_screen_scores(q.data_ptr(), Q, g.data_ptr(), G, D, int(gallery_is_normalized), eps,
+                                             out.data_ptr(), bound.data_ptr(), ws.data_ptr(), ws.numel(), stream_ptr(q.device)))
+    return out, bound
 
 
 _LABEL_MODES = {None: LABEL_ANY, "same": LABEL_SAME, "different": LABEL_DIFFERENT}
diff --git a/include/mi355_retrieval.h b/include/mi355_retrieval.h
--- a/include/mi355_retrieval.h
+++ b/include/mi355_retrieval.h
@@ -65,9 +65,14 @@
     MI355_RANK_PATH_F16_GEMM = 5,
     MI355_RANK_PATH_F16_GEMV = 6,
     MI355_RANK_PATH_FUSED = 0x100,
-    MI355_RANK_PATH_BITONIC = 0x200
+    MI355_RANK_PATH_BITONIC = 0x200,
+    MI355_RANK_PATH_SCREENED = 0x400
 };
 int mi355_rank_last_path(void);
+
+int mi355_rank_screen_stats(const void* workspace, int64_t* out, void* stream);
+int mi355_rank_screen_scores(const float* queries, int64_t Q, const float* gallery, int64_t G, int dim, int gallery_is_normalized,
+                             float eps, float* out_scores, float* out_bound, void* workspace, size_t workspace_bytes, void* stream);
 
 #define MI355_ROC_MAX_THRESHOLDS 4096
 size_t mi355_roc_pairs_workspace_bytes(int64_t Q, int64_t G, int dim);
```

Result: faster. 62420 (median of 6 runs) (+2.9%).
